# karltan0328/POPE

Hardware: AMD Instinct MI355X
Metric: image-pairs/s (DINOv2-S/14 extract+match, 640x480) (higher is better)
Workload: dtype f16x3 (fp32 operands split hi+lo into f16, 3 MFMAs per product, fp32 accumulate)

## Files before the change

include/pope_hip.h:

```cpp
#ifndef POPE_HIP_H
#define POPE_HIP_H

#include <stddef.h>

#ifdef __cplusplus
extern "C" {
#endif

#define POPE_ABI_VERSION 9

enum {
    POPE_EPI_BIAS = 0,
    POPE_EPI_BIAS_GELU = 1,
    POPE_EPI_BIAS_LS_RES = 2,
    POPE_EPI_BIAS_SWIGLU = 11,
    POPE_EPI_QKV_F16 = 8
};

enum { POPE_PREC_F32_MFMA = 0, POPE_PREC_F16X3 = 1, POPE_PREC_F16 = 2  };
enum { POPE_RANGE_PATCH = 1, POPE_RANGE_LAYERNORM = 2, POPE_RANGE_QKV = 4, POPE_RANGE_GELU = 8, POPE_RANGE_MATCH = 16,
       POPE_RANGE_INPUT = 32 };

int pope_abi_version(void);
const char* pope_error_string(int code);
// ... 7 lines not shown
int pope_linear_prec_f32(const float* A, const float* W, const float* bias, float* C, int M, int N, int K,
                         int epilogue, const float* gamma, const float* res, int precision,
                         unsigned* range_flag, void* stream);

#define POPE_PLANES_ACT_SCALE 8.0f
#define POPE_PLANES_W_SCALE 256.0f
int pope_split_planes_f32(const float* src, void* planes, int rows, int cols, float scale,
                          unsigned* range_flag, void* stream);
int pope_linear_planes_f32(const void* a_planes, const void* w_planes, const float* bias, float* C,
                           void* c_planes, int M, int N, int K, int epilogue, const float* gamma,
                           const float* res, unsigned* range_flag, void* stream);

int pope_layernorm_planes_f32(const float* x, const float* weight, const float* bias, void* y_planes,
                              int rows, int dim, float eps, unsigned* range_flag, void* stream);

int pope_linear_rowln_f32(const void* a_planes, const void* w_planes, int M, int K, const float* bias, const float* gamma,
                          const float* res, int res_mod, float* x, const float* ln_w, const float* ln_b, float eps,
                          void* ln_planes, float* ln_out, unsigned* range_flag, void* stream);
int pope_layernorm_rowln_order_f32(const float* x, const float* weight, const float* bias, void* y_planes, float* y_f32,
                                   int rows, float eps, unsigned* range_flag, void* stream);

int pope_layernorm_f16(const float* x, const float* weight, const float* bias, void* y_f16, int rows, int dim, float eps,
                       unsigned* range_flag, void* stream);
int pope_to_f16(const float* x, void* y_f16, long long n, unsigned* range_flag, void* stream);
int pope_linear_f16(const void* a_f16, const void* w_f16, const float* bias, float* C, void* c_f16, int M, int N, int K,
                    int epilogue, const float* gamma, const float* res, int res_mod, unsigned* range_flag, void* stream);
int pope_div_planes_f32(const float* src, long long batch_stride, void* planes, int n, int rows, int cols, float divisor,
                        float scale, unsigned* range_flag, void* stream);

int pope_patch_embed_f32(const float* img, const float* proj_w, const float* posb, float* tokens,
                         int B, int H, int W, int patch, int dim, void* stream);
int pope_patch_embed_planes_f32(const float* img, const void* proj_w_planes, const float* posb, float* tokens,
                                int B, int H, int W, int patch, int dim, void* a_planes_scratch,
                                size_t scratch_bytes, unsigned* range_flag, void* stream);

int pope_attention_f32(const float* qkv, float* out, int B, int N, int heads, void* stream);
int pope_attention_prec_f32(const float* qkv, float* out, int B, int N, int heads, int precision,
                            unsigned* range_flag, void* stream);
int pope_attention_planes_f32(const void* qkv_planes, void* out_planes, int B, int N, int heads, void* stream);

int pope_attention_f16(const void* qkv_f16, void* out_f16, int B, int N, int heads, void* stream);

int pope_attention_planes_diag_f32(const void* qkv_planes, void* out_planes, int B, int N, int heads, long long* exact_passes_host,
                                   void* stream);

int pope_cls_cosine_f32(const float* ref, const float* fea, int P, int D, float eps, float* scores,
                        void* stream);


typedef struct pope_vit_block_weights {
    const float *norm1_w, *norm1_b;
    const float *qkv_w, *qkv_b;
    const float *proj_w, *proj_b;
    const float *ls1;
    const float *norm2_w, *norm2_b;
    const float *fc1_w, *fc1_b;
    const float *fc2_w, *fc2_b;
    const float *ls2;
    const void *qkv_wp, *fc1_wp, *fc2_wp, *proj_wp;
} pope_vit_block_weights;

typedef struct pope_vit_weights {
    int dim, depth, heads, patch, hidden;
    const float* patch_w;
    const float *norm_w, *norm_b;
    const pope_vit_block_weights* blocks_host;
    int precision;
    const void* patch_wp;
} pope_vit_weights;

size_t pope_vit_workspace_bytes(int B, int ntok, int dim, int hidden);

enum { POPE_FFN_MLP = 0, POPE_FFN_SWIGLU = 1 };

int pope_vit_forward_f32(const pope_vit_weights* w_host, const float* img, int B, int H, int W,
                         const float* posb, float* x_prenorm, float* x_norm,
                         int n_taps, const int* tap_blocks_host, float* const* tap_out_host,
                         void* workspace, size_t workspace_bytes, unsigned* range_flag, void* stream);

int pope_vit_forward_ffn_f32(const pope_vit_weights* w_host, int ffn, const float* img, int B, int H, int W,
                             const float* posb, float* x_prenorm, float* x_norm,
                             int n_taps, const int* tap_blocks_host, float* const* tap_out_host,
                             void* workspace, size_t workspace_bytes, unsigned* range_flag, void* stream);

enum { POPE_K_PATCH_EMBED = 0, POPE_K_LAYERNORM = 1, POPE_K_GEMM_QKV = 2, POPE_K_ATTENTION = 3,
       POPE_K_GEMM_PROJ = 4, POPE_K_GEMM_FC1 = 5, POPE_K_GEMM_FC2 = 6, POPE_K_TAP_COPY = 7 };
int pope_vit_launch_count(int depth);
int pope_vit_forward_profiled_mask_f32(const pope_vit_weights* w_host, const float* img, int B, int H, int W,
                                       const float* posb, float* x_prenorm, float* x_norm,
                                       void* workspace, size_t workspace_bytes, unsigned* range_flag, void* stream,
                                       void* const* events_host, int n_events, int* kinds_host,
                                       int* n_launches_host, unsigned kind_mask);
int pope_vit_forward_ffn_profiled_mask_f32(const pope_vit_weights* w_host, int ffn, const float* img, int B, int H, int W,
                                           const float* posb, float* x_prenorm, float* x_norm,
                                           void* workspace, size_t workspace_bytes, unsigned* range_flag, void* stream,
                                           void* const* events_host, int n_events, int* kinds_host,
                                           int* n_launches_host, unsigned kind_mask);
int pope_event_create(void** event_host);
int pope_event_destroy(void* event);
int pope_event_elapsed_ms(void* start, void* stop, float* ms_host);


size_t pope_dense_match_workspace_bytes_prec(int n, int L, int S, int C, int precision, int publish_conf);
int pope_dense_match_prec_f32(const float* feat0, long long stride0, const float* feat1, long long stride1,
                              int n, int L, int S, int C, int h0, int w0, int h1, int w1,
                              float thr, int border_rm, float temperature, float scale,
                              float* conf_matrix, long long* b_ids, long long* i_ids, long long* j_ids,
                              float* mconf, float* mkpts0_c, float* mkpts1_c, int* counts,
                              void* workspace, size_t workspace_bytes, int precision, unsigned* range_flag,
                              void* stream);
size_t pope_dense_match_masked_workspace_bytes(int n, int L, int S, int C, int precision, int publish_conf, int has_border_masks);
int pope_dense_match_masked_f32(const float* feat0, long long stride0, const float* feat1, long long stride1,
                                int n, int L, int S, int C, int h0, int w0, int h1, int w1,
                                float thr, int border_rm, float temperature, float scale,
                                const float* fill_mask0, const float* fill_mask1, const float* border_mask0,
                                const float* border_mask1, const float* scale0, const float* scale1,
                                float* conf_matrix, long long* b_ids, long long* i_ids, long long* j_ids,
                                float* mconf, float* mkpts0_c, float* mkpts1_c, int* counts,
                                void* workspace, size_t workspace_bytes, int precision, unsigned* range_flag,
                                void* stream);
size_t pope_dense_match_sinkhorn_workspace_bytes(int n, int L, int S, int C, int precision, int publish_conf, int has_border_masks);
int pope_dense_match_sinkhorn_f32(const float* feat0, long long stride0, const float* feat1, long long stride1,
                                  int n, int L, int S, int C, int h0, int w0, int h1, int w1,
                                  float thr, int border_rm, const float* bin_score, int skh_iters, int skh_prefilter, float scale,
                                  const float* fill_mask0, const float* fill_mask1, const float* border_mask0,
                                  const float* border_mask1, const float* scale0, const float* scale1,
                                  float* conf_matrix, long long* b_ids, long long* i_ids, long long* j_ids,
                                  float* mconf, float* mkpts0_c, float* mkpts1_c, int* counts,
                                  void* workspace, size_t workspace_bytes, int precision, unsigned* range_flag,
                                  void* stream);
size_t pope_dense_match_workspace_bytes(int n, int L, int S);
int pope_dense_match_f32(const float* feat0, long long stride0, const float* feat1, long long stride1,
                         int n, int L, int S, int C,
                         int h0, int w0, int h1, int w1, float thr, int border_rm, float temperature,
                         float scale, float* conf_matrix, long long* b_ids, long long* i_ids,
                         long long* j_ids, float* mconf, float* mkpts0_c, float* mkpts1_c, int* counts,
                         void* workspace, size_t workspace_bytes, void* stream);


typedef struct pope_loftr_layer_weights {
    const void *q_wp, *kv_wp, *merge_wp, *mlp0_wp, *mlp1_wp;
    const float *norm1_w, *norm1_b, *norm2_w, *norm2_b;
} pope_loftr_layer_weights;
size_t pope_loftr_layer_workspace_bytes(int n, int L, int S, int C, int nhead);
int pope_loftr_encoder_layer_f32(const pope_loftr_layer_weights* w_host, float* x, const float* source,
                                 int n, int L, int S, int C, int nhead, float ln_eps, int precision,
                                 void* workspace, size_t workspace_bytes, unsigned* range_flag, void* stream);
int pope_loftr_encoder_layer_masked_f32(const pope_loftr_layer_weights* w_host, float* x, const float* source,
                                        const float* x_mask, const float* source_mask,
                                        int n, int L, int S, int C, int nhead, float ln_eps, int precision,
                                        void* workspace, size_t workspace_bytes, unsigned* range_flag, void* stream);
int pope_loftr_encoder_layer_full_f32(const pope_loftr_layer_weights* w_host, float* x, const float* source,
                                      int n, int L, int S, int C, int nhead, float ln_eps, int precision,
                                      void* workspace, size_t workspace_bytes, unsigned* range_flag, void* stream);
int pope_loftr_full_attention_f32(const float* q, const float* kv, int n, int L, int S, int C, int nhead, int precision,
                                  float* out, unsigned* range_flag, void* stream);

typedef struct pope_resnetfpn_weights {
    const void* w[22];
    const float* b[22];
} pope_resnetfpn_weights;
size_t pope_resnetfpn_workspace_bytes(int n, int H, int W);
int pope_resnetfpn_forward_f32(const pope_resnetfpn_weights* w_host, const float* gray, int n, int H, int W, int precision,
                               float* out_c, float* out_f, void* workspace, size_t workspace_bytes,
                               unsigned* range_flag, void* stream);

enum { POPE_CONV3 = 0, POPE_CONV_S2 = 1, POPE_CONV1_UP = 2, POPE_CONV_STEM = 3 };
typedef struct pope_conv_layer_args {
    int form, precision;
    int n, H, W;
    int cch, taps;
    const void* a;
    size_t a_rows;
    const void* w;
    const float* bias;
    int N, ldc;
    float slope;
    void* out_planes;
    float* out_f32;
    int zero_border;
    const void* res;
    int ldres;
    const float* up_src;
    int up_lds;
    void* scratch;
    size_t scratch_bytes;
    unsigned* range_flag;
} pope_conv_layer_args;
size_t pope_conv_layer_scratch_bytes(int form, int n, int H, int W, int cch, int taps);
int pope_conv_layer_f32(const pope_conv_layer_args* args_host, void* stream);

size_t pope_fine_preprocess_workspace_bytes(int M, int Wn, int Cc, int Cf);
int pope_fine_preprocess_f32(const float* feat_f0, const long long* strides0_host, int H0, int W0, int wc0,
// ... 291 lines not shown
```

pope_amd/_lib.py:

```python
import ctypes as C
import os
import subprocess

_CSRC = os.path.join(os.path.dirname(os.path.abspath(__file__)), "csrc")
LIB_PATH = os.environ.get("POPE_LIB_PATH") or os.path.join(_CSRC, "libpope_hip.so")

c_float_p = C.POINTER(C.c_float)
c_int_p = C.POINTER(C.c_int)
c_ll_p = C.POINTER(C.c_longlong)


class VitBlockWeights(C.Structure):
    _fields_ = [(n, C.c_void_p) for n in (
        "norm1_w", "norm1_b", "qkv_w", "qkv_b", "proj_w", "proj_b", "ls1",
        "norm2_w", "norm2_b", "fc1_w", "fc1_b", "fc2_w", "fc2_b", "ls2", "qkv_wp", "fc1_wp", "fc2_wp", "proj_wp")]


class VitWeights(C.Structure):
    _fields_ = [("dim", C.c_int), ("depth", C.c_int), ("heads", C.c_int), ("patch", C.c_int),
                ("hidden", C.c_int), ("patch_w", C.c_void_p), ("norm_w", C.c_void_p),
                ("norm_b", C.c_void_p), ("blocks_host", C.POINTER(VitBlockWeights)), ("precision", C.c_int),
                ("patch_wp", C.c_void_p)]


# ... 56 lines not shown
    _fields_ = [("num_sample", C.c_int), ("mode", C.c_int), ("layers", PoseRegressorLayer * 4), ("mlp_w", C.c_void_p * 7),
                ("mlp_b", C.c_void_p * 7)] + [(n, C.c_void_p) for n in ("trans_w", "trans_b", "rot_w", "rot_b")]


class MocopeEncoderLayer(C.Structure):
    _fields_ = [(n, C.c_void_p) for n in ("in_proj_w", "in_proj_b", "out_proj_w", "out_proj_b", "linear1_w", "linear1_b", "linear2_w",
                                           "linear2_b", "norm1_w", "norm1_b", "norm2_w", "norm2_b")]


class MocopeDecoderLayer(C.Structure):
    _fields_ = [(n, C.c_void_p) for n in ("in_proj_w", "in_proj_b", "out_proj_w", "out_proj_b", "cross_in_proj_w", "cross_in_proj_b",
                                           "cross_out_proj_w", "cross_out_proj_b", "linear1_w", "linear1_b", "linear2_w", "linear2_b",
                                           "norm1_w", "norm1_b", "norm2_w", "norm2_b", "norm3_w", "norm3_b")]


class MocopeTransformer(C.Structure):
    _fields_ = [("enc", MocopeEncoderLayer * 6), ("enc_norm_w", C.c_void_p), ("enc_norm_b", C.c_void_p),
                ("dec", MocopeDecoderLayer * 6), ("dec_norm_w", C.c_void_p), ("dec_norm_b", C.c_void_p)]


class MocopeWeights(C.Structure):
    _fields_ = [("num_sample", C.c_int), ("mode", C.c_int), ("transformer_mkpts", MocopeTransformer), ("mkpts_as_q", MocopeTransformer),
                ("cnn_as_q", MocopeTransformer), ("mlp1_w", C.c_void_p * 2), ("mlp1_b", C.c_void_p * 2), ("mlp_img_w", C.c_void_p),
                ("mlp_img_b", C.c_void_p), ("mlp2_w", C.c_void_p * 7), ("mlp2_b", C.c_void_p * 7)] + [
        (n, C.c_void_p) for n in ("trans_w", "trans_b", "rot_w", "rot_b")]


class ConvNextBlockWeights(C.Structure):
    _fields_ = [(n, C.c_void_p) for n in ("dw_w", "dw_b", "norm_w", "norm_b", "pw1_w", "pw1_b", "grn_gamma", "grn_beta", "pw2_w",
                                           "pw2_b", "pw1_wp", "pw2_wp")]


class ConvNextWeights(C.Structure):
    _fields_ = [("depths", C.c_int * 4), ("dims", C.c_int * 4), ("num_classes", C.c_int)] + [
        (n, C.c_void_p) for n in ("stem_w", "stem_b", "stem_ln_w", "stem_ln_b")] + [
        (n, C.c_void_p * 3) for n in ("ds_ln_w", "ds_ln_b", "ds_w", "ds_b", "ds_wp")] + [
        ("blocks_host", C.POINTER(ConvNextBlockWeights))] + [(n, C.c_void_p) for n in ("norm_w", "norm_b", "head_w", "head_b", "ones")]


PREC_F32_MFMA, PREC_F16X3, PREC_F16 = 0, 1, 2
PLANES_ACT_SCALE, PLANES_W_SCALE = 8.0, 256.0
PRECISIONS = {"f32": PREC_F32_MFMA, "f16x3": PREC_F16X3, "f16": PREC_F16}
FFN_KINDS = {"mlp": 0, "swiglu": 1}
EPI_BIAS_SWIGLU = 11
EPI_QKV_F16 = 8
CONV3, CONV_S2, CONV1_UP, CONV_STEM = 0, 1, 2, 3
c_uint_p = C.POINTER(C.c_uint)
F16_MAX = 65504.0
RANGE_BITS = {1: "patch embed input", 2: "LayerNorm output", 4: "q/k/v", 8: "MLP hidden (GELU / SwiGLU output)",
              16: "matcher features", 32: "op-level operand"}

PROTOTYPES = {
    "pope_abi_version": (C.c_int, []),
    "pope_error_string": (C.c_char_p, [C.c_int]),
    "pope_layernorm_f32": (C.c_int, [C.c_void_p] * 4 + [C.c_int, C.c_int, C.c_float, C.c_void_p]),
    "pope_linear_f32": (C.c_int, [C.c_void_p] * 4 + [C.c_int] * 4 + [C.c_void_p] * 3),
    "pope_linear_prec_f32": (C.c_int, [C.c_void_p] * 4 + [C.c_int] * 4 + [C.c_void_p] * 2 + [C.c_int, C.c_void_p, C.c_void_p]),
    "pope_split_planes_f32": (C.c_int, [C.c_void_p, C.c_void_p, C.c_int, C.c_int, C.c_float, C.c_void_p, C.c_void_p]),
    "pope_linear_planes_f32": (C.c_int, [C.c_void_p] * 5 + [C.c_int] * 4 + [C.c_void_p] * 4),
    "pope_layernorm_planes_f32": (C.c_int, [C.c_void_p] * 4 + [C.c_int, C.c_int, C.c_float, C.c_void_p, C.c_void_p]),
    "pope_linear_rowln_f32": (C.c_int, [C.c_void_p, C.c_void_p, C.c_int, C.c_int] + [C.c_void_p] * 3 + [C.c_int]
                              + [C.c_void_p] * 3 + [C.c_float] + [C.c_void_p] * 4),
    "pope_layernorm_rowln_order_f32": (C.c_int, [C.c_void_p] * 5 + [C.c_int, C.c_float, C.c_void_p, C.c_void_p]),
    "pope_layernorm_f16": (C.c_int, [C.c_void_p] * 4 + [C.c_int, C.c_int, C.c_float, C.c_void_p, C.c_void_p]),
    "pope_to_f16": (C.c_int, [C.c_void_p, C.c_void_p, C.c_longlong, C.c_void_p, C.c_void_p]),
    "pope_linear_f16": (C.c_int, [C.c_void_p] * 5 + [C.c_int] * 4 + [C.c_void_p, C.c_void_p, C.c_int, C.c_void_p, C.c_void_p]),
    "pope_div_planes_f32": (C.c_int, [C.c_void_p, C.c_longlong, C.c_void_p, C.c_int, C.c_int, C.c_int, C.c_float, C.c_float,
                                      C.c_void_p, C.c_void_p]),
    "pope_patch_embed_f32": (C.c_int, [C.c_void_p] * 4 + [C.c_int] * 5 + [C.c_void_p]),
    "pope_attention_f32": (C.c_int, [C.c_void_p, C.c_void_p, C.c_int, C.c_int, C.c_int, C.c_void_p]),
    "pope_attention_prec_f32": (C.c_int, [C.c_void_p, C.c_void_p, C.c_int, C.c_int, C.c_int, C.c_int, C.c_void_p, C.c_void_p]),
    "pope_patch_embed_planes_f32": (C.c_int, [C.c_void_p] * 4 + [C.c_int] * 5 + [C.c_void_p, C.c_size_t, C.c_void_p, C.c_void_p]),
    "pope_attention_planes_f32": (C.c_int, [C.c_void_p, C.c_void_p, C.c_int, C.c_int, C.c_int, C.c_void_p]),
    "pope_attention_f16": (C.c_int, [C.c_void_p, C.c_void_p, C.c_int, C.c_int, C.c_int, C.c_void_p]),
    "pope_attention_planes_diag_f32": (C.c_int, [C.c_void_p, C.c_void_p, C.c_int, C.c_int, C.c_int, c_ll_p, C.c_void_p]),
    "pope_cls_cosine_f32": (C.c_int, [C.c_void_p, C.c_void_p, C.c_int, C.c_int, C.c_float, C.c_void_p, C.c_void_p]),
    "pope_vit_workspace_bytes": (C.c_size_t, [C.c_int] * 4),
    "pope_vit_forward_f32": (C.c_int, [C.POINTER(VitWeights), C.c_void_p, C.c_int, C.c_int, C.c_int, C.c_void_p,
                                       C.c_void_p, C.c_void_p, C.c_int, c_int_p, C.POINTER(C.c_void_p),
                                       C.c_void_p, C.c_size_t, C.c_void_p, C.c_void_p]),
    "pope_vit_forward_ffn_f32": (C.c_int, [C.POINTER(VitWeights), C.c_int, C.c_void_p, C.c_int, C.c_int, C.c_int, C.c_void_p,
                                           C.c_void_p, C.c_void_p, C.c_int, c_int_p, C.POINTER(C.c_void_p),
                                           C.c_void_p, C.c_size_t, C.c_void_p, C.c_void_p]),
    "pope_vit_forward_ffn_profiled_mask_f32": (C.c_int, [C.POINTER(VitWeights), C.c_int, C.c_void_p, C.c_int, C.c_int, C.c_int,
                                                         C.c_void_p, C.c_void_p, C.c_void_p, C.c_void_p, C.c_size_t,
                                                         C.c_void_p, C.c_void_p, C.POINTER(C.c_void_p), C.c_int, c_int_p,
                                                         c_int_p, C.c_uint]),
    "pope_vit_launch_count": (C.c_int, [C.c_int]),
    "pope_vit_forward_profiled_mask_f32": (C.c_int, [C.POINTER(VitWeights), C.c_void_p, C.c_int, C.c_int, C.c_int,
                                                     C.c_void_p, C.c_void_p, C.c_void_p, C.c_void_p, C.c_size_t,
                                                     C.c_void_p, C.c_void_p, C.POINTER(C.c_void_p), C.c_int, c_int_p,
                                                     c_int_p, C.c_uint]),
    "pope_event_create": (C.c_int, [C.POINTER(C.c_void_p)]),
    "pope_event_destroy": (C.c_int, [C.c_void_p]),
    "pope_event_elapsed_ms": (C.c_int, [C.c_void_p, C.c_void_p, c_float_p]),
    "pope_dense_match_workspace_bytes": (C.c_size_t, [C.c_int] * 3),
    "pope_dense_match_f32": (C.c_int, [C.c_void_p, C.c_longlong, C.c_void_p, C.c_longlong] + [C.c_int] * 8 + [C.c_float, C.c_int, C.c_float,
                                                                                  C.c_float] + [C.c_void_p] * 8
                             + [C.c_void_p, C.c_size_t, C.c_void_p]),
    "pope_dense_match_workspace_bytes_prec": (C.c_size_t, [C.c_int] * 6),
    "pope_dense_match_prec_f32": (C.c_int, [C.c_void_p, C.c_longlong, C.c_void_p, C.c_longlong] + [C.c_int] * 8
                                  + [C.c_float, C.c_int, C.c_float, C.c_float] + [C.c_void_p] * 8
                                  + [C.c_void_p, C.c_size_t, C.c_int, C.c_void_p, C.c_void_p]),
    "pope_dense_match_masked_workspace_bytes": (C.c_size_t, [C.c_int] * 7),
    "pope_dense_match_masked_f32": (C.c_int, [C.c_void_p, C.c_longlong, C.c_void_p, C.c_longlong] + [C.c_int] * 8
                                    + [C.c_float, C.c_int, C.c_float, C.c_float] + [C.c_void_p] * 6 + [C.c_void_p] * 8
                                    + [C.c_void_p, C.c_size_t, C.c_int, C.c_void_p, C.c_void_p]),
    "pope_dense_match_sinkhorn_workspace_bytes": (C.c_size_t, [C.c_int] * 7),
    "pope_dense_match_sinkhorn_f32": (C.c_int, [C.c_void_p, C.c_longlong, C.c_void_p, C.c_longlong] + [C.c_int] * 8
                                      + [C.c_float, C.c_int, C.c_void_p, C.c_int, C.c_int, C.c_float] + [C.c_void_p] * 6
                                      + [C.c_void_p] * 8 + [C.c_void_p, C.c_size_t, C.c_int, C.c_void_p, C.c_void_p]),
    "pope_loftr_layer_workspace_bytes": (C.c_size_t, [C.c_int] * 5),
    "pope_loftr_encoder_layer_f32": (C.c_int, [C.POINTER(LoftrLayerWeights), C.c_void_p, C.c_void_p] + [C.c_int] * 5
                                     + [C.c_float, C.c_int, C.c_void_p, C.c_size_t, C.c_void_p, C.c_void_p]),
    "pope_loftr_encoder_layer_masked_f32": (C.c_int, [C.POINTER(LoftrLayerWeights)] + [C.c_void_p] * 4 + [C.c_int] * 5
                                            + [C.c_float, C.c_int, C.c_void_p, C.c_size_t, C.c_void_p, C.c_void_p]),
    "pope_loftr_encoder_layer_full_f32": (C.c_int, [C.POINTER(LoftrLayerWeights), C.c_void_p, C.c_void_p] + [C.c_int] * 5
                                          + [C.c_float, C.c_int, C.c_void_p, C.c_size_t, C.c_void_p, C.c_void_p]),
    "pope_loftr_full_attention_f32": (C.c_int, [C.c_void_p, C.c_void_p] + [C.c_int] * 6 + [C.c_void_p, C.c_void_p, C.c_void_p]),
    "pope_resnetfpn_workspace_bytes": (C.c_size_t, [C.c_int] * 3),
    "pope_resnetfpn_forward_f32": (C.c_int, [C.POINTER(ResnetFpnWeights), C.c_void_p, C.c_int, C.c_int, C.c_int, C.c_int, C.c_void_p,
                                             C.c_void_p, C.c_void_p, C.c_size_t, C.c_void_p, C.c_void_p]),
    "pope_conv_layer_scratch_bytes": (C.c_size_t, [C.c_int] * 6),
    "pope_conv_layer_f32": (C.c_int, [C.POINTER(ConvLayerArgs), C.c_void_p]),
    "pope_fine_preprocess_workspace_bytes": (C.c_size_t, [C.c_int] * 4),
    "pope_fine_preprocess_f32": (C.c_int, [C.c_void_p, c_ll_p, C.c_int, C.c_int, C.c_int, C.c_void_p, c_ll_p, C.c_int, C.c_int, C.c_int,
                                           C.c_void_p, C.c_void_p] + [C.c_int] * 4 + [C.c_void_p] * 3 + [C.c_int] * 3
                                 + [C.c_void_p] * 4 + [C.c_int, C.c_void_p] + [C.c_void_p, C.c_size_t, C.c_void_p, C.c_void_p]),
    "pope_fine_preprocess_indexed_f32": (C.c_int, [C.c_void_p, c_ll_p, C.c_int, C.c_int, C.c_int, C.c_void_p, c_ll_p, C.c_int, C.c_int,
                                                   C.c_int, C.c_void_p, C.c_void_p] + [C.c_int] * 4 + [C.c_void_p] * 3 + [C.c_int] * 3
                                         + [C.c_void_p] * 4 + [C.c_int, C.c_void_p] + [C.c_void_p, C.c_size_t, C.c_void_p]
                                         + [C.c_void_p, C.c_int, C.c_int, C.c_void_p]),
    "pope_fine_match_f32": (C.c_int, [C.c_void_p, C.c_void_p, C.c_int, C.c_int, C.c_int, C.c_void_p, C.c_float, C.c_void_p,
                                      C.c_void_p, C.c_void_p]),
    "pope_fine_match_scaled_f32": (C.c_int, [C.c_void_p, C.c_void_p, C.c_int, C.c_int, C.c_int, C.c_void_p, C.c_float, C.c_void_p,
                                             C.c_void_p, C.c_void_p, C.c_void_p, C.c_void_p]),
    "pope_sam_encoder_workspace_bytes": (C.c_size_t, [C.POINTER(SamEncoderWeights), C.c_int]),
    "pope_sam_encoder_forward_f32": (C.c_int, [C.POINTER(SamEncoderWeights), C.c_void_p, C.c_int, C.c_void_p, C.c_int, c_int_p,
                                               C.POINTER(C.c_void_p), C.c_void_p, C.c_size_t, C.c_void_p, C.c_void_p]),
    "pope_sam_decoder_workspace_bytes": (C.c_size_t, [C.POINTER(SamDecoderWeights), C.c_int, C.c_int, C.c_int]),
    "pope_sam_decoder_forward_f32": (C.c_int, [C.POINTER(SamDecoderWeights)] + [C.c_void_p] * 3 + [C.c_int, C.c_int, C.c_void_p,
                                                                                                  C.c_longlong, C.c_int]
                                     + [C.c_void_p] * 5 + [C.c_size_t, C.c_void_p, C.c_void_p]),
    "pope_sam_decoder_images_workspace_bytes": (C.c_size_t, [C.POINTER(SamDecoderWeights), C.c_int, c_int_p, C.c_int, C.c_int,
                                                             C.c_longlong]),
    "pope_sam_decoder_forward_images_f32": (C.c_int, [C.POINTER(SamDecoderWeights), C.c_void_p, C.c_int, C.c_void_p, C.c_void_p,
                                                      c_int_p, C.c_int, C.c_int, C.c_void_p, C.c_longlong, C.c_int]
                                            + [C.c_void_p] * 3 + [C.c_size_t, C.c_void_p, C.c_void_p]),
    "pope_sam_mask_embed_f32": (C.c_int, [C.POINTER(SamMaskEmbedWeights), C.c_void_p, C.c_int, C.c_void_p, C.c_void_p]),
    "pope_sam_postprocess_workspace_bytes": (C.c_size_t, [C.c_int] * 3),
    "pope_sam_postprocess_f32": (C.c_int, [C.c_void_p] + [C.c_int] * 3 + [C.c_void_p] + [C.c_int] * 6 + [C.c_double, C.c_double]
                                 + [C.c_void_p] * 4 + [C.c_size_t, C.c_void_p]),
    "pope_sam_nms_f32": (C.c_int, [C.c_void_p, C.c_void_p, C.c_int, C.c_float, C.c_void_p, C.c_void_p, C.c_void_p]),
    "pope_sam_nms_segments_f32": (C.c_int, [C.c_void_p] * 3 + [C.c_int, C.c_int, C.c_float, C.c_void_p, C.c_void_p, C.c_void_p]),
    "pope_sam_rle_u32": (C.c_int, [C.c_void_p] + [C.c_int] * 3 + [C.c_void_p] * 3 + [C.c_longlong, C.c_void_p]),
    "pope_sam_small_regions_workspace_bytes": (C.c_size_t, [C.c_int] * 3),
    "pope_sam_small_regions_u32": (C.c_int, [C.c_void_p] + [C.c_int] * 4 + [C.c_void_p] * 5 + [C.c_size_t, C.c_void_p]),
    "pope_preprocess_u8_f32": (C.c_int, [C.c_void_p, C.c_int, C.c_int, C.c_int] + [C.c_void_p] * 3 + [C.c_int] + [C.c_void_p] * 3
                               + [C.c_int] * 7 + [c_float_p, c_float_p, C.c_void_p, C.c_void_p, C.c_size_t, C.c_void_p]),
    "pope_resize_u8": (C.c_int, [C.c_void_p, C.c_int, C.c_int, C.c_int] + [C.c_void_p] * 3 + [C.c_int] + [C.c_void_p] * 3
                       + [C.c_int] * 3 + [C.c_void_p, C.c_void_p, C.c_size_t, C.c_void_p]),
    "pope_sam_preprocess_u8_f32": (C.c_int, [C.c_void_p, C.c_int, C.c_int, C.c_int] + [C.c_void_p] * 3 + [C.c_int] + [C.c_void_p] * 3
                                   + [C.c_int] * 5 + [c_float_p, c_float_p, C.c_void_p, C.c_void_p, C.c_size_t, C.c_void_p]),
    "pope_crop_normalize_u8_f32": (C.c_int, [C.c_void_p] + [C.c_int] * 7 + [c_float_p, c_float_p, C.c_void_p, C.c_void_p]),
    "pope_gray_u8_f32": (C.c_int, [C.c_void_p, C.c_int, C.c_int, C.c_int, C.c_void_p, C.c_void_p]),
    "pope_pose_images_u8_f32": (C.c_int, [C.c_void_p] + [C.c_int] * 3 + [C.c_void_p, C.c_int] + [C.c_void_p] * 4 + [C.c_int] * 3
                                + [C.c_void_p, C.c_void_p]),
    "pope_crop_warp_u8": (C.c_int, [C.c_void_p, C.c_int, C.c_int, C.c_int, C.c_void_p, C.c_void_p, C.c_int, C.c_int, C.c_int, C.c_void_p,
                                    C.c_void_p]),
    "pope_estimate_pose_workspace_bytes": (C.c_size_t, [C.c_int, C.c_longlong]),
    "pope_estimate_pose_f64": (C.c_int, [C.c_void_p] * 5 + [C.c_int, C.c_longlong, C.c_double, C.c_double, C.c_int, C.c_ulonglong]
                               + [C.c_void_p] * 5 + [C.c_void_p, C.c_size_t, C.c_void_p]),
    "pope_pose_regressor_workspace_bytes": (C.c_size_t, [C.c_int, C.c_int]),
    "pope_pose_regressor_forward_f32": (C.c_int, [C.POINTER(PoseRegressorWeights)] + [C.c_void_p] * 7 + [C.c_int] * 3 + [C.c_longlong]
                                        + [C.c_void_p] * 4 + [C.c_size_t, C.c_void_p]),
    "pope_pose_regressor_embedding_f32": (C.c_int, [C.c_void_p] * 7 + [C.c_int, C.c_int, C.c_longlong] + [C.c_void_p] * 4),
    "pope_pose_regressor_encoder_f32": (C.c_int, [C.POINTER(PoseRegressorWeights)] + [C.c_void_p] * 7 + [C.c_int] * 3 + [C.c_longlong]
                                        + [C.c_void_p] * 4),
    "pope_pose_regressor_layer_f32": (C.c_int, [C.POINTER(PoseRegressorLayer), C.c_void_p] + [C.c_int] * 3 + [C.c_void_p]),
    "pope_pose_regressor_stream_linear_f32": (C.c_int, [C.c_void_p] * 4 + [C.c_int, C.c_longlong, C.c_int, C.c_void_p]),
    "pope_pose_regressor_tail_f32": (C.c_int, [C.POINTER(PoseRegressorWeights), C.c_void_p, C.c_void_p, C.c_int] + [C.c_void_p] * 3),
    "pope_mocope_linear_f32": (C.c_int, [C.c_void_p] * 4 + [C.c_int] * 4 + [C.c_void_p]),
    "pope_mocope_attention_f32": (C.c_int, [C.c_void_p, C.c_int] * 3 + [C.c_void_p] + [C.c_int] * 4 + [C.c_void_p]),
    "pope_mocope_add_ln_f32": (C.c_int, [C.c_void_p] * 6 + [C.c_int, C.c_int, C.c_void_p]),
    "pope_mocope_ffn76_f32": (C.c_int, [C.c_void_p] * 9 + [C.c_int, C.c_void_p]),
    "pope_mocope_workspace_bytes": (C.c_size_t, [C.c_int, C.c_int]),
# ... 180 lines not shown
```

pope_amd/csrc/capi.hip:

```cpp
#include "../../include/pope_hip.h"
#include "common.h"
#include "conv_layer.h"
#include "kernels.h"
#include "linear.h"
#include "stream_device.h"
#include <cstdlib>

namespace {

__global__ __launch_bounds__(256) void cls_cosine_kernel(const float* __restrict__ ref, const float* __restrict__ fea,
                                                          int P, int D, float eps, float* __restrict__ scores) {
    const int lane = threadIdx.x & 63;
    const int p = blockIdx.x * 4 + (threadIdx.x >> 6);
    if (p >= P) return;
    const float* f = fea + size_t(p) * D;
    float dot = 0.f, nr = 0.f, nf = 0.f;
    for (int i = lane; i < D; i += 64) {
        const float a = ref[i], b = f[i];
        dot += a * b;
        nr += a * a;
        nf += b * b;
    }
    dot = wave_sum(dot);
    nr = wave_sum(nr);
// ... 119 lines not shown
    StreamDevice on_device(stream);
    return pope_launch_div_planes(src, batch_stride, planes, n, rows, cols, divisor, scale, range_flag, static_cast<hipStream_t>(stream));
}

int pope_patch_embed_f32(const float* img, const float* proj_w, const float* posb, float* tokens, int B, int H,
                         int W, int patch, int dim, void* stream) {
    StreamDevice on_device(stream);
    return pope_launch_patch_embed_f32(img, proj_w, posb, tokens, B, H, W, patch, dim, static_cast<hipStream_t>(stream));
}

int pope_patch_embed_planes_f32(const float* img, const void* proj_w_planes, const float* posb, float* tokens, int B, int H,
                                int W, int patch, int dim, void* a_planes_scratch, size_t scratch_bytes, unsigned* range_flag,
                                void* stream) {
    StreamDevice on_device(stream);
    return pope_launch_patch_embed_planes(img, proj_w_planes, posb, tokens, B, H, W, patch, dim, a_planes_scratch, scratch_bytes,
                                          range_flag, static_cast<hipStream_t>(stream));
}

int pope_attention_planes_f32(const void* qkv_planes, void* out_planes, int B, int N, int heads, void* stream) {
    StreamDevice on_device(stream);
    if (!qkv_planes || !out_planes) return POPE_ERR_ARG;
    return pope_launch_attention_f16x3_planes_io(qkv_planes, out_planes, B, N, heads, static_cast<hipStream_t>(stream));
}

int pope_attention_f16(const void* qkv_f16, void* out_f16, int B, int N, int heads, void* stream) {
    StreamDevice on_device(stream);
    return pope_launch_attention_f16_dma(qkv_f16, out_f16, B, N, heads, static_cast<hipStream_t>(stream));
}

int pope_attention_planes_diag_f32(const void* qkv_planes, void* out_planes, int B, int N, int heads, long long* exact_passes_host,
                                   void* stream) {
    StreamDevice on_device(stream);
    if (!qkv_planes || !out_planes) return POPE_ERR_ARG;
    return pope_launch_attention_f16x3_planes_io_diag(qkv_planes, out_planes, B, N, heads, exact_passes_host, static_cast<hipStream_t>(stream));
}

int pope_attention_f32(const float* qkv, float* out, int B, int N, int heads, void* stream) {
    return pope_attention_prec_f32(qkv, out, B, N, heads, POPE_PREC_F32_MFMA, nullptr, stream);
}

int pope_attention_prec_f32(const float* qkv, float* out, int B, int N, int heads, int precision, unsigned* range_flag,
                            void* stream) {
    StreamDevice on_device(stream);
    if (!qkv || !out) return POPE_ERR_ARG;
    if (precision == POPE_PREC_F16X3 && range_flag) {
        if (B <= 0 || N <= 0 || heads <= 0) return POPE_ERR_ARG;
        const int rc = pope_launch_range_check(qkv, size_t(B) * N * 3 * heads * 64, 1.0f, range_flag, POPE_RANGE_INPUT,
                                               static_cast<hipStream_t>(stream));
        if (rc) return rc;
    }
    if (precision == POPE_PREC_F16X3) return pope_launch_attention_f16x3(qkv, out, B, N, heads, static_cast<hipStream_t>(stream));
    if (precision != POPE_PREC_F32_MFMA) return POPE_ERR_ARG;
    return pope_launch_attention_f32(qkv, out, B, N, heads, static_cast<hipStream_t>(stream));
}

int pope_cls_cosine_f32(const float* ref, const float* fea, int P, int D, float eps, float* scores, void* stream) {
    StreamDevice on_device(stream);
    if (!ref || !fea || !scores || P <= 0 || D <= 0) return POPE_ERR_ARG;
    hipLaunchKernelGGL(cls_cosine_kernel, dim3((P + 3) / 4), dim3(256), 0, static_cast<hipStream_t>(stream), ref, fea,
                       P, D, eps, scores);
    return pope_check_launch();
}

int pope_event_create(void** event_host) {
    if (!event_host) return POPE_ERR_ARG;
    hipEvent_t e;
    if (hipEventCreate(&e) != hipSuccess) return POPE_ERR_LAUNCH;
    *event_host = e;
    return POPE_OK;
}
int pope_event_destroy(void* event) {
    return hipEventDestroy(static_cast<hipEvent_t>(event)) == hipSuccess ? POPE_OK : POPE_ERR_LAUNCH;
}
int pope_event_elapsed_ms(void* start, void* stop, float* ms_host) {
    if (!ms_host) return POPE_ERR_ARG;
    return hipEventElapsedTime(ms_host, static_cast<hipEvent_t>(start), static_cast<hipEvent_t>(stop)) == hipSuccess
               ? POPE_OK : POPE_ERR_LAUNCH;
}

namespace {
struct MatchLayout {
    size_t nl, ns, part, rowp, colp, pl0, pl1, simb, total;
    int ncb, nrb, nrb2, ldp;
    MatchLayout(int n, int L, int S, int C, int precision, bool publish_conf) {
        nl = pope_align256(size_t(n) * L * 4);
        ns = pope_align256(size_t(n) * S * 4);
        ncb = 2 * ((S + 127) / 128);
        nrb = 4 * ((L + 127) / 128);
        nrb2 = pope_match_nrb2(L);
        ldp = (S + 3) & ~3;
        part = pope_align256(size_t(n) * nrb2 * ldp * 4);
        const bool x3 = precision == POPE_PREC_F16X3;
        rowp = x3 ? pope_align256(size_t(n) * L * ncb * 8) : 0;
        colp = x3 ? pope_align256(size_t(n) * nrb * ldp * 4) : 0;
        pl0 = x3 ? pope_align256(size_t(n) * L * C * 4) : 0;
        pl1 = x3 ? pope_align256(size_t(n) * S * C * 4) : 0;
        simb = publish_conf ? 0 : pope_align256(size_t(n) * L * S * 4);
        total = 7 * nl + 3 * ns + part + rowp + 2 * colp + pl0 + pl1 + simb;
    }
};
}

size_t pope_dense_match_workspace_bytes(int n, int L, int S) {
    if (n <= 0 || L <= 0 || S <= 0) return 0;
    return MatchLayout(n, L, S, 4, POPE_PREC_F32_MFMA, true).total;
}

size_t pope_dense_match_workspace_bytes_prec(int n, int L, int S, int C, int precision, int publish_conf) {
    if (n <= 0 || L <= 0 || S <= 0 || C <= 0) return 0;
    return MatchLayout(n, L, S, C, precision, publish_conf != 0).total;
}

int pope_dense_match_f32(const float* feat0, long long stride0, const float* feat1, long long stride1, int n, int L,
                         int S, int C, int h0, int w0, int h1, int w1, float thr, int border_rm, float temperature, float scale, float* conf_matrix,
                         long long* b_ids, long long* i_ids, long long* j_ids, float* mconf, float* mkpts0_c,
                         float* mkpts1_c, int* counts, void* workspace, size_t workspace_bytes, void* stream) {
    return pope_dense_match_prec_f32(feat0, stride0, feat1, stride1, n, L, S, C, h0, w0, h1, w1, thr, border_rm, temperature, scale,
                                     conf_matrix, b_ids, i_ids, j_ids, mconf, mkpts0_c, mkpts1_c, counts, workspace,
                                     workspace_bytes, POPE_PREC_F32_MFMA, nullptr, stream);
}

int pope_dense_match_prec_f32(const float* feat0, long long stride0, const float* feat1, long long stride1, int n, int L,
                              int S, int C, int h0, int w0, int h1, int w1, float thr, int border_rm, float temperature, float scale, float* conf_matrix,
                              long long* b_ids, long long* i_ids, long long* j_ids, float* mconf, float* mkpts0_c,
                              float* mkpts1_c, int* counts, void* workspace, size_t workspace_bytes, int precision,
                              unsigned* range_flag, void* stream) {
    return pope_dense_match_masked_f32(feat0, stride0, feat1, stride1, n, L, S, C, h0, w0, h1, w1, thr, border_rm, temperature, scale,
                                       nullptr, nullptr, nullptr, nullptr, nullptr, nullptr, conf_matrix, b_ids, i_ids, j_ids, mconf,
                                       mkpts0_c, mkpts1_c, counts, workspace, workspace_bytes, precision, range_flag, stream);
}

size_t pope_dense_match_masked_workspace_bytes(int n, int L, int S, int C, int precision, int publish_conf, int has_border_masks) {
    if (n <= 0 || L <= 0 || S <= 0 || C <= 0) return 0;
    return MatchLayout(n, L, S, C, precision, publish_conf != 0).total + (has_border_masks ? pope_align256(size_t(n) * 4 * 4) : 0);
}

namespace {
struct SinkhornLayout {
    size_t u, v, cmax, total;
    SinkhornLayout(int n, int L, int S) {
        u = pope_align256(size_t(n) * (L + 1) * 4);
        v = pope_align256(size_t(n) * (S + 1) * 4);
        cmax = pope_align256(size_t(n) * S * 4);
        total = u + v + cmax;
    }
};

int dense_match_entry(const float* feat0, long long stride0, const float* feat1, long long stride1, int n, int L,
                      int S, int C, int h0, int w0, int h1, int w1, float thr, int border_rm, float temperature, float scale,
                      const float* fill_mask0, const float* fill_mask1, const float* border_mask0, const float* border_mask1,
                      const float* scale0, const float* scale1, float* conf_matrix, long long* b_ids, long long* i_ids,
                      long long* j_ids, float* mconf, float* mkpts0_c, float* mkpts1_c, int* counts, void* workspace,
                      size_t workspace_bytes, int precision, unsigned* range_flag, void* stream, const float* bin_score,
                      int skh_iters, int skh_prefilter) {
    if (!feat0 || !feat1 || !b_ids || !i_ids || !j_ids || !mconf || !mkpts0_c || !mkpts1_c || !counts || !workspace)
        return POPE_ERR_ARG;
    if (n <= 0 || L <= 0 || S <= 0 || C <= 0) return POPE_ERR_ARG;
    if (precision != POPE_PREC_F32_MFMA && precision != POPE_PREC_F16X3) return POPE_ERR_ARG;
    StreamDevice on_device(stream);
    const bool publish = conf_matrix != nullptr;
    const bool padded = border_mask0 || border_mask1;
    const MatchLayout lay(n, L, S, C, precision, publish);
    const size_t ext_bytes = padded ? pope_align256(size_t(n) * 4 * 4) : 0;
    const SinkhornLayout skh(n, L, S);
    if (workspace_bytes < lay.total + ext_bytes + (bin_score ? skh.total : 0)) return POPE_ERR_WORKSPACE;
    pope_carver ws{static_cast<char*>(workspace)};
    MatchParams p = {};
    p.feat0 = feat0; p.feat1 = feat1;
    p.n = n; p.L = L; p.S = S; p.C = C;
    p.bs0 = stride0; p.bs1 = stride1;
    p.h0 = h0; p.w0 = w0; p.h1 = h1; p.w1 = w1;
    p.thr = thr; p.temperature = temperature; p.border = border_rm; p.scale = scale;
    p.publish_conf = publish;
    p.ncb = lay.ncb; p.nrb = lay.nrb; p.nrb2 = lay.nrb2; p.ldp = lay.ldp;
    p.row_max = ws.take<float>(lay.nl);
    p.row_sum = ws.take<float>(lay.nl);
    p.conf_rowmax = ws.take<float>(lay.nl);
    p.row_j = ws.take<int>(lay.nl);
    p.row_conf = ws.take<float>(lay.nl);
    p.row_arg = ws.take<int>(lay.nl);
    p.row_cnt = ws.take<int>(lay.nl);
    p.col_max = ws.take<float>(lay.ns);
    p.col_sum = ws.take<float>(lay.ns);
    p.conf_colmax = ws.take<float>(lay.ns);
    p.colmax_part = ws.take<float>(lay.part);
    if (precision == POPE_PREC_F16X3) {
        p.row_part = ws.take<float>(lay.rowp);
        p.col_pmax = ws.take<float>(lay.colp);
        p.col_psum = ws.take<float>(lay.colp);
        p.planes0 = ws.take(lay.pl0);
        p.planes1 = ws.take(lay.pl1);
    }
    p.sim = publish ? conf_matrix : ws.take<float>(lay.simb);
    p.counts = counts;
    p.range_flag = range_flag;
    p.b_ids = b_ids; p.i_ids = i_ids; p.j_ids = j_ids;
    p.mconf = mconf; p.mkpts0 = mkpts0_c; p.mkpts1 = mkpts1_c;
    p.fill0 = fill_mask0; p.fill1 = fill_mask1;
    p.border0 = border_mask0; p.border1 = border_mask1;
    if (padded) p.extent = reinterpret_cast<int*>(static_cast<char*>(workspace) + lay.total);
    p.scale0 = scale0; p.scale1 = scale1;
    if (!bin_score) return pope_launch_dense_match_f32(p, static_cast<hipStream_t>(stream));
    pope_carver tail{static_cast<char*>(workspace) + lay.total + ext_bytes};
    p.bin_score = bin_score; p.skh_iters = skh_iters; p.skh_prefilter = skh_prefilter;
    p.skh_u = tail.take<float>(skh.u);
    p.skh_v = tail.take<float>(skh.v);
    p.skh_cmax = tail.take<float>(skh.cmax);
    return pope_launch_dense_match_sinkhorn_f32(p, static_cast<hipStream_t>(stream));
}
}

int pope_dense_match_masked_f32(const float* feat0, long long stride0, const float* feat1, long long stride1, int n, int L,
                                int S, int C, int h0, int w0, int h1, int w1, float thr, int border_rm, float temperature, float scale,
                                const float* fill_mask0, const float* fill_mask1, const float* border_mask0, const float* border_mask1,
                                const float* scale0, const float* scale1, float* conf_matrix, long long* b_ids, long long* i_ids,
                                long long* j_ids, float* mconf, float* mkpts0_c, float* mkpts1_c, int* counts, void* workspace,
                                size_t workspace_bytes, int precision, unsigned* range_flag, void* stream) {
    return dense_match_entry(feat0, stride0, feat1, stride1, n, L, S, C, h0, w0, h1, w1, thr, border_rm, temperature, scale, fill_mask0,
                             fill_mask1, border_mask0, border_mask1, scale0, scale1, conf_matrix, b_ids, i_ids, j_ids, mconf, mkpts0_c,
                             mkpts1_c, counts, workspace, workspace_bytes, precision, range_flag, stream, nullptr, 0, 0);
}

size_t pope_dense_match_sinkhorn_workspace_bytes(int n, int L, int S, int C, int precision, int publish_conf, int has_border_masks) {
    if (n <= 0 || L <= 0 || S <= 0 || C <= 0) return 0;
    return pope_dense_match_masked_workspace_bytes(n, L, S, C, precision, publish_conf, has_border_masks) + SinkhornLayout(n, L, S).total;
}

int pope_dense_match_sinkhorn_f32(const float* feat0, long long stride0, const float* feat1, long long stride1, int n, int L,
                                  int S, int C, int h0, int w0, int h1, int w1, float thr, int border_rm, const float* bin_score,
                                  int skh_iters, int skh_prefilter, float scale, const float* fill_mask0, const float* fill_mask1,
                                  const float* border_mask0, const float* border_mask1, const float* scale0, const float* scale1,
                                  float* conf_matrix, long long* b_ids, long long* i_ids, long long* j_ids, float* mconf,
                                  float* mkpts0_c, float* mkpts1_c, int* counts, void* workspace, size_t workspace_bytes,
                                  int precision, unsigned* range_flag, void* stream) {
    if (!bin_score || skh_iters < 1) return POPE_ERR_ARG;
    return dense_match_entry(feat0, stride0, feat1, stride1, n, L, S, C, h0, w0, h1, w1, thr, border_rm, 1.0f, scale, fill_mask0,
                             fill_mask1, border_mask0, border_mask1, scale0, scale1, conf_matrix, b_ids, i_ids, j_ids, mconf, mkpts0_c,
                             mkpts1_c, counts, workspace, workspace_bytes, precision, range_flag, stream, bin_score, skh_iters,
                             skh_prefilter);
}

size_t pope_loftr_layer_workspace_bytes(int n, int L, int S, int C, int nhead) {
    if (n <= 0 || L <= 0 || S <= 0 || C <= 0 || nhead <= 0) return 0;
    return pope_loftr_layer_workspace(n, L, S, C, nhead);
}

static int loftr_layer_call(const pope_loftr_layer_weights* w, float* x, const float* source, const float* x_mask,
                            const float* source_mask, int n, int L, int S, int C, int nhead, float ln_eps, int precision,
                            void* workspace, size_t workspace_bytes, unsigned* range_flag, void* stream, int attention) {
    if (!w || !x || !source || !workspace || n <= 0 || L <= 0 || S <= 0) return POPE_ERR_ARG;
    StreamDevice on_device(stream);
    LoftrLayerParams p = {};
    p.x = x; p.source = source; p.n = n; p.L = L; p.S = S; p.C = C; p.H = nhead;
    p.precision = precision;
    if (precision == POPE_PREC_F32_MFMA) {
        p.q_w = static_cast<const float*>(w->q_wp); p.kv_w = static_cast<const float*>(w->kv_wp);
        p.merge_w = static_cast<const float*>(w->merge_wp); p.mlp0_w = static_cast<const float*>(w->mlp0_wp);
        p.mlp1_w = static_cast<const float*>(w->mlp1_wp);
    }
    p.q_wp = w->q_wp; p.kv_wp = w->kv_wp; p.merge_wp = w->merge_wp; p.mlp0_wp = w->mlp0_wp; p.mlp1_wp = w->mlp1_wp;
    p.norm1_w = w->norm1_w; p.norm1_b = w->norm1_b; p.norm2_w = w->norm2_w; p.norm2_b = w->norm2_b;
    p.ln_eps = ln_eps; p.ws = workspace; p.ws_bytes = workspace_bytes; p.range_flag = range_flag;
    p.x_mask = x_mask; p.source_mask = source_mask;
    p.attention = attention;
    return pope_launch_loftr_layer(p, static_cast<hipStream_t>(stream));
}

int pope_loftr_encoder_layer_f32(const pope_loftr_layer_weights* w, float* x, const float* source, int n, int L, int S, int C,
                                 int nhead, float ln_eps, int precision, void* workspace, size_t workspace_bytes,
                                 unsigned* range_flag, void* stream) {
    return pope_loftr_encoder_layer_masked_f32(w, x, source, nullptr, nullptr, n, L, S, C, nhead, ln_eps, precision, workspace,
                                               workspace_bytes, range_flag, stream);
}

int pope_loftr_encoder_layer_masked_f32(const pope_loftr_layer_weights* w, float* x, const float* source, const float* x_mask,
                                        const float* source_mask, int n, int L, int S, int C, int nhead, float ln_eps, int precision,
                                        void* workspace, size_t workspace_bytes, unsigned* range_flag, void* stream) {
    return loftr_layer_call(w, x, source, x_mask, source_mask, n, L, S, C, nhead, ln_eps, precision, workspace, workspace_bytes,
                            range_flag, stream, LOFTR_ATTN_LINEAR);
}

int pope_loftr_encoder_layer_full_f32(const pope_loftr_layer_weights* w, float* x, const float* source, int n, int L, int S, int C,
                                      int nhead, float ln_eps, int precision, void* workspace, size_t workspace_bytes,
                                      unsigned* range_flag, void* stream) {
    if ((C != 256 && C != 128) || nhead != 8 || (precision != POPE_PREC_F32_MFMA && precision != POPE_PREC_F16X3)) return POPE_ERR_ARG;
    return loftr_layer_call(w, x, source, nullptr, nullptr, n, L, S, C, nhead, ln_eps, precision, workspace, workspace_bytes, range_flag,
                            stream, LOFTR_ATTN_FULL);
}

int pope_loftr_full_attention_f32(const float* q, const float* kv, int n, int L, int S, int C, int nhead, int precision, float* out,
                                  unsigned* range_flag, void* stream) {
    if (precision != POPE_PREC_F32_MFMA && precision != POPE_PREC_F16X3) return POPE_ERR_ARG;
    POPE_TRY(pope_loftr_full_attention_check(q, kv, n, L, S, C, nhead, out));
    StreamDevice on_device(stream);
    return pope_launch_loftr_full_attention(q, kv, n, L, S, C, nhead, false, out, range_flag, static_cast<hipStream_t>(stream));
}

size_t pope_conv_layer_scratch_bytes(int form, int n, int H, int W, int cch, int taps) {
    return pope_conv_layer_scratch(form, n, H, W, cch, taps);
}

int pope_conv_layer_f32(const pope_conv_layer_args* args, void* stream) {
    if (!args) return POPE_ERR_ARG;
    if (const int rc = pope_conv_layer_check(*args)) return rc;
    StreamDevice on_device(stream);
// ... 550 lines not shown
```

pope_amd/csrc/gemm_rowln.hip:

```cpp
#include <type_traits>

#include "gemm_core.h"
#include "gemm_routes.h"

namespace {

typedef _Float16 f16x4 __attribute__((ext_vector_type(4)));
typedef _Float16 f16x8 __attribute__((ext_vector_type(8)));
typedef __attribute__((ext_vector_type(4))) unsigned u32x4;
typedef __attribute__((ext_vector_type(2))) unsigned u32x2;

constexpr int RN = 384, RK = 32;
constexpr int ROWB = 64;
template <int RM_, int NWM_> struct RlGeo {
    static constexpr int RM = RM_, NWM = NWM_, NW = 4 * NWM, RTH = 64 * NW;
    static constexpr int NMI = RM / NWM / 16;
    static constexpr int STAGE_H = (RM + RN) * ROWB;
    static constexpr size_t STATS_OFF = size_t(2) * STAGE_H * sizeof(_Float16);
    static constexpr size_t CTAB_OFF = STATS_OFF + size_t(2) * 4 * RM * sizeof(float);
    static constexpr size_t PF_OFF = CTAB_OFF + size_t(4) * RN * sizeof(float);
    static constexpr size_t LDS_BYTES = PF_OFF + size_t(NW) * 256;
    static constexpr int EROWS = size_t(NW) * 16 * 100 * sizeof(float) <= size_t(STAGE_H) * sizeof(_Float16) ? 16 : 8;
    static constexpr int AROWS = RM / NW, WROWS = RN / NW;
    static constexpr int NPF = (RM * 12 + RTH - 1) / RTH;
    static_assert(size_t(NW) * EROWS * 100 * sizeof(float) <= size_t(STAGE_H) * sizeof(_Float16), "transposition buffers must fit a stage");
    static_assert(LDS_BYTES <= 160 * 1024, "LDS of a CU");
    static_assert(WROWS % 8 == 0 && AROWS % 8 == 0 && RM == NWM * NMI * 16, "eight rows per staging instruction");
};
typedef __attribute__((address_space(3))) void* lds_void_ptr;
constexpr float A_SCALE = K_PLANES_ACT_SCALE, W_SCALE = K_PLANES_W_SCALE;

__device__ __forceinline__ int pope_lane_id() {
    unsigned z = 0;
    asm volatile("" : "+s"(z));
    return int(__builtin_amdgcn_mbcnt_hi(~0u, __builtin_amdgcn_mbcnt_lo(~0u, z)));
}
__device__ __forceinline__ f32x4 mfma16(f16x8 a, f16x8 b, f32x4 c) {
    return __builtin_amdgcn_mfma_f32_16x16x32_f16(a, b, c, 0, 0, 0);
}
__device__ __forceinline__ float quad_sum(float v) {
    float a, b;
    pope_xor16_pair(v, a, b);
    pope_xor32_pair(a + b, a, b);
    return a + b;
}

#ifndef RL_LAG
#define RL_LAG 3
#endif
#ifndef RL_LAG_STAGE_BEHIND
#define RL_LAG_STAGE_BEHIND 1
#endif

#ifdef RL_STAMPS
__device__ unsigned long long g_rl_dbg[2][3][64];
#define RL_STAMP_IF(cond, slot)                                                                                    \
    do {                                                                                                           \
        if (LN && blockIdx.x == 0 && (threadIdx.x & 255) == 0 && (cond) && rl_si + (slot) < 64)    \
            g_rl_dbg[threadIdx.x >> 8][g.K == 384 ? 0 : (g.K == 1536 ? 1 : 2)][rl_si + (slot)] = wall_clock64();   \
    } while (0)
#define RL_STAMP(slot) RL_STAMP_IF(true, slot)
#define RL_STAMP_K(slot) RL_STAMP_IF(kt == 1, slot)
#else
#define RL_STAMP(slot) do {} while (0)
#define RL_STAMP_K(slot) do {} while (0)
#endif

__device__ __forceinline__ void rl_barrier() {
    __builtin_amdgcn_fence(__ATOMIC_RELEASE, "workgroup", "local");
    __builtin_amdgcn_s_barrier();
    __builtin_amdgcn_fence(__ATOMIC_ACQUIRE, "workgroup", "local");
}

enum { RL_LN_PLANES = 0, RL_LN_F32 = 1, RL_BIAS_PLANES = 2, RL_GELU_PLANES = 3 };

template <class G, int MODE, bool RES_TABLE>
__global__ __launch_bounds__(G::RTH) void gemm_rowln16_kernel(const GemmParams g, int n_tiles, int ncol) {
    constexpr bool LN = MODE == RL_LN_PLANES || MODE == RL_LN_F32, LN_PLANES = MODE == RL_LN_PLANES;
    constexpr int RM = G::RM, NMI = G::NMI, RTH = G::RTH, STAGE_H = G::STAGE_H, EROWS = G::EROWS, AROWS = G::AROWS, WROWS = G::WROWS;
    constexpr int WMR = 16 * NMI;
    constexpr int NIA = AROWS / 8, NIW = WROWS / 8;
    extern __shared__ __attribute__((aligned(16))) float smem[];
    _Float16* lds = reinterpret_cast<_Float16*>(smem);
    float* stats = reinterpret_cast<float*>(reinterpret_cast<char*>(smem) + G::STATS_OFF);
    float* ctab = reinterpret_cast<float*>(reinterpret_cast<char*>(smem) + G::CTAB_OFF);

    const int tid = threadIdx.x, lane = tid & 63;
    const int wave = __builtin_amdgcn_readfirstlane(tid >> 6);
    const int wm = wave >> 2, wn = wave & 3;
    const int nk = g.K / RK;
    const unsigned lda4 = unsigned(g.lda) * 4u, ldw4 = unsigned(g.ldw) * 4u;
    const __amdgpu_buffer_rsrc_t ra = __builtin_amdgcn_make_buffer_rsrc(const_cast<void*>(g.a_pl), 0, unsigned(g.M) * lda4, 0x00020000);
    const __amdgpu_buffer_rsrc_t rw = __builtin_amdgcn_make_buffer_rsrc(const_cast<void*>(g.w_pl), 0, unsigned(g.N) * ldw4, 0x00020000);
    auto row_tile = [&](int t) -> int { return LN ? t : t / ncol; };
    auto col_tile = [&](int t) -> int { return LN ? 0 : t - (t / ncol) * ncol; };

    const int grid = gridDim.x, full_rounds = n_tiles / grid;
    const int remapped = xcd_remap(blockIdx.x, grid);
    const int tail_cand = full_rounds * grid + int(blockIdx.x);
    const int tail_tile = tail_cand < n_tiles ? tail_cand : n_tiles;
    auto tile_of = [&](int ord) -> int {
        const int in_tail = pope_uniform_select(ord == full_rounds, tail_tile, n_tiles);
        return pope_uniform_select(ord < full_rounds, ord * grid + remapped, in_tail);
    };
    const int first = tile_of(0);
    if (first >= n_tiles) return;
    if (LN && tid < RN) {
        const float gm = g.gamma ? g.gamma[tid] : 1.0f;
        ctab[tid] = gm * (1.0f / (A_SCALE * W_SCALE));
        ctab[RN + tid] = (g.bias ? g.bias[tid] : 0.f) * gm;
        ctab[2 * RN + tid] = g.ln_w[tid];
        ctab[3 * RN + tid] = g.ln_b[tid];
    }

    const unsigned a8 = 8u * lda4, w8 = 8u * ldw4;
    auto dma = [&](int stage, int t, int kt_) {
        int ln_ = pope_lane_id();
        asm volatile("" : "+v"(ln_));
        const int r8 = ln_ >> 3, piece = (ln_ & 7) ^ r8;
        const int lt = t < n_tiles ? t : n_tiles - 1;
        _Float16* S_ = lds + stage * STAGE_H;
        const unsigned vt = unsigned(row_tile(lt) * RM + AROWS * wave + r8) * lda4 + unsigned(piece) * 16u;
        const unsigned ko = unsigned(kt_) * 128u + unsigned(col_tile(lt)) * unsigned(RN) * ldw4;
        const unsigned vw0 = unsigned(WROWS * wave + r8) * ldw4 + unsigned(piece) * 16u;
#pragma unroll
        for (int i = 0; i < NIA; ++i)
            __builtin_amdgcn_raw_ptr_buffer_load_lds(ra, (lds_void_ptr)(S_ + (AROWS * wave + 8 * i) * ROWB), 16, vt + i * a8, unsigned(kt_) * 128u, 0, LN ? 3 : 0);
#pragma unroll
        for (int i = 0; i < NIW; ++i)
            __builtin_amdgcn_raw_ptr_buffer_load_lds(rw, (lds_void_ptr)(S_ + (RM + WROWS * wave + 8 * i) * ROWB), 16, vw0, ko + i * w8, 0, 0);
    };
    f32x4 acc[NMI][6];
    auto zero_acc = [&]() {
#pragma unroll
        for (int mi = 0; mi < NMI; ++mi)
#pragma unroll
            for (int ni = 0; ni < 6; ++ni) acc[mi][ni] = f32x4{0.f, 0.f, 0.f, 0.f};
    };

    const __amdgpu_buffer_rsrc_t rx = __builtin_amdgcn_make_buffer_rsrc(g.C, 0, unsigned(g.M) * unsigned(RN) * 4u, 0x00020000);
    const __amdgpu_buffer_rsrc_t rln = __builtin_amdgcn_make_buffer_rsrc(LN_PLANES ? g.ln_planes : static_cast<void*>(g.ln_f32), 0,
                                                                         unsigned(g.M) * unsigned(RN) * 4u, 0x00020000);
    const __amdgpu_buffer_rsrc_t rres = __builtin_amdgcn_make_buffer_rsrc(
        const_cast<float*>(g.res), 0, unsigned(RES_TABLE ? g.res_mod : g.M) * unsigned(g.ldres) * 4u, 0x00020000);

    lds_void_ptr pf_pad = (lds_void_ptr)(reinterpret_cast<char*>(smem) + G::PF_OFF + wave * 256);
    auto prefetch_res = [&](int tile_, int j) {
        int t_ = wave * 64 + pope_lane_id();
        asm volatile("" : "+v"(t_));
        const unsigned L = unsigned(t_) + unsigned(RTH) * unsigned(j), row = L / 12u, pc = L - 12u * row;
        const unsigned off = RM * 12 % RTH == 0 || L < unsigned(RM * 12) ? (unsigned(tile_) * RM + row) * unsigned(RN) * 4u + pc * 128u : 0xFFFFFF00u;
        __builtin_amdgcn_raw_ptr_buffer_load_lds(rres, pf_pad, 4, off, 0, 0, 0);
    };

    int rl_si = 0;
    [[maybe_unused]] auto epilogue = [&](int tile, int free_stage) {
        const int m0 = tile * RM;
        float* wreg = reinterpret_cast<float*>(lds + free_stage * STAGE_H) + wave * (EROWS * 100);
        int elane = pope_lane_id();
        asm volatile("" : "+v"(elane));
        RL_STAMP(1);
        int l15 = elane & 15, q4 = elane >> 4;
        asm volatile("" : "+v"(l15), "+v"(q4));
        const int er = l15 & (EROWS - 1);
#pragma unroll
        for (int mi = 0; mi < NMI; ++mi)
#pragma unroll
            for (int ni = 0; ni < 6; ++ni) asm volatile("" : "+v"(acc[mi][ni]));
        const int col0 = wn * 96 + 4 * q4;
#pragma unroll
        for (int ni = 0; ni < 6; ++ni) {
            const f32x4 gam = *reinterpret_cast<const f32x4*>(ctab + col0 + 16 * ni);
            const f32x4 bia = *reinterpret_cast<const f32x4*>(ctab + RN + col0 + 16 * ni);
#pragma unroll
            for (int mi = 0; mi < NMI; ++mi) {
                const unsigned row = unsigned(m0 + wm * WMR + mi * 16 + l15);
                const unsigned rr = RES_TABLE ? row % unsigned(g.res_mod) : row;
                const f32x4 r = __builtin_bit_cast(f32x4, __builtin_amdgcn_raw_buffer_load_b128(
                                    rres, rr * unsigned(g.ldres) * 4u + unsigned(col0) * 4u, ni * 64, 0));
                acc[mi][ni] = r + acc[mi][ni] * gam + bia;
            }
#pragma unroll
            for (int mi = 0; mi < NMI; ++mi) asm volatile("" : "+v"(acc[mi][ni]));
            __builtin_amdgcn_sched_barrier(0);
        }
        __builtin_amdgcn_sched_barrier(0);
        RL_STAMP(2);
        const int rl = wm * WMR + l15;
#pragma unroll
        for (int mi = 0; mi < NMI; ++mi) {
            float s = 0.f;
#pragma unroll
            for (int ni = 0; ni < 6; ++ni) s += (acc[mi][ni][0] + acc[mi][ni][1]) + (acc[mi][ni][2] + acc[mi][ni][3]);
            s = quad_sum(s);
            if (q4 == 0) stats[wn * RM + rl + 16 * mi] = s;
        }
        rl_barrier();
        float mean[NMI], rstd[NMI];
#pragma unroll
        for (int mi = 0; mi < NMI; ++mi) {
            const float* p = stats + rl + 16 * mi;
            mean[mi] = ((p[0] + p[RM]) + (p[2 * RM] + p[3 * RM])) * (1.0f / float(RN));
        }
        __builtin_amdgcn_sched_barrier(0);
        RL_STAMP(3);
        auto store_lines = [&](const __amdgpu_buffer_rsrc_t& rdst, int row_base) {
            int el = elane;
            asm volatile("" : "+v"(el));
            const int epiece = el & 7;
#pragma unroll
            for (int t = 0; t < (EROWS * 3) / 8; ++t) {
                const int L = t * 8 + (el >> 3), row = (L * 43) >> 7, ln = L - 3 * row;
                const f32x4 v = *reinterpret_cast<const f32x4*>(&wreg[row * 100 + ln * 32 + epiece * 4]);
                const unsigned off = unsigned(row_base + row) * unsigned(RN) * 4u + unsigned(wn * 96 + ln * 32 + epiece * 4) * 4u;
                __builtin_amdgcn_raw_buffer_store_b128(__builtin_bit_cast(u32x4, v), rdst, off, 0, 0);
            }
        };
#pragma unroll
        for (int mi = 0; mi < NMI; ++mi) {
#pragma unroll
            for (int h = 0; h < 16 / EROWS; ++h) {
                if (EROWS == 16 || (l15 >> 3) == h) {
#pragma unroll
                    for (int ni = 0; ni < 6; ++ni) *reinterpret_cast<f32x4*>(&wreg[er * 100 + ni * 16 + 4 * q4]) = acc[mi][ni];
                }
                __builtin_amdgcn_wave_barrier();
                store_lines(rx, m0 + wm * WMR + mi * 16 + h * EROWS);
                __builtin_amdgcn_wave_barrier();
            }
        }
#pragma unroll
        for (int mi = 0; mi < NMI; ++mi) {
            float qs = 0.f;
#pragma unroll
            for (int ni = 0; ni < 6; ++ni) {
                const f32x4 d = acc[mi][ni] - mean[mi];
                acc[mi][ni] = d;
                qs += (d[0] * d[0] + d[1] * d[1]) + (d[2] * d[2] + d[3] * d[3]);
            }
            qs = quad_sum(qs);
            if (q4 == 0) stats[4 * RM + wn * RM + rl + 16 * mi] = qs;
        }
        rl_barrier();
#pragma unroll
        for (int mi = 0; mi < NMI; ++mi) {
            const float* p = stats + 4 * RM + rl + 16 * mi;
            const float var = ((p[0] + p[RM]) + (p[2 * RM] + p[3 * RM])) * (1.0f / float(RN));
            rstd[mi] = 1.0f / sqrtf(var + g.ln_eps);
        }
        __builtin_amdgcn_sched_barrier(0);
        RL_STAMP(4);
        const int live = g.M - (m0 + rl);
        float finite_probe = 0.f;
#pragma unroll
        for (int mi = 0; mi < NMI; ++mi) finite_probe += 16 * mi < live ? __builtin_fabsf(mean[mi]) + rstd[mi] : 0.f;
        f32x2 amax = {0.f, 0.f};
#pragma unroll
        for (int mi = 0; mi < NMI; ++mi) {
#pragma unroll
            for (int h = 0; h < 16 / EROWS; ++h) {
                if (EROWS == 16 || (l15 >> 3) == h) {
#pragma unroll
                    for (int ni = 0; ni < 6; ++ni) {
                        const f32x4 lw = *reinterpret_cast<const f32x4*>(ctab + 2 * RN + col0 + 16 * ni);
                        const f32x4 lb = *reinterpret_cast<const f32x4*>(ctab + 3 * RN + col0 + 16 * ni);
                        const f32x4 y = acc[mi][ni] * rstd[mi] * lw + lb;
                        if constexpr (LN_PLANES) {
                            const f32x4 ys = y * A_SCALE;
                            pope_amax4x2(amax, 16 * mi < live ? ys : f32x4{0.f, 0.f, 0.f, 0.f});
                            f16x4 hi, lo;
                            pope_split4(ys, hi, lo);
                            const int c = ni * 16 + 4 * q4;
                            _Float16* hp = reinterpret_cast<_Float16*>(wreg) + er * 200 + pope_planes_col(c);
                            *reinterpret_cast<f16x4*>(hp) = hi;
                            *reinterpret_cast<f16x4*>(hp + 32) = lo;
                        } else {
                            *reinterpret_cast<f32x4*>(&wreg[er * 100 + ni * 16 + 4 * q4]) = y;
                        }
                    }
                }
                __builtin_amdgcn_wave_barrier();
                store_lines(rln, m0 + wm * WMR + mi * 16 + h * EROWS);
                __builtin_amdgcn_wave_barrier();
            }
        }
        if constexpr (LN_PLANES)
            pope_range_flag(g.range_flag, POPE_RANGE_LAYERNORM,
                            !(__builtin_fmaxf(amax[0], amax[1]) < POPE_F16_OVERFLOW) ||
                                !(finite_probe < INFINITY));
        RL_STAMP(5);
    };

    const __amdgpu_buffer_rsrc_t rcp = __builtin_amdgcn_make_buffer_rsrc(LN ? static_cast<void*>(g.C) : g.c_pl, 0,
                                                                         unsigned(g.M) * unsigned(g.ldc) * 4u, 0x00020000);
    [[maybe_unused]] auto epilogue_planes = [&](int tile, int free_stage) {
        const int m0 = row_tile(tile) * RM, n0 = col_tile(tile) * RN;
        float* wreg = reinterpret_cast<float*>(lds + free_stage * STAGE_H) + wave * (EROWS * 100);
        int elane = pope_lane_id();
        asm volatile("" : "+v"(elane));
        int l15 = elane & 15, q4 = elane >> 4;
        asm volatile("" : "+v"(l15), "+v"(q4));
        const int er = l15 & (EROWS - 1);
#pragma unroll
        for (int mi = 0; mi < NMI; ++mi)
#pragma unroll
            for (int ni = 0; ni < 6; ++ni) asm volatile("" : "+v"(acc[mi][ni]));
        const int col0 = n0 + wn * 96 + 4 * q4;
        constexpr float inv = 1.0f / (A_SCALE * W_SCALE);
        f32x4 bias[6];
#pragma unroll
        for (int ni = 0; ni < 6; ++ni) bias[ni] = g.bias ? *reinterpret_cast<const f32x4*>(g.bias + col0 + 16 * ni) : f32x4{0.f, 0.f, 0.f, 0.f};
        f32x2 amax = {0.f, 0.f};
#pragma unroll
        for (int mi = 0; mi < NMI; ++mi) {
#pragma unroll
            for (int h = 0; h < 16 / EROWS; ++h) {
                if (EROWS == 16 || (l15 >> 3) == h) {
#pragma unroll
                    for (int ni = 0; ni < 6; ++ni) {
                        f32x4 v = acc[mi][ni] * inv + bias[ni];
                        if constexpr (MODE == RL_GELU_PLANES) {
                            const f32x2 g01 = pope_gelu_erf_pair(f32x2{v[0], v[1]}), g23 = pope_gelu_erf_pair(f32x2{v[2], v[3]});
                            v = f32x4{g01[0], g01[1], g23[0], g23[1]};
                        }
                        pope_amax4x2(amax, v);
                        f16x4 hi, lo;
                        pope_split4(v * A_SCALE, hi, lo);
                        const int c = ni * 16 + 4 * q4;
                        _Float16* hp = reinterpret_cast<_Float16*>(wreg) + er * 200 + pope_planes_col(c);
                        *reinterpret_cast<f16x4*>(hp) = hi;
                        *reinterpret_cast<f16x4*>(hp + 32) = lo;
                    }
                }
                __builtin_amdgcn_wave_barrier();
                {
                    int el = elane;
                    asm volatile("" : "+v"(el));
                    const int epiece = el & 7;
                    const int row_base = m0 + wm * WMR + mi * 16 + h * EROWS;
#pragma unroll
                    for (int t = 0; t < (EROWS * 3) / 8; ++t) {
                        const int L = t * 8 + (el >> 3), row = (L * 43) >> 7, ln = L - 3 * row;
                        const f32x4 v = *reinterpret_cast<const f32x4*>(&wreg[row * 100 + ln * 32 + epiece * 4]);
                        const unsigned off = unsigned(row_base + row) * unsigned(g.ldc) * 4u + unsigned(n0 + wn * 96 + ln * 32 + epiece * 4) * 4u;
                        __builtin_amdgcn_raw_buffer_store_b128(__builtin_bit_cast(u32x4, v), rcp, off, 0, 2);
                    }
                }
                __builtin_amdgcn_wave_barrier();
            }
        }
        pope_range_flag(g.range_flag, g.range_bit, !(__builtin_fmaxf(amax[0], amax[1]) * A_SCALE < POPE_F16_OVERFLOW));
    };

    dma(0, first, 0);
    zero_acc();
    int tile = first, kt = 0, ord = 0, next_tile = tile_of(1);
    RL_STAMP(0);

    constexpr int LAG = RL_LAG;
    static_assert(LAG >= 0 && LAG <= 3 && G::NW == 8, "waves 4 - 7 are the SIMD partners of waves 0 - 3");
    [[maybe_unused]] const bool late = LAG > 0 && wave >= 4;
    enum { ROLE_IN_PHASE = 0, ROLE_LATE_FIRST = 1, ROLE_LATE = 2 };
    f16x8 ah[NMI], al[NMI];
    [[maybe_unused]] f16x8 dwl[LAG > 0 ? LAG : 1], dwh[LAG > 0 ? LAG : 1];
    auto mfma_block = [&](int ni, const f16x8& l, const f16x8& h, [[maybe_unused]] bool first_of_step) {
#pragma unroll
        for (int mi = 0; mi < NMI; ++mi) {
            acc[mi][ni] = mfma16(l, ah[mi], acc[mi][ni]);
// ... 39 lines not shown
                wh[nxt] = *reinterpret_cast<const f16x8*>(S + w_row + (ni + 1) * 16 * ROWB + sw_hi);
            } else if constexpr (ROLE != ROLE_IN_PHASE) {
#pragma unroll
                for (int j = 0; j < LAG; ++j) {
                    dwl[j] = *reinterpret_cast<const f16x8*>(S + w_row + (NOW + j) * 16 * ROWB + sw_lo);
                    dwh[j] = *reinterpret_cast<const f16x8*>(S + w_row + (NOW + j) * 16 * ROWB + sw_hi);
                }
            }
            if constexpr (LN && !RES_TABLE)
                if (ni == 2 && g.rl_prefetch && kt >= nk - 1 - G::NPF && kt < nk - 1 && nk > G::NPF) prefetch_res(tile, kt - (nk - 1 - G::NPF));
            mfma_block(ni, wl[cur], wh[cur], ROLE != ROLE_LATE && ni == 0);
            __builtin_amdgcn_sched_barrier(0);
        }
    };

    for (int s = 0; tile < n_tiles; ++s) {
        if (!LN || kt != 0 || ord == 0) __builtin_amdgcn_s_waitcnt(0x0f70);
        if constexpr (LAG > 0) __builtin_amdgcn_s_waitcnt(0xc07f);
        rl_barrier();
        RL_STAMP_K(6);
        const _Float16* S = lds + (s & 1) * STAGE_H;
        if constexpr (LAG > 0) {
            int role = pope_uniform_select(late, pope_uniform_select(kt == 0, int(ROLE_LATE_FIRST), int(ROLE_LATE)), int(ROLE_IN_PHASE));
            if (role == ROLE_IN_PHASE) kstep(std::integral_constant<int, ROLE_IN_PHASE>{}, s, S);
            asm volatile("" : "+s"(role));
            if (role == ROLE_LATE_FIRST) kstep(std::integral_constant<int, ROLE_LATE_FIRST>{}, s, S);
            asm volatile("" : "+s"(role));
            if (role == ROLE_LATE) kstep(std::integral_constant<int, ROLE_LATE>{}, s, S);
        } else {
            kstep(std::integral_constant<int, ROLE_IN_PHASE>{}, s, S);
        }
        if (++kt == nk) {
            rl_barrier();
            if constexpr (LAG > 0) {
                if (late) deferred_blocks();
#pragma unroll
                for (int t = 0; t < NMI; ++t) ah[t] = __builtin_nondeterministic_value(ah[t]), al[t] = __builtin_nondeterministic_value(al[t]);
#pragma unroll
                for (int j = 0; j < LAG; ++j) dwl[j] = __builtin_nondeterministic_value(dwl[j]), dwh[j] = __builtin_nondeterministic_value(dwh[j]);
            }
            if constexpr (LN) epilogue(tile, s & 1);
            else epilogue_planes(tile, s & 1);
            zero_acc();
            kt = 0;
            tile = next_tile;
            next_tile = tile_of(++ord + 1);
            rl_si += 8;
            RL_STAMP(0);
        }
    }
    __builtin_amdgcn_s_waitcnt(0x0f70);
}

template <class G, int MODE, bool RES_TABLE>
int launch_rowln_geo(const GemmParams& g, hipStream_t stream) {
    const int ncol = (g.N + RN - 1) / RN;
    const int tiles = ((g.M + G::RM - 1) / G::RM) * ncol, cus = pope_cu_count();
    return pope_launch_lds<gemm_rowln16_kernel<G, MODE, RES_TABLE>>(dim3(tiles < cus ? tiles : cus), dim3(G::RTH), G::LDS_BYTES, stream,
                                                                    g, tiles, ncol);
}

template <int MODE, bool RES_TABLE>
int launch_rowln(const GemmParams& g, hipStream_t stream) {
    const long long cus = pope_cu_count(), ncol = (g.N + RN - 1) / RN;
    const long long r128 = (((g.M + 127) / 128) * ncol + cus - 1) / cus * 128, r192 = (((g.M + 191) / 192) * ncol + cus - 1) / cus * 192;
    return r192 <= r128 ? launch_rowln_geo<RlGeo<192, 2>, MODE, RES_TABLE>(g, stream)
                        : launch_rowln_geo<RlGeo<128, 2>, MODE, RES_TABLE>(g, stream);
}

}

#ifdef RL_STAMPS
extern "C" int pope_lab_rowln_stamps(unsigned long long* host384) {
    return hipMemcpyFromSymbol(host384, HIP_SYMBOL(g_rl_dbg), sizeof(unsigned long long) * 384) == hipSuccess ? 0 : -1;
}
#endif

bool pope_gemm_rowln_supported(const GemmParams& g) {
    return g.N == RN && g.ldc == RN && g.K >= 2 * RK && (g.K % RK) == 0 && g.lda == g.K && g.ldw == g.K && g.ldres == RN &&
           size_t(g.M + 192) * g.lda * 4 < (size_t(1) << 32) && size_t(g.M + 192) * RN * 4 < (size_t(1) << 32) - 512;
}

bool pope_gemm_rowln_args_ok(const GemmParams& g) {
    if (!g.a_pl || !g.w_pl || !g.C || !g.res || !g.ln_w || !g.ln_b || (!g.ln_planes) == (!g.ln_f32) || g.M <= 0) return false;
    if (!pope_gemm_rowln_supported(g)) return false;
    return g.res_mod >= 0 && (g.res_mod > 0 || g.gamma);
}

int pope_launch_gemm_rowln(const GemmParams& g_in, hipStream_t stream) {
    GemmParams g = g_in;
    g.rl_prefetch = 1;
    if (!pope_gemm_rowln_args_ok(g)) return POPE_ERR_ARG;
    if (g.res_mod > 0) return g.ln_planes ? launch_rowln<RL_LN_PLANES, true>(g, stream) : launch_rowln<RL_LN_F32, true>(g, stream);
    return g.ln_planes ? launch_rowln<RL_LN_PLANES, false>(g, stream) : launch_rowln<RL_LN_F32, false>(g, stream);
}

bool pope_stream384_supported(const GemmParams& g) {
    if (g.plain || !g.a_pl || !g.w_pl || !g.c_pl || g.conv_cch > 0 || g.nbatch > 1) return false;
    if (g.epilogue != EPI_BIAS && g.epilogue != EPI_BIAS_GELU) return false;
    if (g.N % RN || g.K < 2 * RK || (g.K % RK) || g.lda != g.K || g.ldw != g.K || g.ldc != g.N) return false;
    if (size_t(g.M + 192) * g.lda * 4 >= (size_t(1) << 32) || size_t(g.N) * g.ldw * 4 >= (size_t(1) << 32) ||
        size_t(g.M + 192) * g.ldc * 4 >= (size_t(1) << 32) - 512)
        return false;
    return size_t((g.M + 191) / 192) * (g.N / RN) >= size_t(4) * pope_cu_count();
}

int pope_launch_stream384(const GemmParams& g, hipStream_t stream) {
    return g.epilogue == EPI_BIAS_GELU ? launch_rowln_geo<RlGeo<192, 2>, RL_GELU_PLANES, false>(g, stream)
                                       : launch_rowln_geo<RlGeo<192, 2>, RL_BIAS_PLANES, false>(g, stream);
}
```

pope_amd/csrc/kernels.h:

```cpp
#pragma once
#include <hip/hip_runtime.h>
#include <stddef.h>
#include <type_traits>
#include <utility>
#include "../../include/pope_hip.h"

enum GemmEpilogue {
    EPI_BIAS = 0,
    EPI_BIAS_GELU = 1,
    EPI_BIAS_LS_RES = 2,
    EPI_POSB = 3,
    EPI_BIAS_RELU = 5,
    EPI_SIM = 4,
    EPI_SIM_MASK = 10,
    EPI_SAM_QKV = 7,
    EPI_QKV_F16 = 8,
    EPI_CONV_UP = 9,
    EPI_BIAS_SWIGLU = 11,
    EPI_CONV = 6,
};

struct GemmParams {
    const float* A;
    const float* W;
    const float* bias;
    float* C;
    int lda, ldw, ldc;
    int M, N, K;
    int epilogue;
    const float* gamma;
    const float* res;
    int ldres;
    int nbatch;
    float alpha, divisor;
    float* row_part;
    float* col_pmax;
    float* col_psum;
    int ncb, nrb, ldp;
    float divisor_eff, rdiv;
    int res_mod;
    const void* a_pl;
    const void* w_pl;
    void* c_pl;
    unsigned* range_flag;
    unsigned range_bit;
    const float* ln_w; const float* ln_b;
    float ln_eps;
    void* ln_planes;
    float* ln_f32;
    int rl_prefetch;
    const void* res_pl;
    int ldres_pl;
    float act_slope;
    int conv_cch, conv_wp;
    int conv_s2_taps, conv_s2_hpi, conv_s2_hpo, conv_s2_wpo, conv_s2_in_rows;
    const float* up_src;
    int up_lds, up_hp, up_wp, up_n;
    float up_sh, up_sw;
    unsigned up_m_hw, up_m_w;
    int plain;
    void *sam_q, *sam_k, *sam_v;
    unsigned sam_bytes[3];
    const int* sam_rowmap;
    int sam_hd, sam_dim, sam_npad, sam_dq, sam_dv;
    float sam_qscale;
    const float* posb;
    int ntok, img_h, img_w, patch, grid_w;
    const float* sim_mask0;
    const float* sim_mask1;
};

int pope_launch_gemm_nt_f32(const GemmParams& g, hipStream_t stream);

bool pope_gemm_f16x3_supported(const GemmParams& g);
int pope_launch_gemm_planes(const GemmParams& g, hipStream_t stream);
bool pope_wide_conv_s2_supported(const GemmParams& g);
bool pope_gemm_rowln_supported(const GemmParams& g);
bool pope_gemm_rowln_args_ok(const GemmParams& g);
int pope_launch_gemm_rowln(const GemmParams& g, hipStream_t stream);
constexpr float K_PLANES_ACT_SCALE = 8.0f, K_PLANES_W_SCALE = 256.0f;

template <typename F, int... NV>
inline bool pope_ln_dispatch(int dim, F&& f, std::integer_sequence<int, NV...>) {
    return ((dim == 128 * NV && (f(std::integral_constant<int, NV>{}), true)) || ...);
}
template <typename F>
inline bool pope_ln_dispatch(int dim, F&& f) {
    return pope_ln_dispatch(dim, f, std::integer_sequence<int, 1, 2, 3, 4, 5, 6, 8, 10, 12, 16>{});
}
inline bool pope_ln_width_ok(int dim) { return pope_ln_dispatch(dim, [](auto) {}); }

int pope_launch_layernorm_planes(const float* x, int ldx, const float* w, const float* b, void* y_pl,
                                 int rows, int dim, float eps, unsigned* range_flag, hipStream_t stream);
int pope_launch_layernorm_rowln_order(const float* x, const float* w, const float* b, void* y_planes, float* y_f32, int rows, float eps,
                                      unsigned* flag, hipStream_t stream);
int pope_launch_im2col_planes(const float* img, void* a_planes, int B, int H, int W, int patch, int kp, unsigned* range_flag,
                              hipStream_t stream);
int pope_launch_patch_embed_f32(const float* img, const float* proj_w, const float* posb, float* tokens, int B, int H, int W,
                                int patch, int dim, hipStream_t stream);
int pope_launch_patch_embed_planes(const float* img, const void* proj_w_planes, const float* posb, float* tokens, int B, int H, int W,
                                   int patch, int dim, void* a_planes_scratch, size_t scratch_bytes, unsigned* range_flag,
                                   hipStream_t stream);
int pope_launch_div_planes(const float* src, long long bs, void* planes, int n, int rows, int cols, float divisor, float scale,
                           unsigned* range_flag, hipStream_t stream);
int pope_launch_split_planes(const float* src, void* pl, int rows, int ld, float scale, unsigned* range_flag, hipStream_t stream);
int pope_launch_range_check(const float* x, size_t n, float scale, unsigned* flag, unsigned bit, hipStream_t stream);
int pope_launch_gemm_nt_f16x3(const GemmParams& g, hipStream_t stream);

int pope_launch_layernorm_f32(const float* x, int ldx, const float* w, const float* b, float* y, int ldy,
                              int rows, int dim, float eps, hipStream_t stream);

int pope_launch_layernorm_f16(const float* x, const float* w, const float* b, void* y_f16, int rows, int dim, float eps, unsigned* flag,
                              hipStream_t stream);
int pope_launch_to_f16(const float* x, void* y_f16, long long n4, unsigned* flag, hipStream_t stream);
int pope_launch_attention_f16_dma(const void* qkv_f16, void* out_f16, int B, int N, int heads, hipStream_t stream);
int pope_launch_attention_f32(const float* qkv, float* out, int B, int N, int heads, hipStream_t stream);
int pope_launch_attention_f16x3(const float* qkv, float* out, int B, int N, int heads, hipStream_t stream);
int pope_launch_attention_f16x3_planes_io_diag(const void* qkv_planes, void* out_planes, int B, int N, int heads, long long* exact_passes_host,
                                               hipStream_t stream);
int pope_launch_attention_f16x3_planes_io(const void* qkv_planes, void* out_planes, int B, int N, int heads, hipStream_t stream);

struct MatchParams {
    const float* feat0;
    const float* feat1;
    int n, L, S, C;
    long long bs0, bs1;
    int h0, w0, h1, w1;
    float thr, temperature;
    int border;
    float scale;
    float* sim;
    int publish_conf;
    void* planes0; void* planes1;
    float* row_part; float* col_pmax; float* col_psum;
    int ncb, nrb, ldp;
    float* row_max; float* row_sum;
    float* col_max; float* col_sum;
    float* colmax_part;
    int nrb2;
    float* conf_colmax;
    float* conf_rowmax;
    int* row_arg; int* row_cnt;
    int* row_j;
    float* row_conf;
    unsigned* range_flag;
    int* counts;
    long long* b_ids; long long* i_ids; long long* j_ids;
    float* mconf; float* mkpts0; float* mkpts1;
    const float* fill0; const float* fill1;
    const float* border0; const float* border1;
    int* extent;
    const float* scale0; const float* scale1;
    const float* bin_score;
    int skh_iters, skh_prefilter;
    float* skh_u; float* skh_v; float* skh_cmax;
    float skh_norm, skh_log_mu_bin, skh_log_nu_bin;
};
int pope_match_nrb2(int L);
int pope_launch_dense_match_f32(const MatchParams& p, hipStream_t stream);
int pope_launch_dense_match_sinkhorn_f32(MatchParams p, hipStream_t stream);
int pope_launch_sinkhorn_passes(const MatchParams& p, hipStream_t stream);

#ifdef __HIPCC__
struct RowBest {
    float v;
    int idx, cnt;
    __device__ __forceinline__ void take(float c, int col) {
        const bool gt = c > v, eq = c == v;
        cnt = gt ? 1 : cnt + (eq ? 1 : 0);
        idx = gt ? col : idx;
        v = gt ? c : v;
    }
    __device__ __forceinline__ void merge(float ov, int oidx, int ocnt) {
        const bool gt = ov > v, eq = ov == v;
        cnt = gt ? ocnt : cnt + (eq ? ocnt : 0);
        idx = gt ? oidx : (eq && oidx < idx ? oidx : idx);
        v = gt ? ov : v;
    }
};
#endif

struct PreprocParams {
    const unsigned char* img;
    int P, Hin, Win;
    const int *hstart, *hcount, *hk; int kh;
    const int *vstart, *vcount, *vk; int kv;
    int top, left, ch, cw;
    int row0, nrows;
    float mean[3], std[3];
    unsigned char* tmp;
    float* out;
};
int pope_launch_preprocess(const PreprocParams& p, hipStream_t stream);
struct ResizeParams {
    const unsigned char* img;
    int P, Hin, Win;
    const int *hstart, *hcount, *hk; int kh;
    const int *vstart, *vcount, *vk; int kv;
    int OH, OW;
    bool f32;
    int S, flip;
    float mean[3], std[3];
    void* out;
    unsigned char* tmp; size_t tmp_bytes;
};
int pope_resize_check(const ResizeParams& p);
int pope_launch_resize(const ResizeParams& p, hipStream_t stream);
int pope_launch_gray(const unsigned char* bgr, size_t npix, float* out, hipStream_t stream);
int pope_launch_crop_warp(const unsigned char* img, int H, int W, int C, const double* minv, const int* win, int P, int oh, int ow,
                          unsigned char* out, hipStream_t stream);
int pope_launch_crop_norm(const unsigned char* img, int P, int Hin, int Win, int top, int left, int ch, int cw, const float* mean,
                          const float* std, float* out, hipStream_t stream);
struct PoseImagesParams {
    const unsigned char* src;
    int P, Hin, Win;
    const int* rows; int Q;
// ... 254 lines not shown
```

pope_amd/csrc/match.hip:

```cpp
#include "gemm_core.h"
#include "kernels.h"

namespace {

using namespace gemm_core;

constexpr float L2E = 1.44269504088896340736f;

template <bool MASKED>
__global__ __launch_bounds__(THREADS, 3) void sim_kernel(const MatchParams p, float inv_unused) {
    extern __shared__ __attribute__((aligned(16))) float smem[];
    const int tiles_n = (p.S + BN - 1) / BN;
    const int tile = xcd_remap(blockIdx.x, gridDim.x);
    const int m0 = (tile / tiles_n) * BM, n0 = (tile % tiles_n) * BN;
    const int pair = blockIdx.y;
    const float* f0 = p.feat0 + size_t(pair) * p.bs0;
    const float* f1 = p.feat1 + size_t(pair) * p.bs1;
    const float norm = sqrtf(float(p.C));

    f32x16 acc[2][2];
    mainloop(fn_loader([&](int row, int k) {
                 f32x4 v = {0.f, 0.f, 0.f, 0.f};
                 if (m0 + row < p.L && k < p.C) v = *reinterpret_cast<const f32x4*>(f0 + size_t(m0 + row) * p.C + k) / norm;
                 return v;
// ... 399 lines not shown
                cbest[k][1] = fmaxf(cbest[k][1], c[k][1]);
                m = fmaxf(m, fmaxf(c[k][0], c[k][1]));
            }
            if constexpr (PUBLISH) {
                const __amdgpu_buffer_rsrc_t rs = row_rsrc(row);
#pragma unroll
                for (int k = 0; k < NK; ++k) __builtin_amdgcn_raw_buffer_store_b64(__builtin_bit_cast(u32x2m, c[k]), rs, voff, 512 * k, 0);
            }
            m = wave_max(m);
            int first = BIG, cnt = 0;
#pragma unroll
            for (int k = 0; k < NK; ++k) {
                const unsigned long long m0 = __ballot(c[k][0] == m), m1 = __ballot(c[k][1] == m);
                cnt += __popcll(m0) + __popcll(m1);
                const int a = pope_uniform_select(m0 != 0, 2 * __builtin_ctzll(m0 | (1ull << 63)), BIG);
                const int b2 = pope_uniform_select(m1 != 0, 2 * __builtin_ctzll(m1 | (1ull << 63)) + 1, BIG);
                const int cand = c0 + 128 * k + (a < b2 ? a : b2);
                first = first < cand ? first : cand;
            }
            if (lane == 0) {
                float bv = m;
                int bi = first, bc = cnt;
                if (c0) {
                    const float pv = p.conf_rowmax[prow + row];
                    const int pi = p.row_arg[prow + row], pc = p.row_cnt[prow + row];
                    if (pv > m) { bv = pv; bi = pi; bc = pc; }
                    else if (pv == m) { bi = pi; bc = pc + cnt; }
                }
                p.conf_rowmax[prow + row] = bv;
                p.row_arg[prow + row] = bi;
                p.row_cnt[prow + row] = bc;
            }
        };
        f32x2 ca[NK], cb[NK];
        fetch(row0, ca);
#pragma unroll 1
        for (int r = 0; r < RPW; r += 2) {
            fetch(row0 + r + 1, cb);
            process(row0 + r, ca);
            fetch(row0 + r + 2, ca);
            process(row0 + r + 1, cb);
        }
        if (c0) __syncthreads();
#pragma unroll
        for (int k = 0; k < NK; ++k) *reinterpret_cast<f32x2*>(&cmax_s[wave][128 * k + 2 * lane]) = cbest[k];
        __syncthreads();
        float* out = p.colmax_part + (size_t(pair) * p.nrb2 + blk) * p.ldp;
        for (int cc = threadIdx.x; cc < 128 * NK && c0 + cc < p.S; cc += 256)
            out[c0 + cc] = fmaxf(fmaxf(cmax_s[0][cc], cmax_s[1][cc]), fmaxf(cmax_s[2][cc], cmax_s[3][cc]));
    }
}

template <bool PUBLISH>
void launch_conf_pass(const MatchParams& p, hipStream_t stream) {
    const dim3 blocks((p.L + CP_ROWS - 1) / CP_ROWS, p.n);
    if (p.S & 1) {
        hipLaunchKernelGGL((conf_pass_kernel<PUBLISH>), blocks, dim3(256), 0, stream, p);
        return;
    }
    const int nk = (p.S + 127) / 128;
    if (nk <= 4) hipLaunchKernelGGL((conf_pass_fast_kernel<PUBLISH, 4>), blocks, dim3(256), 0, stream, p);
    else if (nk <= 8) hipLaunchKernelGGL((conf_pass_fast_kernel<PUBLISH, 8>), blocks, dim3(256), 0, stream, p);
    else if (nk <= 12) hipLaunchKernelGGL((conf_pass_fast_kernel<PUBLISH, 12>), blocks, dim3(256), 0, stream, p);
    else hipLaunchKernelGGL((conf_pass_fast_kernel<PUBLISH, 16>), blocks, dim3(256), 0, stream, p);
}

template <bool PUBLISH>
void launch_conf_and_select(const MatchParams& p, hipStream_t stream) {
    launch_conf_pass<PUBLISH>(p, stream);
    hipLaunchKernelGGL(combine_colmax_kernel, dim3((p.S + 255) / 256, p.n), dim3(256), 0, stream, p);
    if (p.extent) hipLaunchKernelGGL((select_kernel<PUBLISH, true>), dim3((p.L + 3) / 4, p.n), dim3(256), 0, stream, p);
    else hipLaunchKernelGGL((select_kernel<PUBLISH, false>), dim3((p.L + 3) / 4, p.n), dim3(256), 0, stream, p);
}

}

int pope_match_nrb2(int L) { return (L + CP_ROWS - 1) / CP_ROWS; }

namespace {

int check_match_params(const MatchParams& p) {
    if (p.n <= 0 || p.L <= 0 || p.S <= 0 || p.C <= 0 || (p.C & 3) || p.n > 65535) return POPE_ERR_ARG;
    if (p.L != p.h0 * p.w0 || p.S != p.h1 * p.w1) return POPE_ERR_ARG;
    if (p.bs0 < (long long)p.L * p.C || p.bs1 < (long long)p.S * p.C || (p.bs0 & 3) || (p.bs1 & 3)) return POPE_ERR_ARG;
    if ((reinterpret_cast<uintptr_t>(p.feat0) & 15) || (reinterpret_cast<uintptr_t>(p.feat1) & 15)) return POPE_ERR_ARG;
    if (!p.sim || !p.colmax_part || p.nrb2 != pope_match_nrb2(p.L) || p.ldp < p.S || (p.ldp & 3)) return POPE_ERR_ARG;
    if ((p.border0 || p.border1) && !p.extent) return POPE_ERR_ARG;
    return POPE_OK;
}

int launch_contraction(const MatchParams& p, bool col_stats, hipStream_t stream) {
    const bool fill = p.fill0 || p.fill1;
    bool sim_done = false;
    if (p.planes0 && p.planes1 && p.row_part && p.col_pmax && p.col_psum && (p.C & 31) == 0 && p.C >= 64) {
        const float norm = sqrtf(float(p.C));
        int rc = pope_launch_div_planes(p.feat0, p.bs0, p.planes0, p.n, p.L, p.C, norm, K_PLANES_W_SCALE, p.range_flag, stream);
        if (!rc) rc = pope_launch_div_planes(p.feat1, p.bs1, p.planes1, p.n, p.S, p.C, norm, K_PLANES_W_SCALE, p.range_flag, stream);
        if (rc) return rc;
        GemmParams g = {};
        g.a_pl = p.planes0; g.w_pl = p.planes1; g.C = p.sim;
        g.M = p.L; g.N = p.S; g.K = p.C; g.lda = p.C; g.ldw = p.C; g.ldc = p.S;
        g.nbatch = p.n;
        g.divisor_eff = p.temperature * (K_PLANES_W_SCALE * K_PLANES_W_SCALE);
        g.rdiv = 1.0f / g.divisor_eff;
        g.epilogue = EPI_SIM;
        g.row_part = p.row_part; g.col_pmax = p.col_pmax; g.col_psum = p.col_psum;
        g.ncb = p.ncb; g.nrb = p.nrb; g.ldp = p.ldp;
        g.sim_mask0 = p.fill0; g.sim_mask1 = p.fill1;
        rc = pope_launch_gemm_planes(g, stream);
        if (rc == 0) {
            sim_done = true;
            hipLaunchKernelGGL(combine_row_stats_kernel, dim3(unsigned((size_t(p.n) * p.L + 255) / 256)), dim3(256), 0, stream, p);
            if (col_stats) hipLaunchKernelGGL(combine_col_stats_kernel, dim3((p.S + 255) / 256, p.n), dim3(256), 0, stream, p);
        } else if (rc != POPE_ERR_ARG) {
            return rc;
        }
    }
    if (!sim_done) {
        const int tiles = ((p.L + BM - 1) / BM) * ((p.S + BN - 1) / BN);
        if (fill) hipLaunchKernelGGL(sim_kernel<true>, dim3(tiles, p.n), dim3(THREADS), LDS_BYTES, stream, p, 0.f);
        else hipLaunchKernelGGL(sim_kernel<false>, dim3(tiles, p.n), dim3(THREADS), LDS_BYTES, stream, p, 0.f);
        hipLaunchKernelGGL(row_stats_kernel, dim3((p.L + 3) / 4, p.n), dim3(256), 0, stream, p);
        if (col_stats) hipLaunchKernelGGL(col_stats_kernel, dim3((p.S + 63) / 64, p.n), dim3(256), 0, stream, p);
    }
    return POPE_OK;
}

void launch_compaction(const MatchParams& p, hipStream_t stream) {
    hipLaunchKernelGGL(count_kernel, dim3(p.n), dim3(256), 0, stream, p);
    if (p.scale0 || p.scale1) hipLaunchKernelGGL(scatter_kernel<true>, dim3(p.n), dim3(256), 0, stream, p);
    else hipLaunchKernelGGL(scatter_kernel<false>, dim3(p.n), dim3(256), 0, stream, p);
}

}

int pope_launch_dense_match_f32(const MatchParams& p, hipStream_t stream) {
    POPE_TRY(check_match_params(p));
    POPE_TRY(launch_contraction(p, true, stream));
    if (p.extent) hipLaunchKernelGGL(border_extent_kernel, dim3(p.n, 2), dim3(256), 0, stream, p);
    if (p.publish_conf) launch_conf_and_select<true>(p, stream);
    else launch_conf_and_select<false>(p, stream);
    launch_compaction(p, stream);
    return pope_check_launch();
}

int pope_launch_dense_match_sinkhorn_f32(MatchParams p, hipStream_t stream) {
    POPE_TRY(check_match_params(p));
    if (!p.bin_score || p.skh_iters < 1 || !p.skh_u || !p.skh_v || !p.skh_cmax) return POPE_ERR_ARG;
    p.temperature = 1.0f;
    p.skh_norm = -logf(float(p.L + p.S));
    p.skh_log_mu_bin = logf(float(p.S)) + p.skh_norm;
    p.skh_log_nu_bin = logf(float(p.L)) + p.skh_norm;
    POPE_TRY(launch_contraction(p, false, stream));
    if (p.extent) hipLaunchKernelGGL(border_extent_kernel, dim3(p.n, 2), dim3(256), 0, stream, p);
    POPE_TRY(pope_launch_sinkhorn_passes(p, stream));
    hipLaunchKernelGGL(combine_colmax_kernel, dim3((p.S + 255) / 256, p.n), dim3(256), 0, stream, p);
    if (p.extent) hipLaunchKernelGGL((select_kernel<true, true>), dim3((p.L + 3) / 4, p.n), dim3(256), 0, stream, p);
    else hipLaunchKernelGGL((select_kernel<true, false>), dim3((p.L + 3) / 4, p.n), dim3(256), 0, stream, p);
    launch_compaction(p, stream);
    return pope_check_launch();
}
```

pope_amd/csrc/vit_forward.hip:

```cpp
#include "../../include/pope_hip.h"
#include "common.h"
#include "kernels.h"
#include "linear.h"
#include "stream_device.h"

namespace {

struct Recorder {
    void* const* events;
    int capacity;
    int* kinds;
    int n;
    unsigned mask = ~0u;
    bool open = false;
    bool mark(int kind, hipStream_t stream) {
        if (!events) return true;
        const bool sel = kind >= 0 && ((mask >> kind) & 1u);
        if (!sel && !open) return true;
        if (n >= capacity) return false;
        if (hipEventRecord(static_cast<hipEvent_t>(events[n]), stream) != hipSuccess) return false;
        if (kinds) kinds[n] = sel ? kind : -1;
        open = sel;
        ++n;
        return true;
    }
};

}

int pope_launch_patch_embed_f32(const float* img, const float* proj_w, const float* posb, float* tokens, int B, int H, int W,
                                int patch, int dim, hipStream_t stream) {
    if (!img || !proj_w || !posb || !tokens || B <= 0 || patch <= 0 || H % patch || W % patch) return POPE_ERR_ARG;
    GemmParams g = {};
    g.A = img; g.W = proj_w; g.C = tokens;
    g.K = 3 * patch * patch;
    g.ldw = g.K; g.ldc = dim;
    g.ntok = 1 + (H / patch) * (W / patch);
    g.M = B * g.ntok; g.N = dim;
    g.epilogue = EPI_POSB;
    g.posb = posb;
    g.img_h = H; g.img_w = W; g.patch = patch; g.grid_w = W / patch;
    return pope_launch_gemm_nt_f32(g, stream);
}

int pope_launch_patch_embed_planes(const float* img, const void* proj_w_planes, const float* posb, float* tokens, int B, int H, int W,
                                   int patch, int dim, void* a_planes_scratch, size_t scratch_bytes, unsigned* range_flag,
                                   hipStream_t stream) {
    if (!img || !proj_w_planes || !posb || !tokens || !a_planes_scratch || B <= 0 || patch <= 0 || H % patch || W % patch)
        return POPE_ERR_ARG;
    const int kp = (3 * patch * patch + 31) & ~31, ntok = 1 + (H / patch) * (W / patch);
    if (scratch_bytes < size_t(B) * ntok * kp * 4) return POPE_ERR_WORKSPACE;
    POPE_TRY(pope_launch_im2col_planes(img, a_planes_scratch, B, H, W, patch, kp, range_flag, stream));
    GemmParams g = pope_linear_params(LINEAR_PLANES, a_planes_scratch, proj_w_planes, nullptr, tokens, nullptr, B * ntok, dim, kp,
                                      EPI_BIAS_LS_RES, nullptr, posb, ntok);
    g.range_bit = 0;
    return pope_launch_gemm_planes(g, stream);
}

static int vit_forward_impl(const pope_vit_weights* w, int ffn, const float* img, int B, int H, int W, const float* posb,
                            float* x_prenorm, float* x_norm, int n_taps, const int* tap_blocks_host,
                            float* const* tap_out_host, void* workspace, size_t workspace_bytes, unsigned* range_flag,
                            void* stream_, Recorder& rec) {
    if (!w || !img || !posb || !x_prenorm || !workspace || !w->blocks_host) return POPE_ERR_ARG;
    if (w->dim != w->heads * 64 || w->patch <= 0 || H % w->patch || W % w->patch || B <= 0) return POPE_ERR_ARG;
    if (n_taps < 0 || (n_taps > 0 && (!tap_blocks_host || !tap_out_host))) return POPE_ERR_ARG;
    hipStream_t stream = static_cast<hipStream_t>(stream_);
    const int dim = w->dim, hidden = w->hidden, prec = w->precision;
    if (prec != POPE_PREC_F32_MFMA && prec != POPE_PREC_F16X3 && prec != POPE_PREC_F16) return POPE_ERR_ARG;
    if (ffn != POPE_FFN_MLP && ffn != POPE_FFN_SWIGLU) return POPE_ERR_ARG;
    const bool swiglu = ffn == POPE_FFN_SWIGLU;
    if (swiglu && (prec == POPE_PREC_F16 || hidden <= 0 || (hidden & 31))) return POPE_ERR_ARG;
    for (int i = 0; swiglu && i < w->depth; ++i)
        if (!w->blocks_host[i].fc1_w || !w->blocks_host[i].fc1_b || !w->blocks_host[i].fc2_w) return POPE_ERR_ARG;
    StreamDevice on_device(stream_);
    const int fc1_n = swiglu ? 2 * hidden : hidden, fc1_epi = swiglu ? int(EPI_BIAS_SWIGLU) : int(EPI_BIAS_GELU);
    const int ntok = 1 + (H / w->patch) * (W / w->patch);
    const int rows = B * ntok;
    if (workspace_bytes < pope_vit_workspace_bytes(B, ntok, dim, hidden)) return POPE_ERR_WORKSPACE;

    pope_carver ws{static_cast<char*>(workspace)};
    float* xn = ws.take<float>(size_t(rows) * dim * sizeof(float));
    float* big = reinterpret_cast<float*>(ws.at);
    const size_t big_bytes = workspace_bytes - size_t(ws.at - static_cast<char*>(workspace));
    float* qkv = big;
    float* att = big + size_t(rows) * 3 * dim;
    float* hid = big;
    float* x = x_prenorm;
    const float eps = 1e-6f;

    bool planes = (prec == POPE_PREC_F16X3 || prec == POPE_PREC_F16) && dim % 32 == 0 && dim >= 64 && hidden % 32 == 0;
    for (int i = 0; planes && i < w->depth; ++i) {
        const pope_vit_block_weights& k = w->blocks_host[i];
        planes = k.qkv_wp && k.proj_wp && k.fc1_wp && k.fc2_wp;
    }
    const bool plain = prec == POPE_PREC_F16;
    if (plain && (!planes || !w->patch_wp || (dim & 63) || (hidden & 63))) return POPE_ERR_ARG;
    const GemmParams probe = pope_linear_params(LINEAR_PLANES, nullptr, nullptr, nullptr, nullptr, nullptr, rows, dim, dim, EPI_BIAS_LS_RES);
    const bool fusable = planes && !plain && w->patch_wp && pope_gemm_rowln_supported(probe);
    const bool small = fusable && 3 * ((rows + 127) / 128) <= 2 * pope_cu_count();
    const bool fused = fusable && !small;
    const LinearForm form = plain ? LINEAR_PLAIN : planes ? LINEAR_PLANES : LINEAR_F32;

    auto norm = [&](const float* nw, const float* nb) {
        if (plain) return pope_launch_layernorm_f16(x, nw, nb, xn, rows, dim, eps, range_flag, stream);
        if (small) return pope_launch_layernorm_rowln_order(x, nw, nb, xn, nullptr, rows, eps, range_flag, stream);
        if (planes) return pope_launch_layernorm_planes(x, dim, nw, nb, xn, rows, dim, eps, range_flag, stream);
        return pope_launch_layernorm_f32(x, dim, nw, nb, xn, dim, rows, dim, eps, stream);
    };
    auto linear = [&](const void* a, const float* wf, const void* wp, const float* bias, float* Cf, void* c_pk, int N, int K, int epi,
                      const float* gamma, const float* res) {
        if (form == LINEAR_F32) {
            if (!wf) return POPE_ERR_ARG;
            float* C = Cf ? Cf : static_cast<float*>(c_pk);
            return pope_launch_gemm_nt_f32(pope_linear_params(form, a, wf, bias, C, nullptr, rows, N, K, epi, gamma, res), stream);
        }
        GemmParams g = pope_linear_params(form, a, wp, bias, Cf, c_pk, rows, N, K, epi, gamma, res, 0, plain || c_pk ? range_flag : nullptr);
        if (epi == EPI_QKV_F16) { g.sam_dim = N / 3; g.sam_qscale = 0.125f * 1.44269504088896340736f; }
        return pope_launch_gemm_planes(g, stream);
    };
    auto rowln = [&](const void* a_pl, const void* w_pl, int K, const float* bias, const float* gamma, const float* res, int res_mod,
                     const float* ln_w, const float* ln_b, void* ln_planes, float* ln_f32) {
        return pope_launch_gemm_rowln(pope_linear_rowln_params(a_pl, w_pl, rows, dim, K, bias, gamma, res, res_mod, x, ln_w, ln_b, eps,
                                                               ln_planes, ln_f32, range_flag), stream);
    };
    auto attention = [&] {
        if (plain) return pope_launch_attention_f16_dma(qkv, att, B, ntok, w->heads, stream);
        if (planes) return pope_launch_attention_f16x3_planes_io(qkv, att, B, ntok, w->heads, stream);
        return pope_launch_attention_f32(qkv, att, B, ntok, w->heads, stream);
    };

#define POPE_MARK(kind) do { if (!rec.mark(kind, stream)) return POPE_ERR_ARG; } while (0)
    POPE_MARK(POPE_K_PATCH_EMBED);
    if (fused) {
        const int kp = (3 * w->patch * w->patch + 31) & ~31;
        if (big_bytes < size_t(rows) * kp * 4) return POPE_ERR_WORKSPACE;
        POPE_TRY(pope_launch_im2col_planes(img, big, B, H, W, w->patch, kp, range_flag, stream));
        const pope_vit_block_weights& k0 = w->blocks_host[0];
        POPE_TRY(rowln(big, w->patch_wp, kp, nullptr, nullptr, posb, ntok, k0.norm1_w, k0.norm1_b, xn, nullptr));
    } else if (planes && w->patch_wp) {
        POPE_TRY(pope_launch_patch_embed_planes(img, w->patch_wp, posb, x, B, H, W, w->patch, dim, big, big_bytes, range_flag, stream));
    } else {
        POPE_TRY(pope_launch_patch_embed_f32(img, w->patch_w, posb, x, B, H, W, w->patch, dim, stream));
    }
    for (int i = 0; i < w->depth; ++i) {
        const pope_vit_block_weights& k = w->blocks_host[i];
        if (!fused) {
            POPE_MARK(POPE_K_LAYERNORM);
            POPE_TRY(norm(k.norm1_w, k.norm1_b));
        }
        POPE_MARK(POPE_K_GEMM_QKV);
        POPE_TRY(linear(xn, k.qkv_w, k.qkv_wp, k.qkv_b, nullptr, qkv, 3 * dim, dim, plain ? EPI_QKV_F16 : EPI_BIAS, nullptr, nullptr));
        POPE_MARK(POPE_K_ATTENTION);
        POPE_TRY(attention());
        POPE_MARK(POPE_K_GEMM_PROJ);
        if (fused) POPE_TRY(rowln(att, k.proj_wp, dim, k.proj_b, k.ls1, x, 0, k.norm2_w, k.norm2_b, xn, nullptr));
        else POPE_TRY(linear(att, k.proj_w, k.proj_wp, k.proj_b, x, nullptr, dim, dim, EPI_BIAS_LS_RES, k.ls1, x));
        if (!fused) {
            POPE_MARK(POPE_K_LAYERNORM);
            POPE_TRY(norm(k.norm2_w, k.norm2_b));
        }
        POPE_MARK(POPE_K_GEMM_FC1);
        POPE_TRY(linear(xn, k.fc1_w, k.fc1_wp, k.fc1_b, nullptr, hid, fc1_n, dim, fc1_epi, nullptr, nullptr));
        POPE_MARK(POPE_K_GEMM_FC2);
        if (fused && i + 1 < w->depth) {
            const pope_vit_block_weights& kn = w->blocks_host[i + 1];
            POPE_TRY(rowln(hid, k.fc2_wp, hidden, k.fc2_b, k.ls2, x, 0, kn.norm1_w, kn.norm1_b, xn, nullptr));
        } else if (fused && x_norm) {
            POPE_TRY(rowln(hid, k.fc2_wp, hidden, k.fc2_b, k.ls2, x, 0, w->norm_w, w->norm_b, nullptr, x_norm));
        } else {
            POPE_TRY(linear(hid, k.fc2_w, k.fc2_wp, k.fc2_b, x, nullptr, dim, hidden, EPI_BIAS_LS_RES, k.ls2, x));
        }
        for (int t = 0; t < n_taps; ++t)
            if (tap_blocks_host[t] == i && tap_out_host[t]) {
                POPE_MARK(POPE_K_TAP_COPY);
                if (hipMemcpyAsync(tap_out_host[t], x, size_t(rows) * dim * sizeof(float), hipMemcpyDeviceToDevice, stream) != hipSuccess)
                    return POPE_ERR_LAUNCH;
            }
    }
    if (x_norm && !fused) {
        POPE_MARK(POPE_K_LAYERNORM);
        if (small) POPE_TRY(pope_launch_layernorm_rowln_order(x, w->norm_w, w->norm_b, nullptr, x_norm, rows, eps, nullptr, stream));
        else POPE_TRY(pope_launch_layernorm_f32(x, dim, w->norm_w, w->norm_b, x_norm, dim, rows, dim, eps, stream));
    }
    POPE_MARK(-1);
#undef POPE_MARK
    return POPE_OK;
}

extern "C" {

size_t pope_vit_workspace_bytes(int B, int ntok, int dim, int hidden) {
    if (B <= 0 || ntok <= 0 || dim <= 0 || hidden <= 0) return 0;
    const size_t rows = size_t(B) * ntok;
    const size_t big = size_t(hidden) > size_t(4) * dim ? size_t(hidden) : size_t(4) * dim;
    return pope_align256(rows * dim * sizeof(float)) + pope_align256(rows * big * sizeof(float));
}

int pope_vit_forward_f32(const pope_vit_weights* w, const float* img, int B, int H, int W, const float* posb,
                         float* x_prenorm, float* x_norm, int n_taps, const int* tap_blocks_host,
                         float* const* tap_out_host, void* workspace, size_t workspace_bytes, unsigned* range_flag,
                         void* stream) {
    return pope_vit_forward_ffn_f32(w, POPE_FFN_MLP, img, B, H, W, posb, x_prenorm, x_norm, n_taps, tap_blocks_host, tap_out_host,
                                    workspace, workspace_bytes, range_flag, stream);
}

int pope_vit_forward_ffn_f32(const pope_vit_weights* w, int ffn, const float* img, int B, int H, int W, const float* posb,
                             float* x_prenorm, float* x_norm, int n_taps, const int* tap_blocks_host,
                             float* const* tap_out_host, void* workspace, size_t workspace_bytes, unsigned* range_flag,
                             void* stream) {
    Recorder rec{nullptr, 0, nullptr, 0};
    return vit_forward_impl(w, ffn, img, B, H, W, posb, x_prenorm, x_norm, n_taps, tap_blocks_host, tap_out_host, workspace,
                            workspace_bytes, range_flag, stream, rec);
}

int pope_vit_forward_profiled_mask_f32(const pope_vit_weights* w, const float* img, int B, int H, int W,
                                       const float* posb, float* x_prenorm, float* x_norm, void* workspace,
                                       size_t workspace_bytes, unsigned* range_flag, void* stream,
                                       void* const* events_host, int n_events, int* kinds_host, int* n_launches_host,
                                       unsigned kind_mask) {
    return pope_vit_forward_ffn_profiled_mask_f32(w, POPE_FFN_MLP, img, B, H, W, posb, x_prenorm, x_norm, workspace, workspace_bytes,
                                                  range_flag, stream, events_host, n_events, kinds_host, n_launches_host, kind_mask);
}

int pope_vit_forward_ffn_profiled_mask_f32(const pope_vit_weights* w, int ffn, const float* img, int B, int H, int W,
                                           const float* posb, float* x_prenorm, float* x_norm, void* workspace,
                                           size_t workspace_bytes, unsigned* range_flag, void* stream,
                                           void* const* events_host, int n_events, int* kinds_host, int* n_launches_host,
                                           unsigned kind_mask) {
    if (!events_host || n_events < 2 || !kinds_host || !n_launches_host) return POPE_ERR_ARG;
    Recorder rec{events_host, n_events, kinds_host, 0};
    rec.mask = kind_mask;
    const int rc = vit_forward_impl(w, ffn, img, B, H, W, posb, x_prenorm, x_norm, 0, nullptr, nullptr, workspace,
                                    workspace_bytes, range_flag, stream, rec);
    *n_launches_host = rec.n > 0 ? rec.n - 1 : 0;
    return rc;
}

int pope_vit_launch_count(int depth) { return depth > 0 ? 7 * depth + 2 : 0; }

}
```

pope_amd/dinov2.py:

```python
import warnings
import ctypes as C
import math
from functools import partial

import torch
import torch.nn as nn
import torch.nn.functional as F

from . import _lib
from ._lib import PopeRangeError, check, on_device_of, ptr, require_cuda, stream_of


DEFAULT_PRECISION = "f16x3"


class _PatchEmbed(nn.Module):
    def __init__(self, img_size, patch_size, in_chans, embed_dim):
        super().__init__()
        self.img_size = (img_size, img_size)
        self.patch_size = (patch_size, patch_size)
        self.patches_resolution = (img_size // patch_size, img_size // patch_size)
        self.num_patches = self.patches_resolution[0] * self.patches_resolution[1]
        self.in_chans, self.embed_dim = in_chans, embed_dim
        self.proj = nn.Conv2d(in_chans, embed_dim, kernel_size=patch_size, stride=patch_size)


class _Attention(nn.Module):
    def __init__(self, dim, num_heads, qkv_bias, proj_bias):
        super().__init__()
        self.num_heads = num_heads
        self.scale = (dim // num_heads) ** -0.5
        self.qkv = nn.Linear(dim, dim * 3, bias=qkv_bias)
        self.proj = nn.Linear(dim, dim, bias=proj_bias)


class _Mlp(nn.Module):
    def __init__(self, dim, hidden, bias):
        super().__init__()
        self.fc1 = nn.Linear(dim, hidden, bias=bias)
        self.fc2 = nn.Linear(hidden, dim, bias=bias)


def swiglu_hidden(dim, mlp_ratio):
    return (int(int(dim * mlp_ratio) * 2 / 3) + 7) // 8 * 8


def swiglu_permutation(hidden):
    t = torch.arange(hidden).view(hidden // 32, 1, 32)
    return torch.cat([t, t + hidden], dim=1).reshape(-1)


class _SwiGLUFFN(nn.Module):

    def __init__(self, dim, hidden, bias):
        super().__init__()
        self.w12 = nn.Linear(dim, 2 * hidden, bias=bias)
        self.w3 = nn.Linear(hidden, dim, bias=bias)


class _LayerScale(nn.Module):
    def __init__(self, dim, init_values):
        super().__init__()
        self.gamma = nn.Parameter(init_values * torch.ones(dim))


class _Block(nn.Module):
    def __init__(self, dim, num_heads, mlp_ratio, qkv_bias, proj_bias, ffn_bias, init_values, swiglu=False):
        super().__init__()
        self.norm1 = nn.LayerNorm(dim, eps=1e-6)
        self.attn = _Attention(dim, num_heads, qkv_bias, proj_bias)
        self.ls1 = _LayerScale(dim, init_values)
        self.norm2 = nn.LayerNorm(dim, eps=1e-6)
        self.mlp = _SwiGLUFFN(dim, swiglu_hidden(dim, mlp_ratio), ffn_bias) if swiglu else _Mlp(dim, int(dim * mlp_ratio), ffn_bias)
        self.ls2 = _LayerScale(dim, init_values)


class DinoVisionTransformer(nn.Module):

    def __init__(self, img_size=224, patch_size=16, in_chans=3, embed_dim=768, depth=12, num_heads=12,
                 mlp_ratio=4.0, qkv_bias=True, ffn_bias=True, proj_bias=True, drop_path_rate=0.0,
                 drop_path_uniform=False, init_values=None, ffn_layer="mlp", block_chunks=0, **_ignored):
        super().__init__()
        if in_chans != 3:
            raise NotImplementedError("pope_amd: the patch-embed kernel is built for 3-channel images")
        if embed_dim != num_heads * 64:
            raise NotImplementedError("pope_amd: attention kernel is built for head_dim 64 (all DINOv2 archs)")
        if ffn_layer not in ("mlp", "swiglu", "swiglufused"):
# ... 89 lines not shown
                    raise PopeRangeError(msg)
                warnings.warn(msg + "; this model runs with precision='f32'")
                w = self._weights("f32")
                self._wcache[precision] = self._wcache["f32"]
                return w
        tensors = []

        def P(t):
            t = t.detach()
            if t.dtype != torch.float32:
                raise TypeError("pope_amd kernels are fp32 (the reference path is fp32, SURVEY.md A15)")
            t = t.contiguous()
            tensors.append(t)
            return t.data_ptr()

        def planes(wt, plain=None):
            if precision not in ("f16x3", "f16") or not wt.is_cuda or wt.shape[1] % 32:
                return None
            if (precision == "f16") if plain is None else plain:
                pl = (wt.detach().float() * _lib.PLANES_W_SCALE).half().contiguous()
            else:
                pl = _lib.to_planes(wt, _lib.PLANES_W_SCALE)
            tensors.append(pl)
            return pl.data_ptr()

        blocks = (_lib.VitBlockWeights * self.n_blocks)()
        for i, b in enumerate(self.blocks):
            w1, b1 = self._ffn_first(b)
            fc2 = self._ffn_linears(b)[1]
            blocks[i] = _lib.VitBlockWeights(
                P(b.norm1.weight), P(b.norm1.bias), P(b.attn.qkv.weight), P(b.attn.qkv.bias),
                P(b.attn.proj.weight), P(b.attn.proj.bias), P(b.ls1.gamma), P(b.norm2.weight), P(b.norm2.bias),
                P(w1), P(b1), P(fc2.weight), P(fc2.bias), P(b.ls2.gamma),
                planes(b.attn.qkv.weight), planes(w1), planes(fc2.weight),
                planes(b.attn.proj.weight))
        pw = self.patch_embed.proj.weight.detach().reshape(self.embed_dim, -1)
        patch_wp = None
        if precision in ("f16x3", "f16") and pw.is_cuda:
            kp = (pw.shape[1] + 31) // 32 * 32
            patch_wp = planes(torch.nn.functional.pad(pw.float(), (0, kp - pw.shape[1])), plain=False)
        w = _lib.VitWeights(self.embed_dim, self.n_blocks, self.num_heads, self.patch_size,
                            self.ffn_hidden, P(pw),
                            P(self.norm.weight), P(self.norm.bias), blocks, _lib.PRECISIONS[precision], patch_wp)
        self._wcache[precision] = (dev_ptr, w, blocks, tensors)
        return w

    def interpolate_pos_encoding(self, x, w, h):
        npatch = x.shape[1] - 1
        N = self.pos_embed.shape[1] - 1
        if npatch == N and w == h:
            return self.pos_embed
        pos = self.pos_embed.detach().float().cpu()
        cls_pos, patch_pos = pos[:, 0], pos[:, 1:]
        dim = pos.shape[-1]
        g = int(math.sqrt(N))
        w0, h0 = w // self.patch_size + 0.1, h // self.patch_size + 0.1
        patch_pos = F.interpolate(patch_pos.reshape(1, g, g, dim).permute(0, 3, 1, 2),
                                  scale_factor=(w0 / math.sqrt(N), h0 / math.sqrt(N)), mode="bicubic")
        assert int(w0) == patch_pos.shape[-2] and int(h0) == patch_pos.shape[-1]
        patch_pos = patch_pos.permute(0, 2, 3, 1).reshape(1, -1, dim)
        return torch.cat((cls_pos.unsqueeze(0), patch_pos), dim=1).to(self.pos_embed.device)

    def _posb(self, H, W, ntok):
        key = (H, W) + _lib.params_key((self.pos_embed, self.cls_token, self.patch_embed.proj.bias))
        if key not in self._posb_cache:
            if len(self._posb_cache) >= 32:
                self._posb_cache = {}
            dummy = torch.empty(1, ntok, 1)
            pos = self.interpolate_pos_encoding(dummy, H, W)[0].detach().float().to(self.pos_embed.device)
            posb = pos + self.patch_embed.proj.bias.detach()[None, :]
            posb[0] = pos[0] + self.cls_token.detach()[0, 0]
            self._posb_cache[key] = posb.contiguous()
        return self._posb_cache[key]

    def _workspace(self, nbytes, device):
        if not isinstance(self._ws, dict):
            self._ws = {}
        key = (str(device), torch.cuda.current_stream(device).cuda_stream)
        ws = self._ws.get(key)
        if ws is None or ws.numel() < nbytes:
            ws = self._ws[key] = torch.empty(nbytes, dtype=torch.uint8, device=device)
        return ws

    def _run(self, x, taps=(), out_norm=None, range_flag=None, precision=None):
        require_cuda(x, "DinoVisionTransformer.forward")
        require_cuda(self.cls_token, "DinoVisionTransformer weights")
        if x.dtype != torch.float32:
            raise TypeError("pope_amd DINOv2 expects float32 images")
        x = x.contiguous()
        B, nc, H, W = x.shape
        p = self.patch_size
        assert H % p == 0, f"Input image height {H} is not a multiple of patch height {p}"
        assert W % p == 0, f"Input image width {W} is not a multiple of patch width: {p}"
        ntok = 1 + (H // p) * (W // p)
        dim = self.embed_dim
        precision = precision or self.precision
        if B == 0:
            e = torch.empty(0, ntok, dim, device=x.device, dtype=torch.float32)
            return e, (out_norm if out_norm is not None else e.clone()), [e.clone() for _ in taps]
        widest = max(4 * dim, self.ffn_hidden)
        max_b = max(1, ((1 << 32) - (1 << 20)) // ((ntok * widest + 256 * widest) * 4))
        max_b = min(max_b, getattr(self, "_max_batch", None) or max_b)
        if B > max_b:
            x_pre = torch.empty(B, ntok, dim, device=x.device, dtype=torch.float32)
            x_norm = out_norm if out_norm is not None else torch.empty(B, ntok, dim, device=x.device, dtype=torch.float32)
            tap_out = [torch.empty(B, ntok, dim, device=x.device, dtype=torch.float32) for _ in taps]
            for s in range(0, B, max_b):
                pre_s, _, taps_s = self._run(x[s:s + max_b], taps, out_norm=x_norm[s:s + max_b], range_flag=range_flag,
                                             precision=precision)
                x_pre[s:s + max_b] = pre_s
                for dst, src in zip(tap_out, taps_s):
                    dst[s:s + max_b] = src
            return x_pre, x_norm, tap_out
        with on_device_of(x):
            w = self._weights(precision)
            guarded = w.precision in (_lib.PREC_F16X3, _lib.PREC_F16)
            own_flag = None
            if guarded and range_flag is None:
                own_flag = range_flag = torch.zeros(1, dtype=torch.int32, device=x.device)
            flag_ptr = C.c_void_p(range_flag.data_ptr()) if (guarded and range_flag is not None) else None
            posb = self._posb(H, W, ntok)
            L = _lib.lib()
            nbytes = L.pope_vit_workspace_bytes(B, ntok, dim, w.hidden)
            ws = self._workspace(nbytes, x.device)
            x_pre = torch.empty(B, ntok, dim, device=x.device, dtype=torch.float32)
            if out_norm is None:
                x_norm = torch.empty(B, ntok, dim, device=x.device, dtype=torch.float32)
            else:
                if out_norm.shape != (B, ntok, dim) or out_norm.dtype != torch.float32 or not out_norm.is_contiguous() \
                        or out_norm.device != x.device:
                    raise ValueError("out_norm must be a contiguous float32 [B, ntok, dim] tensor on the input's device")
                x_norm = out_norm
            tap_out = [torch.empty(B, ntok, dim, device=x.device, dtype=torch.float32) for _ in taps]
            tap_blocks = (C.c_int * max(1, len(taps)))(*taps)
            tap_ptrs = (C.c_void_p * max(1, len(taps)))(*[t.data_ptr() for t in tap_out])
            ffn = _lib.FFN_KINDS[self.ffn]
            slot = self.profiler.next_slot() if (self.profiler is not None and not taps) else None
            if slot is not None:
                off, ev, cap, kinds = slot
                n_launch = C.c_int()
                check(L.pope_vit_forward_ffn_profiled_mask_f32(C.byref(w), ffn, ptr(x), B, H, W, ptr(posb), ptr(x_pre), ptr(x_norm),
                                                               C.c_void_p(ws.data_ptr()), ws.numel(), flag_ptr,
                                                               stream_of(x.device), ev, cap, kinds, C.byref(n_launch),
                                                               self.profiler.mask),
                      "pope_vit_forward_ffn_profiled_mask_f32")
                self.profiler.commit(off, n_launch.value)
            else:
                check(L.pope_vit_forward_ffn_f32(C.byref(w), ffn, ptr(x), B, H, W, ptr(posb), ptr(x_pre), ptr(x_norm),
                                                 len(taps), tap_blocks, tap_ptrs, C.c_void_p(ws.data_ptr()), ws.numel(),
                                                 flag_ptr, stream_of(x.device)), "pope_vit_forward_ffn_f32")
        if own_flag is not None:
            bits = int(own_flag.item())
            if bits:
                self.range_overflow(bits)
                return self._run(x, taps, out_norm=out_norm, precision="f32")
        return x_pre, x_norm, tap_out

    def range_overflow(self, bits):
        self.overflow_events += 1
        msg = (f"pope_amd: f16x3 range contract breached ({_lib.describe_range_bits(bits)}: |value| * scale "
               f">= {_lib.F16_MAX:g} or non-finite)")
        if self.on_overflow == "raise":
            raise PopeRangeError(msg)
        if self.overflow_events == 1:
            warnings.warn(msg + "; re-running on the fp32 MFMA (precision='f32')")

    def prepare_tokens_with_masks(self, x, masks=None):
        if masks is not None:
            raise NotImplementedError("pope_amd: iBOT mask tokens are training-only (out of the hot path)")
        from . import ops
        B, nc, H, W = x.shape
        ntok = 1 + (H // self.patch_size) * (W // self.patch_size)
        require_cuda(x, "prepare_tokens_with_masks")
        prec = "f16x3" if self._weights().precision in (_lib.PREC_F16X3, _lib.PREC_F16) else "f32"
        args = (x, self.patch_embed.proj.weight.detach(), self._posb(H, W, ntok), self.patch_size)
        if prec == "f32":
            return ops.patch_embed(*args, precision="f32")
        flag = torch.zeros(1, dtype=torch.int32, device=x.device)
        out = ops.patch_embed(*args, precision="f16x3", range_flag=flag)
        bits = int(flag.item())
        if bits:
            self.range_overflow(bits)
            out = ops.patch_embed(*args, precision="f32")
        return out

    def forward_features(self, x, masks=None, out_norm=None, range_flag=None, precision=None):
        if isinstance(x, list):
            raise NotImplementedError("pope_amd: nested-tensor (list) inputs are a training-time xformers path")
        if masks is not None:
            raise NotImplementedError("pope_amd: iBOT mask tokens are training-only (out of the hot path)")
        x_pre, x_norm, _ = self._run(x, out_norm=out_norm, range_flag=range_flag, precision=precision)
        return {"x_norm_clstoken": x_norm[:, 0], "x_norm_patchtokens": x_norm[:, 1:],
                "x_prenorm": x_pre, "masks": masks}

    def get_intermediate_layers(self, x, n=1, reshape=False, return_class_token=False, norm=True):
        from . import ops
        total = self.n_blocks
        take = list(range(total - n, total)) if isinstance(n, int) else list(n)
        _, _, outs = self._run(x, taps=take)
        assert len(outs) == len(take), f"only {len(outs)} / {len(take)} blocks found"
        if norm:
            outs = [ops.layernorm(o, self.norm.weight.detach(), self.norm.bias.detach(), 1e-6) for o in outs]
        cls = [o[:, 0] for o in outs]
        outs = [o[:, 1:] for o in outs]
        if reshape:
            B, _, H, W = x.shape
            outs = [o.reshape(B, H // self.patch_size, W // self.patch_size, -1).permute(0, 3, 1, 2).contiguous()
                    for o in outs]
        if return_class_token:
            return tuple(zip(outs, cls))
        return tuple(outs)

    def forward(self, *args, is_training=False, **kwargs):
        ret = self.forward_features(*args, **kwargs)
        return ret if is_training else self.head(ret["x_norm_clstoken"])


def vit_small(patch_size=16, **kw):
    return DinoVisionTransformer(patch_size=patch_size, embed_dim=384, depth=12, num_heads=6, mlp_ratio=4, **kw)


def vit_base(patch_size=16, **kw):
    return DinoVisionTransformer(patch_size=patch_size, embed_dim=768, depth=12, num_heads=12, mlp_ratio=4, **kw)


def vit_large(patch_size=16, **kw):
    return DinoVisionTransformer(patch_size=patch_size, embed_dim=1024, depth=24, num_heads=16, mlp_ratio=4, **kw)


def vit_giant2(patch_size=16, **kw):
    return DinoVisionTransformer(patch_size=patch_size, embed_dim=1536, depth=40, num_heads=24, mlp_ratio=4, **kw)


build_vits14 = partial(vit_small, patch_size=14, img_size=518, init_values=1e-5, ffn_layer="mlp", block_chunks=0)
build_vitg14 = partial(vit_giant2, patch_size=14, img_size=518, init_values=1e-5, ffn_layer="swiglufused", block_chunks=0)
```

pope_amd/matcher.py:

```python
import ctypes as C
import warnings

import torch
import torch.nn as nn

from . import _lib
from ._lib import PopeRangeError, check, on_device_of, ptr, require_cuda, stream_of

default_cfg = {
    "backbone_type": "ResNetFPN",
    "resolution": (8, 2),
    "fine_window_size": 5,
    "fine_concat_coarse_feat": True,
    "resnetfpn": {"initial_dim": 128, "block_dims": [128, 196, 256]},
    "coarse": {"d_model": 256, "d_ffn": 256, "nhead": 8, "layer_names": ["self", "cross"] * 4,
               "attention": "linear", "temp_bug_fix": False},
    "match_coarse": {"thr": 0.2, "border_rm": 2, "match_type": "dual_softmax", "dsmax_temperature": 0.1,
                     "skh_iters": 3, "skh_init_bin_score": 1.0, "skh_prefilter": True,
                     "train_coarse_percent": 0.4, "train_pad_num_gt_min": 200},
    "fine": {"d_model": 128, "d_ffn": 128, "nhead": 8, "layer_names": ["self", "cross"], "attention": "linear"},
}


def _rows_contiguous(f):
    if f.stride(2) == 1 and f.stride(1) == f.shape[2] and f.stride(0) >= f.shape[1] * f.shape[2] \
            and f.stride(0) % 4 == 0 and f.data_ptr() % 16 == 0:
        return f
    return f.contiguous()


DEFAULT_PRECISION = "f16x3"


@torch.no_grad()
def dense_match(feat0, feat1, hw0_c, hw1_c, hw0_i, thr=0.2, border_rm=2, temperature=0.1, precision=None,
                on_overflow="rerun_f32", want_conf=True, mask0=None, mask1=None, border_mask0=None, border_mask1=None,
                scale0=None, scale1=None, match_type="dual_softmax", bin_score=None, skh_iters=3, skh_prefilter=True):
    if match_type not in ("dual_softmax", "sinkhorn"):
        raise ValueError(f"dense_match: match_type is 'dual_softmax' or 'sinkhorn', got {match_type!r}")
    sinkhorn = match_type == "sinkhorn"
    if sinkhorn:
        if not isinstance(bin_score, torch.Tensor):
            raise TypeError("dense_match: match_type='sinkhorn' needs bin_score as a float32 tensor (0-d or one element)")
        if bin_score.dtype != torch.float32:
            raise TypeError(f"dense_match: bin_score is float32, got {bin_score.dtype}")
        if bin_score.numel() != 1:
            raise ValueError(f"dense_match: bin_score holds one value, got shape {tuple(bin_score.shape)}")
        if int(skh_iters) < 1:
            raise ValueError(f"dense_match: skh_iters >= 1, got {skh_iters}")
    require_cuda(feat0, "dense_match")
    require_cuda(feat1, "dense_match")
    if feat0.dtype != torch.float32 or feat1.dtype != torch.float32:
        raise TypeError("dense_match expects float32 features")
    feat0, feat1 = _rows_contiguous(feat0), _rows_contiguous(feat1)
    n, L, Cc = feat0.shape
    S = feat1.shape[1]
    h0, w0 = int(hw0_c[0]), int(hw0_c[1])
    h1, w1 = int(hw1_c[0]), int(hw1_c[1])
    assert feat1.shape[0] == n and feat1.shape[2] == Cc and L == h0 * w0 and S == h1 * w1
    dev = feat0.device
    if mask0 is not None and mask0.dim() == 3:
        mask0 = mask0.flatten(-2)
    if mask1 is not None and mask1.dim() == 3:
        mask1 = mask1.flatten(-2)
    fill0 = _lib.padding_mask(mask0, (n, L), dev, "dense_match mask0")
    fill1 = _lib.padding_mask(mask1, (n, S), dev, "dense_match mask1")
    bord0 = _lib.padding_mask(border_mask0, (n, h0, w0), dev, "dense_match border_mask0")
    bord1 = _lib.padding_mask(border_mask1, (n, h1, w1), dev, "dense_match border_mask1")
    sc0 = _lib.pair_scale(scale0, n, dev, "dense_match scale0")
    sc1 = _lib.pair_scale(scale1, n, dev, "dense_match scale1")
    extra = (fill0, fill1, bord0, bord1, sc0, sc1)
    masked = any(t is not None for t in extra)
    if n == 0:
        el, ef = torch.empty(0, dtype=torch.int64, device=dev), torch.empty(0, dtype=torch.float32, device=dev)
        out = {"b_ids": el, "i_ids": el.clone(), "j_ids": el.clone(), "gt_mask": torch.empty(0, dtype=torch.bool, device=dev),
               "m_bids": el.clone(), "mkpts0_c": ef.reshape(0, 2), "mkpts1_c": ef.reshape(0, 2).clone(), "mconf": ef.clone(),
               "counts": torch.empty(0, dtype=torch.int32),
               "conf_matrix": torch.empty(0, L, S, dtype=torch.float32, device=dev) if want_conf else None}
        return out
    lib = _lib.lib()
    precision = precision or DEFAULT_PRECISION
    if Cc % 32 or Cc < 64:
        precision = "f32"
    prec = _lib.PRECISIONS[precision]
    if sinkhorn:
        bin_score = bin_score.detach()
        if bin_score.device != dev:
            bin_score = bin_score.to(dev)
        ws_bytes = lib.pope_dense_match_sinkhorn_workspace_bytes(n, L, S, Cc, prec, 1 if want_conf else 0,
                                                                 int(bord0 is not None or bord1 is not None))
    elif masked:
        ws_bytes = lib.pope_dense_match_masked_workspace_bytes(n, L, S, Cc, prec, 1 if want_conf else 0,
                                                               int(bord0 is not None or bord1 is not None))
    else:
        ws_bytes = lib.pope_dense_match_workspace_bytes_prec(n, L, S, Cc, prec, 1 if want_conf else 0)
    ws = torch.empty(ws_bytes, dtype=torch.uint8, device=dev)
    conf = torch.empty(n, L, S, dtype=torch.float32, device=dev) if want_conf else None
    cap = n * L
    b_ids = torch.empty(cap, dtype=torch.int64, device=dev)
    i_ids = torch.empty(cap, dtype=torch.int64, device=dev)
    j_ids = torch.empty(cap, dtype=torch.int64, device=dev)
    mconf = torch.empty(cap, dtype=torch.float32, device=dev)
    mk0 = torch.empty(cap, 2, dtype=torch.float32, device=dev)
    mk1 = torch.empty(cap, 2, dtype=torch.float32, device=dev)
    counts = torch.zeros(n + 2, dtype=torch.int32, device=dev)
    flag_ptr = C.c_void_p(counts.data_ptr() + 4 * (n + 1)) if precision == "f16x3" else None
    scale = hw0_i[0] / hw0_c[0]
    bs0 = feat0.stride(0) if n > 1 else L * Cc
    bs1 = feat1.stride(0) if n > 1 else S * Cc
    with on_device_of(feat0):
        if sinkhorn:
            check(lib.pope_dense_match_sinkhorn_f32(C.c_void_p(feat0.data_ptr()), bs0, C.c_void_p(feat1.data_ptr()),
                                                    bs1, n, L, S, Cc, h0, w0, h1, w1, float(thr), int(border_rm),
                                                    C.c_void_p(bin_score.data_ptr()), int(skh_iters), int(bool(skh_prefilter)),
                                                    float(scale), *[ptr(t) for t in extra], ptr(conf), ptr(b_ids),
                                                    ptr(i_ids), ptr(j_ids), ptr(mconf), ptr(mk0), ptr(mk1), ptr(counts),
                                                    C.c_void_p(ws.data_ptr()), ws_bytes, prec, flag_ptr, stream_of(dev)),
                  "pope_dense_match_sinkhorn_f32")
        elif masked:
            check(lib.pope_dense_match_masked_f32(C.c_void_p(feat0.data_ptr()), bs0, C.c_void_p(feat1.data_ptr()),
                                                  bs1, n, L, S, Cc, h0, w0, h1, w1, float(thr), int(border_rm),
                                                  float(temperature), float(scale), *[ptr(t) for t in extra], ptr(conf), ptr(b_ids),
                                                  ptr(i_ids), ptr(j_ids), ptr(mconf), ptr(mk0), ptr(mk1), ptr(counts),
                                                  C.c_void_p(ws.data_ptr()), ws_bytes, prec, flag_ptr, stream_of(dev)),
                  "pope_dense_match_masked_f32")
        else:
            check(lib.pope_dense_match_prec_f32(C.c_void_p(feat0.data_ptr()), bs0, C.c_void_p(feat1.data_ptr()),
                                                bs1, n, L, S, Cc, h0, w0, h1, w1, float(thr), int(border_rm),
                                                float(temperature), float(scale), ptr(conf), ptr(b_ids), ptr(i_ids), ptr(j_ids),
                                                ptr(mconf), ptr(mk0), ptr(mk1), ptr(counts), C.c_void_p(ws.data_ptr()), ws_bytes,
                                                prec, flag_ptr, stream_of(dev)), "pope_dense_match_prec_f32")
    counts_h = counts.cpu()
    if int(counts_h[n + 1]):
        msg = (f"pope_amd: f16x3 range contract breached in dense_match ({_lib.describe_range_bits(int(counts_h[n + 1]))}: "
               f"|feat| / sqrt(C) * {_lib.PLANES_W_SCALE:g} >= {_lib.F16_MAX:g} or non-finite)")
        if on_overflow == "raise":
            raise PopeRangeError(msg)
        warnings.warn(msg + "; re-running with the fp32-MFMA contraction")
        del conf, ws, b_ids, i_ids, j_ids, mconf, mk0, mk1
        return dense_match(feat0, feat1, hw0_c, hw1_c, hw0_i, thr, border_rm, temperature, "f32", on_overflow, want_conf,
                           *extra, match_type=match_type, bin_score=bin_score, skh_iters=skh_iters, skh_prefilter=skh_prefilter)
    m = int(counts_h[n])
    b_ids, i_ids, j_ids, mconf = b_ids[:m], i_ids[:m], j_ids[:m], mconf[:m]
    return {
        "conf_matrix": conf,
        "b_ids": b_ids, "i_ids": i_ids, "j_ids": j_ids,
        "gt_mask": mconf == 0, "m_bids": b_ids,
        "mkpts0_c": mk0[:m], "mkpts1_c": mk1[:m], "mconf": mconf,
        "counts": counts_h[:n],
    }


def _loftr():
    from . import loftr
    return loftr


class CoarseMatching(nn.Module):

    def __init__(self, config):
        super().__init__()
        self.config = config
        self.thr = config["thr"]
        self.border_rm = config["border_rm"]
        self.train_coarse_percent = config["train_coarse_percent"]
        self.train_pad_num_gt_min = config["train_pad_num_gt_min"]
        self.match_type = config["match_type"]
        if self.match_type == "dual_softmax":
            self.temperature = config["dsmax_temperature"]
        elif self.match_type == "sinkhorn":
            self.bin_score = nn.Parameter(torch.tensor(config["skh_init_bin_score"], dtype=torch.float32))
            self.skh_iters = config["skh_iters"]
            self.skh_prefilter = config["skh_prefilter"]
        else:
            raise NotImplementedError(f"pope_amd: match_type is 'dual_softmax' or 'sinkhorn', got {self.match_type!r}")

    def forward(self, feat_c0, feat_c1, data, mask_c0=None, mask_c1=None):
        if self.training:
            raise NotImplementedError("pope_amd: inference only (call .eval())")
        if mask_c0 is not None and mask_c1 is None:
            raise ValueError("CoarseMatching: mask_c0 needs mask_c1 (the fill is mask_c0[i] * mask_c1[j])")
        fill0, fill1 = (mask_c0, mask_c1) if mask_c0 is not None else (None, None)
        bord0, bord1 = (data["mask0"], data["mask1"]) if "mask0" in data else (None, None)
        if self.match_type == "sinkhorn":
            how = {"match_type": "sinkhorn", "bin_score": self.bin_score, "skh_iters": self.skh_iters,
                   "skh_prefilter": self.skh_prefilter}
        else:
            how = {"temperature": self.temperature}
        out = dense_match(feat_c0, feat_c1, data["hw0_c"], data["hw1_c"], data["hw0_i"], self.thr, self.border_rm,
                          mask0=fill0, mask1=fill1, border_mask0=bord0, border_mask1=bord1,
                          scale0=data.get("scale0"), scale1=data.get("scale1"), **how)
        out.pop("counts")
        data.update(out)

# ... 283 lines not shown
```

pope_amd/pipeline.py:

```python
import json

import numpy as np
import torch

from .matcher import dense_match


def shard_range(n_items, rank, world):
    base, rem = divmod(n_items, world)
    start = rank * base + min(rank, rem)
    return start, start + base + (1 if rank < rem else 0)


def gather_counts(local_counts, group=None):
    import torch.distributed as dist
    if not (dist.is_available() and dist.is_initialized()) or dist.get_world_size(group) == 1:
        return local_counts.clone()
    world = dist.get_world_size(group)
    n_local = torch.tensor([local_counts.numel()], dtype=torch.int64, device=local_counts.device)
    sizes = [torch.zeros_like(n_local) for _ in range(world)]
    dist.all_gather(sizes, n_local, group=group)
    sizes = [int(s) for s in sizes]
    cap = max(sizes)
    padded = torch.zeros(cap, dtype=local_counts.dtype, device=local_counts.device)
    padded[:local_counts.numel()] = local_counts
    out = [torch.empty_like(padded) for _ in range(world)]
    dist.all_gather(out, padded, group=group)
    return torch.cat([o[:s] for o, s in zip(out, sizes)])


def load_pair_list(path):
    with open(path) as f:
        doc = json.load(f)
    rows = []
    for o, obj in enumerate(doc["objects"]):
        for key, pairs in obj["bins"].items():
            rows.extend((o, int(key), int(a), int(b)) for a, b in pairs)
    return np.asarray(rows, dtype=np.int64).reshape(-1, 4)


def walk_pair_list(n_pairs, process_batch, batch=128, rank=0, world=1, group=None, device="cpu"):
    lo, hi = shard_range(n_pairs, rank, world)
    parts, n_batches = [], 0
    for s in range(lo, hi, batch):
        e = min(s + batch, hi)
        c = torch.as_tensor(process_batch(s, e), dtype=torch.int32)
        if c.numel() != e - s:
            raise ValueError(f"process_batch({s}, {e}) returned {c.numel()} counts")
        parts.append(c.to(device))
        n_batches += 1
    local = torch.cat(parts) if parts else torch.zeros(0, dtype=torch.int32, device=device)
    return gather_counts(local, group), n_batches


class PairPipeline:

    def __init__(self, model, chunk=64, thr=0.2, border_rm=2, temperature=0.1, streams=1, want_conf=False,
                 match_precision=None):
        self.model = model
        self.chunk = chunk
        self.thr, self.border_rm, self.temperature = thr, border_rm, temperature
        self.n_streams = streams
        self.want_conf = want_conf
        self.match_precision = match_precision
        self._streams = None
        self.reruns = 0

    def _chunk(self, images, tokens, s, flag=None, precision=None):
        self.model(images[s:s + self.chunk], is_training=True, out_norm=tokens[s:s + self.chunk], range_flag=flag,
                   precision=precision)

    @torch.no_grad()
    def extract(self, images, flags=None):
        starts = list(range(0, images.shape[0], self.chunk))
        B, _, H, W = images.shape
        p = self.model.patch_size
        ntok = 1 + (H // p) * (W // p)
        tokens = torch.empty(B, ntok, self.model.embed_dim, device=images.device, dtype=torch.float32)
        fl = (lambda k: None) if flags is None else (lambda k: flags[k:k + 1])
        if self.n_streams <= 1 or len(starts) == 1:
            for k, s in enumerate(starts):
                self._chunk(images, tokens, s, fl(k))
            return tokens
        main = torch.cuda.current_stream(images.device)
        with torch.cuda.device(images.device):
            self.model._weights()
            self.model._posb(H, W, ntok)
        if self._streams is None:
            self._streams = [torch.cuda.Stream(images.device) for _ in range(self.n_streams)]
        for st in self._streams:
            st.wait_stream(main)
        for k, s in enumerate(starts):
            with torch.cuda.stream(self._streams[k % self.n_streams]):
                self._chunk(images, tokens, s, fl(k))
        for st in self._streams:
            main.wait_stream(st)
        return tokens

    def _match(self, t0, t1, hw_c, hw_i):
        return dense_match(t0[:, 1:], t1[:, 1:], hw_c, hw_c, hw_i, self.thr, self.border_rm, self.temperature,
                           precision=self.match_precision, on_overflow=self.model.on_overflow, want_conf=self.want_conf)

    @torch.no_grad()
    def __call__(self, img0, img1):
        assert img0.shape == img1.shape
        n, _, H, W = img0.shape
        p = self.model.patch_size
        n_chunks = -(-n // self.chunk)
        flags = torch.zeros(2 * n_chunks, dtype=torch.int32, device=img0.device)
        t0, t1 = self.extract(img0, flags[:n_chunks]), self.extract(img1, flags[n_chunks:])
        hw_c = (H // p, W // p)
        out = self._match(t0, t1, hw_c, (H, W))
        bits = flags.cpu()
        if int(bits.abs().sum()):
            self.model.range_overflow(int(np.bitwise_or.reduce(bits.numpy())))
            for k in range(n_chunks):
                if int(bits[k]):
                    self._chunk(img0, t0, k * self.chunk, precision="f32")
                if int(bits[n_chunks + k]):
                    self._chunk(img1, t1, k * self.chunk, precision="f32")
            self.reruns += 1
            out = self._match(t0, t1, hw_c, (H, W))
        out["feat0"], out["feat1"] = t0[:, 1:], t1[:, 1:]
        out["cls0"], out["cls1"] = t0[:, 0], t1[:, 0]
        return out
```

Measured before the change: 1489.

## Emit matcher f16x3 planes from the final LayerNorm GEMM epilogue

```diff
diff --git a/include/pope_hip.h b/include/pope_hip.h
--- a/include/pope_hip.h
+++ b/include/pope_hip.h
@@ -113,6 +113,13 @@
                              const float* posb, float* x_prenorm, float* x_norm,
                              int n_taps, const int* tap_blocks_host, float* const* tap_out_host,
                              void* workspace, size_t workspace_bytes, unsigned* range_flag, void* stream);
+
+size_t pope_vit_forward_match_workspace_bytes(int B, int ntok, int dim, int hidden, int has_x_prenorm);
+int pope_vit_forward_match_f32(const pope_vit_weights* w_host, int ffn, const float* img, int B, int H, int W,
+                               const float* posb, float* x_prenorm, float* x_norm,
+                               int n_taps, const int* tap_blocks_host, float* const* tap_out_host,
+                               void* workspace, size_t workspace_bytes, unsigned* range_flag, void* stream,
+                               void* match_planes, float match_divisor, float match_scale, int* match_planes_written_host);
 
 enum { POPE_K_PATCH_EMBED = 0, POPE_K_LAYERNORM = 1, POPE_K_GEMM_QKV = 2, POPE_K_ATTENTION = 3,
        POPE_K_GEMM_PROJ = 4, POPE_K_GEMM_FC1 = 5, POPE_K_GEMM_FC2 = 6, POPE_K_TAP_COPY = 7 };
@@ -127,6 +134,13 @@
                                            void* workspace, size_t workspace_bytes, unsigned* range_flag, void* stream,
                                            void* const* events_host, int n_events, int* kinds_host,
                                            int* n_launches_host, unsigned kind_mask);
+int pope_vit_forward_match_profiled_mask_f32(const pope_vit_weights* w_host, int ffn, const float* img, int B, int H, int W,
+                                             const float* posb, float* x_prenorm, float* x_norm,
+                                             void* workspace, size_t workspace_bytes, unsigned* range_flag, void* stream,
+                                             void* const* events_host, int n_events, int* kinds_host,
+                                             int* n_launches_host, unsigned kind_mask,
+                                             void* match_planes, float match_divisor, float match_scale,
+                                             int* match_planes_written_host);
 int pope_event_create(void** event_host);
 int pope_event_destroy(void* event);
 int pope_event_elapsed_ms(void* start, void* stop, float* ms_host);
@@ -140,6 +154,12 @@
                               float* mconf, float* mkpts0_c, float* mkpts1_c, int* counts,
                               void* workspace, size_t workspace_bytes, int precision, unsigned* range_flag,
                               void* stream);
+size_t pope_dense_match_planes_workspace_bytes(int n, int L, int S, int C, int publish_conf);
+int pope_dense_match_planes_f32(const void* planes0, const void* planes1, int n, int L, int S, int C,
+                                int h0, int w0, int h1, int w1, float thr, int border_rm, float temperature, float scale,
+                                float* conf_matrix, long long* b_ids, long long* i_ids, long long* j_ids,
+                                float* mconf, float* mkpts0_c, float* mkpts1_c, int* counts,
+                                void* workspace, size_t workspace_bytes, void* stream);
 size_t pope_dense_match_masked_workspace_bytes(int n, int L, int S, int C, int precision, int publish_conf, int has_border_masks);
 int pope_dense_match_masked_f32(const float* feat0, long long stride0, const float* feat1, long long stride1,
                                 int n, int L, int S, int C, int h0, int w0, int h1, int w1,
diff --git a/pope_amd/_lib.py b/pope_amd/_lib.py
--- a/pope_amd/_lib.py
+++ b/pope_amd/_lib.py
@@ -162,10 +162,19 @@
     "pope_vit_forward_ffn_f32": (C.c_int, [C.POINTER(VitWeights), C.c_int, C.c_void_p, C.c_int, C.c_int, C.c_int, C.c_void_p,
                                            C.c_void_p, C.c_void_p, C.c_int, c_int_p, C.POINTER(C.c_void_p),
                                            C.c_void_p, C.c_size_t, C.c_void_p, C.c_void_p]),
+    "pope_vit_forward_match_workspace_bytes": (C.c_size_t, [C.c_int] * 5),
+    "pope_vit_forward_match_f32": (C.c_int, [C.POINTER(VitWeights), C.c_int, C.c_void_p, C.c_int, C.c_int, C.c_int, C.c_void_p,
+                                             C.c_void_p, C.c_void_p, C.c_int, c_int_p, C.POINTER(C.c_void_p),
+                                             C.c_void_p, C.c_size_t, C.c_void_p, C.c_void_p,
+                                             C.c_void_p, C.c_float, C.c_float, c_int_p]),
     "pope_vit_forward_ffn_profiled_mask_f32": (C.c_int, [C.POINTER(VitWeights), C.c_int, C.c_void_p, C.c_int, C.c_int, C.c_int,
                                                          C.c_void_p, C.c_void_p, C.c_void_p, C.c_void_p, C.c_size_t,
                                                          C.c_void_p, C.c_void_p, C.POINTER(C.c_void_p), C.c_int, c_int_p,
                                                          c_int_p, C.c_uint]),
+    "pope_vit_forward_match_profiled_mask_f32": (C.c_int, [C.POINTER(VitWeights), C.c_int, C.c_void_p, C.c_int, C.c_int, C.c_int,
+                                                           C.c_void_p, C.c_void_p, C.c_void_p, C.c_void_p, C.c_size_t,
+                                                           C.c_void_p, C.c_void_p, C.POINTER(C.c_void_p), C.c_int, c_int_p,
+                                                           c_int_p, C.c_uint, C.c_void_p, C.c_float, C.c_float, c_int_p]),
     "pope_vit_launch_count": (C.c_int, [C.c_int]),
     "pope_vit_forward_profiled_mask_f32": (C.c_int, [C.POINTER(VitWeights), C.c_void_p, C.c_int, C.c_int, C.c_int,
                                                      C.c_void_p, C.c_void_p, C.c_void_p, C.c_void_p, C.c_size_t,
@@ -182,6 +191,10 @@
     "pope_dense_match_prec_f32": (C.c_int, [C.c_void_p, C.c_longlong, C.c_void_p, C.c_longlong] + [C.c_int] * 8
                                   + [C.c_float, C.c_int, C.c_float, C.c_float] + [C.c_void_p] * 8
                                   + [C.c_void_p, C.c_size_t, C.c_int, C.c_void_p, C.c_void_p]),
+    "pope_dense_match_planes_workspace_bytes": (C.c_size_t, [C.c_int] * 5),
+    "pope_dense_match_planes_f32": (C.c_int, [C.c_void_p, C.c_void_p] + [C.c_int] * 8
+                                    + [C.c_float, C.c_int, C.c_float, C.c_float] + [C.c_void_p] * 8
+                                    + [C.c_void_p, C.c_size_t, C.c_void_p]),
     "pope_dense_match_masked_workspace_bytes": (C.c_size_t, [C.c_int] * 7),
     "pope_dense_match_masked_f32": (C.c_int, [C.c_void_p, C.c_longlong, C.c_void_p, C.c_longlong] + [C.c_int] * 8
                                     + [C.c_float, C.c_int, C.c_float, C.c_float] + [C.c_void_p] * 6 + [C.c_void_p] * 8
diff --git a/pope_amd/csrc/capi.hip b/pope_amd/csrc/capi.hip
--- a/pope_amd/csrc/capi.hip
+++ b/pope_amd/csrc/capi.hip
@@ -225,7 +225,7 @@
 struct MatchLayout {
     size_t nl, ns, part, rowp, colp, pl0, pl1, simb, total;
     int ncb, nrb, nrb2, ldp;
-    MatchLayout(int n, int L, int S, int C, int precision, bool publish_conf) {
+    MatchLayout(int n, int L, int S, int C, int precision, bool publish_conf, bool planes_given = false) {
         nl = pope_align256(size_t(n) * L * 4);
         ns = pope_align256(size_t(n) * S * 4);
         ncb = 2 * ((S + 127) / 128);
@@ -236,8 +236,8 @@
         const bool x3 = precision == POPE_PREC_F16X3;
         rowp = x3 ? pope_align256(size_t(n) * L * ncb * 8) : 0;
         colp = x3 ? pope_align256(size_t(n) * nrb * ldp * 4) : 0;
-        pl0 = x3 ? pope_align256(size_t(n) * L * C * 4) : 0;
-        pl1 = x3 ? pope_align256(size_t(n) * S * C * 4) : 0;
+        pl0 = x3 && !planes_given ? pope_align256(size_t(n) * L * C * 4) : 0;
+        pl1 = x3 && !planes_given ? pope_align256(size_t(n) * S * C * 4) : 0;
         simb = publish_conf ? 0 : pope_align256(size_t(n) * L * S * 4);
         total = 7 * nl + 3 * ns + part + rowp + 2 * colp + pl0 + pl1 + simb;
     }
@@ -295,15 +295,17 @@
                       const float* scale0, const float* scale1, float* conf_matrix, long long* b_ids, long long* i_ids,
                       long long* j_ids, float* mconf, float* mkpts0_c, float* mkpts1_c, int* counts, void* workspace,
                       size_t workspace_bytes, int precision, unsigned* range_flag, void* stream, const float* bin_score,
-                      int skh_iters, int skh_prefilter) {
-    if (!feat0 || !feat1 || !b_ids || !i_ids || !j_ids || !mconf || !mkpts0_c || !mkpts1_c || !counts || !workspace)
+                      int skh_iters, int skh_prefilter, const void* planes0_in = nullptr, const void* planes1_in = nullptr) {
+    const bool planes_given = planes0_in || planes1_in;
+    if (planes_given && (!planes0_in || !planes1_in || precision != POPE_PREC_F16X3 || (C & 31) || C < 64)) return POPE_ERR_ARG;
+    if ((!planes_given && (!feat0 || !feat1)) || !b_ids || !i_ids || !j_ids || !mconf || !mkpts0_c || !mkpts1_c || !counts || !workspace)
         return POPE_ERR_ARG;
     if (n <= 0 || L <= 0 || S <= 0 || C <= 0) return POPE_ERR_ARG;
     if (precision != POPE_PREC_F32_MFMA && precision != POPE_PREC_F16X3) return POPE_ERR_ARG;
     StreamDevice on_device(stream);
     const bool publish = conf_matrix != nullptr;
     const bool padded = border_mask0 || border_mask1;
-    const MatchLayout lay(n, L, S, C, precision, publish);
+    const MatchLayout lay(n, L, S, C, precision, publish, planes_given);
     const size_t ext_bytes = padded ? pope_align256(size_t(n) * 4 * 4) : 0;
     const SinkhornLayout skh(n, L, S);
     if (workspace_bytes < lay.total + ext_bytes + (bin_score ? skh.total : 0)) return POPE_ERR_WORKSPACE;
@@ -331,8 +333,9 @@
         p.row_part = ws.take<float>(lay.rowp);
         p.col_pmax = ws.take<float>(lay.colp);
         p.col_psum = ws.take<float>(lay.colp);
-        p.planes0 = ws.take(lay.pl0);
-        p.planes1 = ws.take(lay.pl1);
+        p.planes0 = planes_given ? const_cast<void*>(planes0_in) : ws.take(lay.pl0);
+        p.planes1 = planes_given ? const_cast<void*>(planes1_in) : ws.take(lay.pl1);
+        p.planes_given = planes_given;
     }
     p.sim = publish ? conf_matrix : ws.take<float>(lay.simb);
     p.counts = counts;
@@ -364,6 +367,22 @@
                              mkpts1_c, counts, workspace, workspace_bytes, precision, range_flag, stream, nullptr, 0, 0);
 }
 
+size_t pope_dense_match_planes_workspace_bytes(int n, int L, int S, int C, int publish_conf) {
+    if (n <= 0 || L <= 0 || S <= 0 || C <= 0) return 0;
+    return MatchLayout(n, L, S, C, POPE_PREC_F16X3, publish_conf != 0, true).total;
+}
+
+int pope_dense_match_planes_f32(const void* planes0, const void* planes1, int n, int L, int S, int C, int h0, int w0, int h1, int w1,
+                                float thr, int border_rm, float temperature, float scale, float* conf_matrix, long long* b_ids,
+                                long long* i_ids, long long* j_ids, float* mconf, float* mkpts0_c, float* mkpts1_c, int* counts,
+                                void* workspace, size_t workspace_bytes, void* stream) {
+    if (!planes0 || !planes1) return POPE_ERR_ARG;
+    return dense_match_entry(nullptr, (long long)L * C, nullptr, (long long)S * C, n, L, S, C, h0, w0, h1, w1, thr, border_rm,
+                             temperature, scale, nullptr, nullptr, nullptr, nullptr, nullptr, nullptr, conf_matrix, b_ids, i_ids,
+                             j_ids, mconf, mkpts0_c, mkpts1_c, counts, workspace, workspace_bytes, POPE_PREC_F16X3, nullptr, stream,
+                             nullptr, 0, 0, planes0, planes1);
+}
+
 size_t pope_dense_match_sinkhorn_workspace_bytes(int n, int L, int S, int C, int precision, int publish_conf, int has_border_masks) {
     if (n <= 0 || L <= 0 || S <= 0 || C <= 0) return 0;
     return pope_dense_match_masked_workspace_bytes(n, L, S, C, precision, publish_conf, has_border_masks) + SinkhornLayout(n, L, S).total;
diff --git a/pope_amd/csrc/gemm_rowln.hip b/pope_amd/csrc/gemm_rowln.hip
--- a/pope_amd/csrc/gemm_rowln.hip
+++ b/pope_amd/csrc/gemm_rowln.hip
@@ -72,11 +72,12 @@
     __builtin_amdgcn_fence(__ATOMIC_ACQUIRE, "workgroup", "local");
 }
 
-enum { RL_LN_PLANES = 0, RL_LN_F32 = 1, RL_BIAS_PLANES = 2, RL_GELU_PLANES = 3 };
+enum { RL_LN_PLANES = 0, RL_LN_F32 = 1, RL_BIAS_PLANES = 2, RL_GELU_PLANES = 3, RL_LN_F32_MATCH = 4 };
 
 template <class G, int MODE, bool RES_TABLE>
 __global__ __launch_bounds__(G::RTH) void gemm_rowln16_kernel(const GemmParams g, int n_tiles, int ncol) {
-    constexpr bool LN = MODE == RL_LN_PLANES || MODE == RL_LN_F32, LN_PLANES = MODE == RL_LN_PLANES;
+    constexpr bool MATCH = MODE == RL_LN_F32_MATCH;
+    constexpr bool LN = MODE == RL_LN_PLANES || MODE == RL_LN_F32 || MATCH, LN_PLANES = MODE == RL_LN_PLANES;
     constexpr int RM = G::RM, NMI = G::NMI, RTH = G::RTH, STAGE_H = G::STAGE_H, EROWS = G::EROWS, AROWS = G::AROWS, WROWS = G::WROWS;
     constexpr int WMR = 16 * NMI;
     constexpr int NIA = AROWS / 8, NIW = WROWS / 8;
@@ -141,6 +142,8 @@
     const __amdgpu_buffer_rsrc_t rx = __builtin_amdgcn_make_buffer_rsrc(g.C, 0, unsigned(g.M) * unsigned(RN) * 4u, 0x00020000);
     const __amdgpu_buffer_rsrc_t rln = __builtin_amdgcn_make_buffer_rsrc(LN_PLANES ? g.ln_planes : static_cast<void*>(g.ln_f32), 0,
                                                                          unsigned(g.M) * unsigned(RN) * 4u, 0x00020000);
+    [[maybe_unused]] const __amdgpu_buffer_rsrc_t rmp = __builtin_amdgcn_make_buffer_rsrc(
+        MATCH ? g.match_pl : nullptr, 0, MATCH && g.match_pl ? unsigned(g.M - g.M / g.match_ntok) * unsigned(RN) * 4u : 0u, 0x00020000);
     const __amdgpu_buffer_rsrc_t rres = __builtin_amdgcn_make_buffer_rsrc(
         const_cast<float*>(g.res), 0, unsigned(RES_TABLE ? g.res_mod : g.M) * unsigned(g.ldres) * 4u, 0x00020000);
 
@@ -216,17 +219,19 @@
                 __builtin_amdgcn_raw_buffer_store_b128(__builtin_bit_cast(u32x4, v), rdst, off, 0, 0);
             }
         };
-#pragma unroll
-        for (int mi = 0; mi < NMI; ++mi) {
-#pragma unroll
-            for (int h = 0; h < 16 / EROWS; ++h) {
-                if (EROWS == 16 || (l15 >> 3) == h) {
-#pragma unroll
-                    for (int ni = 0; ni < 6; ++ni) *reinterpret_cast<f32x4*>(&wreg[er * 100 + ni * 16 + 4 * q4]) = acc[mi][ni];
+        if (!MATCH || g.C) {
+#pragma unroll
+            for (int mi = 0; mi < NMI; ++mi) {
+#pragma unroll
+                for (int h = 0; h < 16 / EROWS; ++h) {
+                    if (EROWS == 16 || (l15 >> 3) == h) {
+#pragma unroll
+                        for (int ni = 0; ni < 6; ++ni) *reinterpret_cast<f32x4*>(&wreg[er * 100 + ni * 16 + 4 * q4]) = acc[mi][ni];
+                    }
+                    __builtin_amdgcn_wave_barrier();
+                    store_lines(rx, m0 + wm * WMR + mi * 16 + h * EROWS);
+                    __builtin_amdgcn_wave_barrier();
                 }
-                __builtin_amdgcn_wave_barrier();
-                store_lines(rx, m0 + wm * WMR + mi * 16 + h * EROWS);
-                __builtin_amdgcn_wave_barrier();
             }
         }
 #pragma unroll
@@ -255,6 +260,7 @@
 #pragma unroll
         for (int mi = 0; mi < NMI; ++mi) finite_probe += 16 * mi < live ? __builtin_fabsf(mean[mi]) + rstd[mi] : 0.f;
         f32x2 amax = {0.f, 0.f};
+        [[maybe_unused]] f32x2 mamax = {0.f, 0.f}, mnan = {0.f, 0.f};
 #pragma unroll
         for (int mi = 0; mi < NMI; ++mi) {
 #pragma unroll
@@ -282,8 +288,58 @@
                 __builtin_amdgcn_wave_barrier();
                 store_lines(rln, m0 + wm * WMR + mi * 16 + h * EROWS);
                 __builtin_amdgcn_wave_barrier();
-            }
-        }
+                if constexpr (MATCH) {
+                    if (g.match_pl) {
+                        const unsigned ntok_ = unsigned(g.match_ntok);
+                        unsigned rb16 = unsigned(m0 + wm * WMR + mi * 16);
+                        asm volatile("" : "+v"(rb16));
+                        const unsigned b0 = rb16 / ntok_, t0 = rb16 - b0 * ntok_;
+                        if (EROWS == 16 || (l15 >> 3) == h) {
+                            const unsigned tl = t0 + unsigned(l15);
+                            const bool counted = 16 * mi < live && tl != 0 && tl != ntok_;
+#pragma unroll
+                            for (int ni = 0; ni < 6; ++ni) {
+                                const f32x4 lw = *reinterpret_cast<const f32x4*>(ctab + 2 * RN + col0 + 16 * ni);
+                                const f32x4 lb = *reinterpret_cast<const f32x4*>(ctab + 3 * RN + col0 + 16 * ni);
+                                const f32x4 y = acc[mi][ni] * rstd[mi] * lw + lb;
+                                const f32x4 ys = (y / g.match_div) * g.match_scale;
+                                const f32x4 yc = counted ? ys : f32x4{0.f, 0.f, 0.f, 0.f};
+                                pope_amax4x2(mamax, yc);
+                                pope_nan_sum4(mnan, yc);
+                                f16x4 hi, lo;
+                                pope_split4(ys, hi, lo);
+                                const int c = ni * 16 + 4 * q4;
+                                _Float16* hp = reinterpret_cast<_Float16*>(wreg) + er * 200 + pope_planes_col(c);
+                                *reinterpret_cast<f16x4*>(hp) = hi;
+                                *reinterpret_cast<f16x4*>(hp + 32) = lo;
+                            }
+                        }
+                        __builtin_amdgcn_wave_barrier();
+                        {
+                            int el = elane;
+                            asm volatile("" : "+v"(el));
+                            const int epiece = el & 7;
+                            const int row_base = m0 + wm * WMR + mi * 16 + h * EROWS;
+#pragma unroll
+                            for (int t = 0; t < (EROWS * 3) / 8; ++t) {
+                                const int L = t * 8 + (el >> 3), row = (L * 43) >> 7, ln = L - 3 * row;
+                                const f32x4 v = *reinterpret_cast<const f32x4*>(&wreg[row * 100 + ln * 32 + epiece * 4]);
+                                const unsigned r = unsigned(row_base + row), tr = t0 + unsigned(h * EROWS + row);
+                                const unsigned b = b0 + (tr >= ntok_ ? 1u : 0u);
+                                const unsigned off = tr == 0 || tr == ntok_
+                                                         ? 0xFFFFFF00u
+                                                         : (r - b - 1u) * unsigned(RN) * 4u + unsigned(wn * 96 + ln * 32 + epiece * 4) * 4u;
+                                __builtin_amdgcn_raw_buffer_store_b128(__builtin_bit_cast(u32x4, v), rmp, off, 0, 0);
+                            }
+                        }
+                        __builtin_amdgcn_wave_barrier();
+                    }
+                }
+            }
+        }
+        if constexpr (MATCH)
+            pope_range_flag(g.range_flag, POPE_RANGE_MATCH,
+                            !(__builtin_fmaxf(mamax[0], mamax[1]) < POPE_F16_OVERFLOW) || pope_nan_seen(mnan));
         if constexpr (LN_PLANES)
             pope_range_flag(g.range_flag, POPE_RANGE_LAYERNORM,
                             !(__builtin_fmaxf(amax[0], amax[1]) < POPE_F16_OVERFLOW) ||
@@ -489,7 +545,9 @@
 }
 
 bool pope_gemm_rowln_args_ok(const GemmParams& g) {
-    if (!g.a_pl || !g.w_pl || !g.C || !g.res || !g.ln_w || !g.ln_b || (!g.ln_planes) == (!g.ln_f32) || g.M <= 0) return false;
+    if (!g.a_pl || !g.w_pl || !g.res || !g.ln_w || !g.ln_b || (!g.ln_planes) == (!g.ln_f32) || g.M <= 0) return false;
+    if ((!g.C || g.match_pl) && (!g.ln_f32 || g.res_mod > 0)) return false;
+    if (g.match_pl && (g.match_ntok < 16 || g.M % g.match_ntok || !(g.match_div > 0.f) || !(g.match_scale > 0.f))) return false;
     if (!pope_gemm_rowln_supported(g)) return false;
     return g.res_mod >= 0 && (g.res_mod > 0 || g.gamma);
 }
@@ -499,6 +557,7 @@
     g.rl_prefetch = 1;
     if (!pope_gemm_rowln_args_ok(g)) return POPE_ERR_ARG;
     if (g.res_mod > 0) return g.ln_planes ? launch_rowln<RL_LN_PLANES, true>(g, stream) : launch_rowln<RL_LN_F32, true>(g, stream);
+    if (!g.C || g.match_pl) return launch_rowln<RL_LN_F32_MATCH, false>(g, stream);
     return g.ln_planes ? launch_rowln<RL_LN_PLANES, false>(g, stream) : launch_rowln<RL_LN_F32, false>(g, stream);
 }
 
diff --git a/pope_amd/csrc/kernels.h b/pope_amd/csrc/kernels.h
--- a/pope_amd/csrc/kernels.h
+++ b/pope_amd/csrc/kernels.h
@@ -68,6 +68,9 @@
     int ntok, img_h, img_w, patch, grid_w;
     const float* sim_mask0;
     const float* sim_mask1;
+    void* match_pl;
+    int match_ntok;
+    float match_div, match_scale;
 };
 
 int pope_launch_gemm_nt_f32(const GemmParams& g, hipStream_t stream);
@@ -132,6 +135,7 @@
     float* sim;
     int publish_conf;
     void* planes0; void* planes1;
+    int planes_given;
     float* row_part; float* col_pmax; float* col_psum;
     int ncb, nrb, ldp;
     float* row_max; float* row_sum;
diff --git a/pope_amd/csrc/match.hip b/pope_amd/csrc/match.hip
--- a/pope_amd/csrc/match.hip
+++ b/pope_amd/csrc/match.hip
@@ -505,8 +505,12 @@
 int check_match_params(const MatchParams& p) {
     if (p.n <= 0 || p.L <= 0 || p.S <= 0 || p.C <= 0 || (p.C & 3) || p.n > 65535) return POPE_ERR_ARG;
     if (p.L != p.h0 * p.w0 || p.S != p.h1 * p.w1) return POPE_ERR_ARG;
-    if (p.bs0 < (long long)p.L * p.C || p.bs1 < (long long)p.S * p.C || (p.bs0 & 3) || (p.bs1 & 3)) return POPE_ERR_ARG;
-    if ((reinterpret_cast<uintptr_t>(p.feat0) & 15) || (reinterpret_cast<uintptr_t>(p.feat1) & 15)) return POPE_ERR_ARG;
+    if (p.planes_given) {
+        if (!p.planes0 || !p.planes1 || !p.row_part || !p.col_pmax || !p.col_psum || (p.C & 31) || p.C < 64) return POPE_ERR_ARG;
+    } else {
+        if (p.bs0 < (long long)p.L * p.C || p.bs1 < (long long)p.S * p.C || (p.bs0 & 3) || (p.bs1 & 3)) return POPE_ERR_ARG;
+        if ((reinterpret_cast<uintptr_t>(p.feat0) & 15) || (reinterpret_cast<uintptr_t>(p.feat1) & 15)) return POPE_ERR_ARG;
+    }
     if (!p.sim || !p.colmax_part || p.nrb2 != pope_match_nrb2(p.L) || p.ldp < p.S || (p.ldp & 3)) return POPE_ERR_ARG;
     if ((p.border0 || p.border1) && !p.extent) return POPE_ERR_ARG;
     return POPE_OK;
@@ -517,9 +521,12 @@
     bool sim_done = false;
     if (p.planes0 && p.planes1 && p.row_part && p.col_pmax && p.col_psum && (p.C & 31) == 0 && p.C >= 64) {
         const float norm = sqrtf(float(p.C));
-        int rc = pope_launch_div_planes(p.feat0, p.bs0, p.planes0, p.n, p.L, p.C, norm, K_PLANES_W_SCALE, p.range_flag, stream);
-        if (!rc) rc = pope_launch_div_planes(p.feat1, p.bs1, p.planes1, p.n, p.S, p.C, norm, K_PLANES_W_SCALE, p.range_flag, stream);
-        if (rc) return rc;
+        int rc = 0;
+        if (!p.planes_given) {
+            rc = pope_launch_div_planes(p.feat0, p.bs0, p.planes0, p.n, p.L, p.C, norm, K_PLANES_W_SCALE, p.range_flag, stream);
+            if (!rc) rc = pope_launch_div_planes(p.feat1, p.bs1, p.planes1, p.n, p.S, p.C, norm, K_PLANES_W_SCALE, p.range_flag, stream);
+            if (rc) return rc;
+        }
         GemmParams g = {};
         g.a_pl = p.planes0; g.w_pl = p.planes1; g.C = p.sim;
         g.M = p.L; g.N = p.S; g.K = p.C; g.lda = p.C; g.ldw = p.C; g.ldc = p.S;
@@ -535,7 +542,7 @@
             sim_done = true;
             hipLaunchKernelGGL(combine_row_stats_kernel, dim3(unsigned((size_t(p.n) * p.L + 255) / 256)), dim3(256), 0, stream, p);
             if (col_stats) hipLaunchKernelGGL(combine_col_stats_kernel, dim3((p.S + 255) / 256, p.n), dim3(256), 0, stream, p);
-        } else if (rc != POPE_ERR_ARG) {
+        } else if (rc != POPE_ERR_ARG || p.planes_given) {
             return rc;
         }
     }
diff --git a/pope_amd/csrc/vit_forward.hip b/pope_amd/csrc/vit_forward.hip
--- a/pope_amd/csrc/vit_forward.hip
+++ b/pope_amd/csrc/vit_forward.hip
@@ -60,8 +60,14 @@
 static int vit_forward_impl(const pope_vit_weights* w, int ffn, const float* img, int B, int H, int W, const float* posb,
                             float* x_prenorm, float* x_norm, int n_taps, const int* tap_blocks_host,
                             float* const* tap_out_host, void* workspace, size_t workspace_bytes, unsigned* range_flag,
-                            void* stream_, Recorder& rec) {
-    if (!w || !img || !posb || !x_prenorm || !workspace || !w->blocks_host) return POPE_ERR_ARG;
+                            void* stream_, Recorder& rec, void* match_planes = nullptr, float match_div = 0.f,
+                            float match_scale = 0.f, int* match_written_host = nullptr) {
+    if (match_written_host) *match_written_host = 0;
+    if (!w || !img || !posb || !workspace || !w->blocks_host) return POPE_ERR_ARG;
+    if (!x_prenorm && !x_norm) return POPE_ERR_ARG;
+    for (int t = 0; !x_prenorm && t < n_taps; ++t)
+        if (tap_blocks_host && tap_blocks_host[t] == w->depth - 1) return POPE_ERR_ARG;
+    if (match_planes && (!x_norm || !(match_div > 0.f) || !(match_scale > 0.f))) return POPE_ERR_ARG;
     if (w->dim != w->heads * 64 || w->patch <= 0 || H % w->patch || W % w->patch || B <= 0) return POPE_ERR_ARG;
     if (n_taps < 0 || (n_taps > 0 && (!tap_blocks_host || !tap_out_host))) return POPE_ERR_ARG;
     hipStream_t stream = static_cast<hipStream_t>(stream_);
@@ -76,16 +82,17 @@
     const int fc1_n = swiglu ? 2 * hidden : hidden, fc1_epi = swiglu ? int(EPI_BIAS_SWIGLU) : int(EPI_BIAS_GELU);
     const int ntok = 1 + (H / w->patch) * (W / w->patch);
     const int rows = B * ntok;
-    if (workspace_bytes < pope_vit_workspace_bytes(B, ntok, dim, hidden)) return POPE_ERR_WORKSPACE;
+    if (workspace_bytes < pope_vit_forward_match_workspace_bytes(B, ntok, dim, hidden, x_prenorm != nullptr)) return POPE_ERR_WORKSPACE;
 
     pope_carver ws{static_cast<char*>(workspace)};
     float* xn = ws.take<float>(size_t(rows) * dim * sizeof(float));
+    float* x_own = x_prenorm ? nullptr : ws.take<float>(size_t(rows) * dim * sizeof(float));
     float* big = reinterpret_cast<float*>(ws.at);
     const size_t big_bytes = workspace_bytes - size_t(ws.at - static_cast<char*>(workspace));
     float* qkv = big;
     float* att = big + size_t(rows) * 3 * dim;
     float* hid = big;
-    float* x = x_prenorm;
+    float* x = x_prenorm ? x_prenorm : x_own;
     const float eps = 1e-6f;
 
     bool planes = (prec == POPE_PREC_F16X3 || prec == POPE_PREC_F16) && dim % 32 == 0 && dim >= 64 && hidden % 32 == 0;
@@ -166,7 +173,13 @@
             const pope_vit_block_weights& kn = w->blocks_host[i + 1];
             POPE_TRY(rowln(hid, k.fc2_wp, hidden, k.fc2_b, k.ls2, x, 0, kn.norm1_w, kn.norm1_b, xn, nullptr));
         } else if (fused && x_norm) {
-            POPE_TRY(rowln(hid, k.fc2_wp, hidden, k.fc2_b, k.ls2, x, 0, w->norm_w, w->norm_b, nullptr, x_norm));
+            GemmParams g = pope_linear_rowln_params(hid, k.fc2_wp, rows, dim, hidden, k.fc2_b, k.ls2, x, 0, x_prenorm, w->norm_w,
+                                                    w->norm_b, eps, nullptr, x_norm, range_flag);
+            if (match_planes && ntok >= 16) {
+                g.match_pl = match_planes; g.match_ntok = ntok; g.match_div = match_div; g.match_scale = match_scale;
+                if (match_written_host) *match_written_host = 1;
+            }
+            POPE_TRY(pope_launch_gemm_rowln(g, stream));
         } else {
             POPE_TRY(linear(hid, k.fc2_w, k.fc2_wp, k.fc2_b, x, nullptr, dim, hidden, EPI_BIAS_LS_RES, k.ls2, x));
         }
@@ -188,6 +201,23 @@
 }
 
 extern "C" {
+
+size_t pope_vit_forward_match_workspace_bytes(int B, int ntok, int dim, int hidden, int has_x_prenorm) {
+    const size_t base = pope_vit_workspace_bytes(B, ntok, dim, hidden);
+    if (!base || has_x_prenorm) return base;
+    return base + pope_align256(size_t(B) * ntok * dim * sizeof(float));
+}
+
+int pope_vit_forward_match_f32(const pope_vit_weights* w, int ffn, const float* img, int B, int H, int W, const float* posb,
+                               float* x_prenorm, float* x_norm, int n_taps, const int* tap_blocks_host,
+                               float* const* tap_out_host, void* workspace, size_t workspace_bytes, unsigned* range_flag,
+                               void* stream, void* match_planes, float match_divisor, float match_scale,
+                               int* match_planes_written_host) {
+    Recorder rec{nullptr, 0, nullptr, 0};
+    return vit_forward_impl(w, ffn, img, B, H, W, posb, x_prenorm, x_norm, n_taps, tap_blocks_host, tap_out_host, workspace,
+                            workspace_bytes, range_flag, stream, rec, match_planes, match_divisor, match_scale,
+                            match_planes_written_host);
+}
 
 size_t pope_vit_workspace_bytes(int B, int ntok, int dim, int hidden) {
     if (B <= 0 || ntok <= 0 || dim <= 0 || hidden <= 0) return 0;
@@ -227,11 +257,24 @@
                                            size_t workspace_bytes, unsigned* range_flag, void* stream,
                                            void* const* events_host, int n_events, int* kinds_host, int* n_launches_host,
                                            unsigned kind_mask) {
+    if (!x_prenorm) return POPE_ERR_ARG;
+    return pope_vit_forward_match_profiled_mask_f32(w, ffn, img, B, H, W, posb, x_prenorm, x_norm, workspace, workspace_bytes,
+                                                    range_flag, stream, events_host, n_events, kinds_host, n_launches_host, kind_mask,
+                                                    nullptr, 0.f, 0.f, nullptr);
+}
+
+int pope_vit_forward_match_profiled_mask_f32(const pope_vit_weights* w, int ffn, const float* img, int B, int H, int W,
+                                             const float* posb, float* x_prenorm, float* x_norm, void* workspace,
+                                             size_t workspace_bytes, unsigned* range_flag, void* stream,
+                                             void* const* events_host, int n_events, int* kinds_host, int* n_launches_host,
+                                             unsigned kind_mask, void* match_planes, float match_divisor, float match_scale,
+                                             int* match_planes_written_host) {
     if (!events_host || n_events < 2 || !kinds_host || !n_launches_host) return POPE_ERR_ARG;
     Recorder rec{events_host, n_events, kinds_host, 0};
     rec.mask = kind_mask;
     const int rc = vit_forward_impl(w, ffn, img, B, H, W, posb, x_prenorm, x_norm, 0, nullptr, nullptr, workspace,
-                                    workspace_bytes, range_flag, stream, rec);
+                                    workspace_bytes, range_flag, stream, rec, match_planes, match_divisor, match_scale,
+                                    match_planes_written_host);
     *n_launches_host = rec.n > 0 ? rec.n - 1 : 0;
     return rc;
 }
diff --git a/pope_amd/dinov2.py b/pope_amd/dinov2.py
--- a/pope_amd/dinov2.py
+++ b/pope_amd/dinov2.py
@@ -3,6 +3,7 @@
 import math
 from functools import partial
 
+import numpy as np
 import torch
 import torch.nn as nn
 import torch.nn.functional as F
@@ -258,7 +259,7 @@
             ws = self._ws[key] = torch.empty(nbytes, dtype=torch.uint8, device=device)
         return ws
 
-    def _run(self, x, taps=(), out_norm=None, range_flag=None, precision=None):
+    def _run(self, x, taps=(), out_norm=None, range_flag=None, precision=None, match_planes=None, want_prenorm=True):
         require_cuda(x, "DinoVisionTransformer.forward")
         require_cuda(self.cls_token, "DinoVisionTransformer weights")
         if x.dtype != torch.float32:
@@ -271,6 +272,14 @@
         ntok = 1 + (H // p) * (W // p)
         dim = self.embed_dim
         precision = precision or self.precision
+        self.match_planes_written = False
+        if match_planes is not None:
+            if match_planes.shape != (B, ntok - 1, dim) or match_planes.dtype != torch.float32 or not match_planes.is_contiguous() \
+                    or match_planes.device != x.device:
+                raise ValueError("match_planes must be a contiguous float32 [B, ntok - 1, dim] tensor (f16 hi/lo planes) on the "
+                                 "input's device")
+            if range_flag is None:
+                raise ValueError("match_planes needs the caller's range_flag: the matcher's range bit travels in it")
         if B == 0:
             e = torch.empty(0, ntok, dim, device=x.device, dtype=torch.float32)
             return e, (out_norm if out_norm is not None else e.clone()), [e.clone() for _ in taps]
@@ -278,15 +287,20 @@
         max_b = max(1, ((1 << 32) - (1 << 20)) // ((ntok * widest + 256 * widest) * 4))
         max_b = min(max_b, getattr(self, "_max_batch", None) or max_b)
         if B > max_b:
-            x_pre = torch.empty(B, ntok, dim, device=x.device, dtype=torch.float32)
+            x_pre = torch.empty(B, ntok, dim, device=x.device, dtype=torch.float32) if want_prenorm else None
             x_norm = out_norm if out_norm is not None else torch.empty(B, ntok, dim, device=x.device, dtype=torch.float32)
             tap_out = [torch.empty(B, ntok, dim, device=x.device, dtype=torch.float32) for _ in taps]
+            written = match_planes is not None
             for s in range(0, B, max_b):
                 pre_s, _, taps_s = self._run(x[s:s + max_b], taps, out_norm=x_norm[s:s + max_b], range_flag=range_flag,
-                                             precision=precision)
-                x_pre[s:s + max_b] = pre_s
+                                             precision=precision, want_prenorm=want_prenorm,
+                                             match_planes=None if match_planes is None else match_planes[s:s + max_b])
+                written = written and self.match_planes_written
+                if want_prenorm:
+                    x_pre[s:s + max_b] = pre_s
                 for dst, src in zip(tap_out, taps_s):
                     dst[s:s + max_b] = src
+            self.match_planes_written = written
             return x_pre, x_norm, tap_out
         with on_device_of(x):
             w = self._weights(precision)
@@ -297,9 +311,11 @@
             flag_ptr = C.c_void_p(range_flag.data_ptr()) if (guarded and range_flag is not None) else None
             posb = self._posb(H, W, ntok)
             L = _lib.lib()
-            nbytes = L.pope_vit_workspace_bytes(B, ntok, dim, w.hidden)
+            nbytes = L.pope_vit_forward_match_workspace_bytes(B, ntok, dim, w.hidden, 1 if want_prenorm else 0)
             ws = self._workspace(nbytes, x.device)
-            x_pre = torch.empty(B, ntok, dim, device=x.device, dtype=torch.float32)
+            x_pre = torch.empty(B, ntok, dim, device=x.device, dtype=torch.float32) if want_prenorm else None
+            match = (ptr(match_planes), float(np.sqrt(np.float32(dim))), _lib.PLANES_W_SCALE)
+            written = C.c_int(0)
             if out_norm is None:
                 x_norm = torch.empty(B, ntok, dim, device=x.device, dtype=torch.float32)
             else:
@@ -315,21 +331,23 @@
             if slot is not None:
                 off, ev, cap, kinds = slot
                 n_launch = C.c_int()
-                check(L.pope_vit_forward_ffn_profiled_mask_f32(C.byref(w), ffn, ptr(x), B, H, W, ptr(posb), ptr(x_pre), ptr(x_norm),
-                                                               C.c_void_p(ws.data_ptr()), ws.numel(), flag_ptr,
-                                                               stream_of(x.device), ev, cap, kinds, C.byref(n_launch),
-                                                               self.profiler.mask),
-                      "pope_vit_forward_ffn_profiled_mask_f32")
+                check(L.pope_vit_forward_match_profiled_mask_f32(C.byref(w), ffn, ptr(x), B, H, W, ptr(posb), ptr(x_pre), ptr(x_norm),
+                                                                 C.c_void_p(ws.data_ptr()), ws.numel(), flag_ptr,
+                                                                 stream_of(x.device), ev, cap, kinds, C.byref(n_launch),
+                                                                 self.profiler.mask, *match, C.byref(written)),
+                      "pope_vit_forward_match_profiled_mask_f32")
                 self.profiler.commit(off, n_launch.value)
             else:
-                check(L.pope_vit_forward_ffn_f32(C.byref(w), ffn, ptr(x), B, H, W, ptr(posb), ptr(x_pre), ptr(x_norm),
-                                                 len(taps), tap_blocks, tap_ptrs, C.c_void_p(ws.data_ptr()), ws.numel(),
-                                                 flag_ptr, stream_of(x.device)), "pope_vit_forward_ffn_f32")
+                check(L.pope_vit_forward_match_f32(C.byref(w), ffn, ptr(x), B, H, W, ptr(posb), ptr(x_pre), ptr(x_norm),
+                                                   len(taps), tap_blocks, tap_ptrs, C.c_void_p(ws.data_ptr()), ws.numel(),
+                                                   flag_ptr, stream_of(x.device), *match, C.byref(written)),
+                      "pope_vit_forward_match_f32")
+            self.match_planes_written = bool(written.value)
         if own_flag is not None:
             bits = int(own_flag.item())
             if bits:
                 self.range_overflow(bits)
-                return self._run(x, taps, out_norm=out_norm, precision="f32")
+                return self._run(x, taps, out_norm=out_norm, precision="f32", want_prenorm=want_prenorm)
         return x_pre, x_norm, tap_out
 
     def range_overflow(self, bits):
@@ -360,12 +378,14 @@
             out = ops.patch_embed(*args, precision="f32")
         return out
 
-    def forward_features(self, x, masks=None, out_norm=None, range_flag=None, precision=None):
+    def forward_features(self, x, masks=None, out_norm=None, range_flag=None, precision=None, match_planes=None,
+                         want_prenorm=True):
         if isinstance(x, list):
             raise NotImplementedError("pope_amd: nested-tensor (list) inputs are a training-time xformers path")
         if masks is not None:
             raise NotImplementedError("pope_amd: iBOT mask tokens are training-only (out of the hot path)")
-        x_pre, x_norm, _ = self._run(x, out_norm=out_norm, range_flag=range_flag, precision=precision)
+        x_pre, x_norm, _ = self._run(x, out_norm=out_norm, range_flag=range_flag, precision=precision, match_planes=match_planes,
+                                     want_prenorm=want_prenorm)
         return {"x_norm_clstoken": x_norm[:, 0], "x_norm_patchtokens": x_norm[:, 1:],
                 "x_prenorm": x_pre, "masks": masks}
 
diff --git a/pope_amd/matcher.py b/pope_amd/matcher.py
--- a/pope_amd/matcher.py
+++ b/pope_amd/matcher.py
@@ -35,7 +35,8 @@
 @torch.no_grad()
 def dense_match(feat0, feat1, hw0_c, hw1_c, hw0_i, thr=0.2, border_rm=2, temperature=0.1, precision=None,
                 on_overflow="rerun_f32", want_conf=True, mask0=None, mask1=None, border_mask0=None, border_mask1=None,
-                scale0=None, scale1=None, match_type="dual_softmax", bin_score=None, skh_iters=3, skh_prefilter=True):
+                scale0=None, scale1=None, match_type="dual_softmax", bin_score=None, skh_iters=3, skh_prefilter=True,
+                planes0=None, planes1=None):
     if match_type not in ("dual_softmax", "sinkhorn"):
         raise ValueError(f"dense_match: match_type is 'dual_softmax' or 'sinkhorn', got {match_type!r}")
     sinkhorn = match_type == "sinkhorn"
@@ -83,6 +84,12 @@
     if Cc % 32 or Cc < 64:
         precision = "f32"
     prec = _lib.PRECISIONS[precision]
+    if (planes0 is None) != (planes1 is None):
+        raise ValueError("dense_match: planes0 and planes1 come together")
+    for name, pl, rows in (("planes0", planes0, L), ("planes1", planes1, S)):
+        if pl is not None and (pl.shape != (n, rows, Cc) or pl.dtype != torch.float32 or not pl.is_contiguous() or pl.device != dev):
+            raise ValueError(f"dense_match: {name} is a contiguous float32-typed [n, {rows}, C] planes tensor on the features' device")
+    use_planes = planes0 is not None and precision == "f16x3" and not masked and not sinkhorn
     if sinkhorn:
         bin_score = bin_score.detach()
         if bin_score.device != dev:
@@ -94,7 +101,8 @@
                                                                int(bord0 is not None or bord1 is not None))
     else:
         ws_bytes = lib.pope_dense_match_workspace_bytes_prec(n, L, S, Cc, prec, 1 if want_conf else 0)
-    ws = torch.empty(ws_bytes, dtype=torch.uint8, device=dev)
+    pl_bytes = lib.pope_dense_match_planes_workspace_bytes(n, L, S, Cc, 1 if want_conf else 0) if use_planes else 0
+    ws = torch.empty(pl_bytes if use_planes else ws_bytes, dtype=torch.uint8, device=dev)
     conf = torch.empty(n, L, S, dtype=torch.float32, device=dev) if want_conf else None
     cap = n * L
     b_ids = torch.empty(cap, dtype=torch.int64, device=dev)
@@ -108,8 +116,21 @@
     scale = hw0_i[0] / hw0_c[0]
     bs0 = feat0.stride(0) if n > 1 else L * Cc
     bs1 = feat1.stride(0) if n > 1 else S * Cc
+    status = -1
+    if use_planes:
+        with on_device_of(feat0):
+            status = lib.pope_dense_match_planes_f32(C.c_void_p(planes0.data_ptr()), C.c_void_p(planes1.data_ptr()), n, L, S, Cc,
+                                                     h0, w0, h1, w1, float(thr), int(border_rm), float(temperature), float(scale),
+                                                     ptr(conf), ptr(b_ids), ptr(i_ids), ptr(j_ids), ptr(mconf), ptr(mk0), ptr(mk1),
+                                                     ptr(counts), C.c_void_p(ws.data_ptr()), pl_bytes, stream_of(dev))
+        if status not in (0, -1):
+            check(status, "pope_dense_match_planes_f32")
+        if status:
+            ws = torch.empty(ws_bytes, dtype=torch.uint8, device=dev)
     with on_device_of(feat0):
-        if sinkhorn:
+        if status == 0:
+            pass
+        elif sinkhorn:
             check(lib.pope_dense_match_sinkhorn_f32(C.c_void_p(feat0.data_ptr()), bs0, C.c_void_p(feat1.data_ptr()),
                                                     bs1, n, L, S, Cc, h0, w0, h1, w1, float(thr), int(border_rm),
                                                     C.c_void_p(bin_score.data_ptr()), int(skh_iters), int(bool(skh_prefilter)),
diff --git a/pope_amd/pipeline.py b/pope_amd/pipeline.py
--- a/pope_amd/pipeline.py
+++ b/pope_amd/pipeline.py
@@ -3,7 +3,9 @@
 import numpy as np
 import torch
 
-from .matcher import dense_match
+from .matcher import DEFAULT_PRECISION, dense_match
+
+MATCH_BIT = 16
 
 
 def shard_range(n_items, rank, world):
@@ -66,21 +68,25 @@
         self._streams = None
         self.reruns = 0
 
-    def _chunk(self, images, tokens, s, flag=None, precision=None):
+    def _chunk(self, images, tokens, s, flag=None, precision=None, planes=None):
         self.model(images[s:s + self.chunk], is_training=True, out_norm=tokens[s:s + self.chunk], range_flag=flag,
-                   precision=precision)
+                   precision=precision, want_prenorm=False, match_planes=None if planes is None else planes[s:s + self.chunk])
+        return planes is not None and self.model.match_planes_written
 
     @torch.no_grad()
-    def extract(self, images, flags=None):
+    def extract(self, images, flags=None, planes=None):
         starts = list(range(0, images.shape[0], self.chunk))
         B, _, H, W = images.shape
         p = self.model.patch_size
         ntok = 1 + (H // p) * (W // p)
         tokens = torch.empty(B, ntok, self.model.embed_dim, device=images.device, dtype=torch.float32)
         fl = (lambda k: None) if flags is None else (lambda k: flags[k:k + 1])
+        if planes is not None and flags is None:
+            raise ValueError("extract: planes need flags (the matcher's range bit travels in the chunks' words)")
+        self.planes_written = planes is not None
         if self.n_streams <= 1 or len(starts) == 1:
             for k, s in enumerate(starts):
-                self._chunk(images, tokens, s, fl(k))
+                self.planes_written &= self._chunk(images, tokens, s, fl(k), planes=planes) or planes is None
             return tokens
         main = torch.cuda.current_stream(images.device)
         with torch.cuda.device(images.device):
@@ -92,14 +98,15 @@
             st.wait_stream(main)
         for k, s in enumerate(starts):
             with torch.cuda.stream(self._streams[k % self.n_streams]):
-                self._chunk(images, tokens, s, fl(k))
+                self.planes_written &= self._chunk(images, tokens, s, fl(k), planes=planes) or planes is None
         for st in self._streams:
             main.wait_stream(st)
         return tokens
 
-    def _match(self, t0, t1, hw_c, hw_i):
+    def _match(self, t0, t1, hw_c, hw_i, planes0=None, planes1=None):
         return dense_match(t0[:, 1:], t1[:, 1:], hw_c, hw_c, hw_i, self.thr, self.border_rm, self.temperature,
-                           precision=self.match_precision, on_overflow=self.model.on_overflow, want_conf=self.want_conf)
+                           precision=self.match_precision, on_overflow=self.model.on_overflow, want_conf=self.want_conf,
+                           planes0=planes0, planes1=planes1)
 
     @torch.no_grad()
     def __call__(self, img0, img1):
@@ -108,18 +115,30 @@
         p = self.model.patch_size
         n_chunks = -(-n // self.chunk)
         flags = torch.zeros(2 * n_chunks, dtype=torch.int32, device=img0.device)
-        t0, t1 = self.extract(img0, flags[:n_chunks]), self.extract(img1, flags[n_chunks:])
         hw_c = (H // p, W // p)
-        out = self._match(t0, t1, hw_c, (H, W))
+        pl0 = pl1 = None
+        if (self.match_precision or DEFAULT_PRECISION) == "f16x3" and n:
+            L, dim = hw_c[0] * hw_c[1], self.model.embed_dim
+            pl0, pl1 = (torch.empty(n, L, dim, device=img0.device, dtype=torch.float32) for _ in range(2))
+        t0 = self.extract(img0, flags[:n_chunks], pl0)
+        handed = self.planes_written
+        t1 = self.extract(img1, flags[n_chunks:], pl1)
+        handed = handed and self.planes_written
+        if not handed:
+            pl0 = pl1 = None
+        out = self._match(t0, t1, hw_c, (H, W), pl0, pl1)
         bits = flags.cpu()
         if int(bits.abs().sum()):
-            self.model.range_overflow(int(np.bitwise_or.reduce(bits.numpy())))
-            for k in range(n_chunks):
-                if int(bits[k]):
-                    self._chunk(img0, t0, k * self.chunk, precision="f32")
-                if int(bits[n_chunks + k]):
-                    self._chunk(img1, t1, k * self.chunk, precision="f32")
-            self.reruns += 1
+            del pl0, pl1
+            vit_bits = bits & ~MATCH_BIT
+            if int(vit_bits.abs().sum()):
+                self.model.range_overflow(int(np.bitwise_or.reduce(vit_bits.numpy())))
+                for k in range(n_chunks):
+                    if int(vit_bits[k]):
+                        self._chunk(img0, t0, k * self.chunk, precision="f32")
+                    if int(vit_bits[n_chunks + k]):
+                        self._chunk(img1, t1, k * self.chunk, precision="f32")
+                self.reruns += 1
             out = self._match(t0, t1, hw_c, (H, W))
         out["feat0"], out["feat1"] = t0[:, 1:], t1[:, 1:]
         out["cls0"], out["cls1"] = t0[:, 0], t1[:, 0]
```

New measurement: 1493, median of 6. About the same (+0.3%).
